# matheusfalcaopinto/triple-hybrid-rag

Hardware: AMD Instinct MI355X
Metric: queries/sec (fused top-10) (higher is better)
Workload: dtype f16 MFMA shortlist scan (f32 accumulate) + f64 rescoring of the f32 rows; 1 GPU; 1000000-doc / 768-d dense-only brute-force cosine top-10 (BASELINE.json configs[1]); pipeline=dense, docs=1000000, dim=768, semantic_top_k=100, fused_top_k=10, shortlist=f16, parallelism=single GPU, world_size_seen=1, rescued_queries=0

## Files before the change

triple-hybrid-rag_amd/_native.py:

```python
from __future__ import annotations

import ctypes as C
import os
from typing import Optional, Tuple

import torch

from . import _build

THR_FLAG_CERTIFIED = 1
THR_FLAG_OVERFLOW = 2
THR_FLAG_EXACT = 4
THR_DENSE_MAX_K = 256
THR_BM25_MAX_TERMS = 32
THR_BM25_MAX_QUERIES = 1 << 20
THR_GRAPH_MAX_SEEDS = 16
THR_RRF_MAX_PER_CHANNEL = 128
THR_TOPK_MAX = 128
THR_SCOPE_MAX_COLS = 8
THR_SCOPE_MAX_PREDS = 4096
THR_SCOPE_MAX_QUERIES = 1 << 20
MAXSIM_TOK_DIMS = (16, 32, 64, 96, 128, 192, 256)
ABI_VERSION = 9

_lib = None


class NativeError(RuntimeError):
    pass


_i64, _i32, _dbl, _sz, _vp = C.c_int64, C.c_int, C.c_double, C.c_size_t, C.c_void_p
_SIGNATURES = {
    "thr_abi_version": (C.c_int, []),
    "thr_error_string": (C.c_char_p, [_i32]),
    "thr_device_info": (_i32, [C.POINTER(_i32), C.POINTER(_i64), C.c_char_p, _i32]),
    "thr_embed_postproc": (_i32, [_vp, _i32, _i32, _i32, _vp, _vp]),
    "thr_doc_norms": (_i32, [_vp, _i64, _i32, _vp, _vp, _vp]),
    "thr_dense_workspace_bytes": (_sz, [_i64, _i32, _i32, _i32]),
    "thr_dense_topk": (_i32, [_vp, _vp, _vp, _i64, _i32, _i64, _vp, _i32, _i32, _i32, _vp, _vp, _vp, _vp,
                              _vp, _vp, _vp, _sz, _vp]),
    "thr_dense_exact_workspace_bytes": (_sz, [_i64, _i32]),
    "thr_dense_topk_exact": (_i32, [_vp, _vp, _i64, _i32, _i64, _vp, _i32, _i32, _vp, _vp, _vp, _vp, _vp,
                                    _vp, _vp, _sz, _vp]),
    "thr_dense_scan_probe": (_i32, [_vp, _vp, _i64, _i32, _vp, _i32, _vp, _sz, _vp]),
    "thr_dense_rescue_workspace_bytes": (_sz, [_i32, _i32]),
    "thr_dense_rescue": (_i32, [_vp, _vp, _i64, _i32, _i64, _vp, _i32, _i32, _vp, _vp, _vp, _vp, _vp, _vp, _vp,
                                _vp, _sz, _vp]),
    "thr_dense_quantize_f16": (_i32, [_vp, _i64, _i32, _vp, _vp, _vp]),
    "thr_dense_f16_workspace_bytes": (_sz, [_i64, _i32, _i32, _i32]),
    "thr_dense_f16_copy_bytes": (_sz, [_i64, _i32]),
    "thr_dense_f16_query_tile": (_i32, [_i32, _i32, _i32]),
    "thr_dense_f16_max_queries": (_i32, [_i32, _i32]),
    "thr_dense_topk_f16": (_i32, [_vp, _vp, _dbl, _vp, _vp, _i64, _i32, _i64, _vp, _i32, _i32,
                                  _i32, _vp, _vp, _vp, _vp, _vp, _vp, _vp, _sz, _vp]),
    "thr_dense_shortlist_f16": (_i32, [_vp, _vp, _dbl, _vp, _i64, _i32, _vp, _i32, _i32, _vp, _vp, _i32, _vp,
                                       _vp, _sz, _vp]),
    "thr_dense_floor": (_i32, [_vp, _i32, _i32, _i32, _i32, _vp, _vp]),
    "thr_dense_finish_f16": (_i32, [_vp, _vp, _dbl, _vp, _vp, _i64, _i32, _i64, _vp, _i32, _i32,
                                    _i32, _vp, _vp, _vp, _vp, _i32, _i32, _vp, _vp, _vp, _vp, _vp, _sz, _vp]),
    "thr_dense_scan_probe_f16": (_i32, [_vp, _vp, _vp, _i64, _i32, _vp, _i32, _vp, _sz, _vp]),
    "thr_dense_scan_stamps_f16": (_i32, [_vp, _i64, _i32, _i32, _vp, _sz, _vp, C.POINTER(_i32), _vp]),
    "thr_lexical_build_workspace_bytes": (_sz, [_i64, _i64]),
    "thr_lexical_build": (_i32, [_vp, _vp, _vp, _i64, _i64, _i64, _vp, _vp, _vp, _vp, _vp, _vp, _vp, _sz, _vp]),
    "thr_csr_append": (_i32, [_vp, _i64, _i64, _vp, _vp, _vp, _i64, _i64, _vp, _vp, _vp, _vp, _vp, _i64, _vp]),
    "thr_csr_compact_workspace_bytes": (_sz, [_i64, _i64]),
    "thr_csr_compact": (_i32, [_vp, _i64, _i64, _vp, _vp, _vp, _i64, _i64, _vp, _vp, _vp, _i64, _vp, _vp, _sz, _vp]),
    "thr_scope_resolve_workspace_bytes": (_sz, [_i64, _i32]),
    "thr_scope_resolve": (_i32, [_vp, _i32, _i64, _vp, _i32, _vp, _vp, _i64, _vp, _vp, _vp, _sz, _vp]),
    "thr_dense_topk_rows_workspace_bytes": (_sz, [_i32, _i32, _i32]),
    "thr_dense_topk_rows": (_i32, [_vp, _vp, _i64, _i32, _i64, _vp, _i32, _i32, _vp, _vp, _i64, _i32, _vp,
                                   _vp, _vp, _vp, _vp, _vp, _sz, _vp]),
    "thr_bm25_block_count": (_sz, [_i64]),
    "thr_bm25_bounds": (_i32, [_vp, _vp, _vp, _vp, _vp, _dbl, _dbl, _dbl, _i64, _i64, _vp, _vp, _vp, _vp]),
    "thr_bm25_workspace_bytes": (_sz, [_i32, _i32, _i32]),
    "thr_bm25_dense_stride": (_i64, [_i64]),
    "thr_bm25_dense_rows": (_i32, [_vp, _vp, _vp, _vp, _vp, _i32, _i64, _i64, _vp, _vp, _vp]),
    "thr_bm25_topk": (_i32, [_vp, _vp, _vp, _vp, _vp, _vp, _vp, _vp, _vp, _vp, _vp, _i64, _dbl, _dbl, _dbl, _i64, _i64, _i64,
                             _vp, _i32, _i32, _i32, _i32, _vp, _vp, _vp, _vp, _vp, _vp, _sz, _vp]),
    "thr_graph_workspace_bytes": (_sz, [_i32, _i64]),
    "thr_graph_topk": (_i32, [_vp, _vp, _i64, _vp, _vp, _vp, _vp, _vp, _vp, _i64, _i64, _vp, _i32,
                              _i32, _i32, _i32, _vp, _vp, _vp, _vp, _vp, _sz, _vp]),
    "thr_graph_topk_scoped": (_i32, [_vp, _vp, _i64, _vp, _vp, _vp, _vp, _vp, _vp, _i64, _i64, _vp, _vp, _vp,
                                     _i32, _i32, _i32, _i32, _vp, _vp, _vp, _vp, _vp, _sz, _vp]),
    "thr_rrf_fuse": (_i32, [_vp, _i32, _vp, _i32, _vp, _i32, _i32, _dbl, _dbl, _dbl, _i32, _i32,
                            _vp, _vp, _vp, _vp, _vp]),
    "thr_rrf_fuse_standalone": (_i32, [_vp, _i32, _vp, _i32, _vp, _i32, _i32, _dbl, _dbl, _dbl, _i32, _i32,
                                       _vp, _vp, _vp, _vp, _vp]),
    "thr_fuse_post": (_i32, [_vp, _vp, _vp, _vp, _i32, _i32, _vp, _i32, _vp, _i32, _vp, _i32, _dbl, _i32,
                             _dbl, _i32, _i32, _vp, _vp, _vp, _vp]),
    "thr_rerank_order": (_i32, [_vp, _i32, _i64, _vp, _vp, _i32, _i32, _i32, _vp, _vp, _vp, _vp]),
    "thr_maxsim": (_i32, [_vp, _i32, _i32, _vp, _i64, _i32, _i32, _vp, _i32, _vp, _i32, _vp]),
    "thr_maxsim_ids": (_i32, [_vp, _i32, _i32, _vp, _i64, _i32, _i32, _vp, _i64, _i32, _vp, _i32, _vp]),
    "thr_maxsim_pack": (_i32, [_vp, _i64, _i32, _i32, _vp, _vp]),
    "thr_merge_topk": (_i32, [_vp, _vp, _i32, _i32, _i32, _i64, _i32, _vp, _vp, _vp, _vp]),
}
EXPORTED_SYMBOLS = tuple(_SIGNATURES)


def lib_path() -> str:
    return _build.LIB_PATH


def load(build_if_missing: bool = True):
    global _lib
    if _lib is not None:
        return _lib
    path = _build.LIB_PATH
    if not os.path.exists(path):
        if not build_if_missing:
            raise NativeError(f"{path} is missing: build it with __graft_entry__.build()")
        _build.build_native()
    try:
        lib = C.CDLL(path)
    except OSError as e:
        raise NativeError(f"cannot load {path}: {e}") from e
    for name, (res, args) in _SIGNATURES.items():
        try:
            fn = getattr(lib, name)
        except AttributeError as e:
            raise NativeError(f"{path} does not export {name}") from e
        fn.restype, fn.argtypes = res, args
    if lib.thr_abi_version() != ABI_VERSION:
        raise NativeError("libthr_hip.so ABI version mismatch; rebuild")
    _lib = lib
    return lib


def _check(rc: int, what: str) -> None:
    if rc != 0:
        msg = load().thr_error_string(rc).decode()
        raise NativeError(f"{what} failed: {msg} (code {rc})")


def _stream() -> int:
    return torch.cuda.current_stream().cuda_stream


def _dev(t: Optional[torch.Tensor], dtype, name: str, ndim: Optional[int] = None) -> int:
    if t is None:
        return 0
    if not isinstance(t, torch.Tensor) or not t.is_cuda:
        raise NativeError(f"{name}: expected a CUDA(HIP) tensor")
    if t.dtype != dtype:
        raise NativeError(f"{name}: expected dtype {dtype}, got {t.dtype}")
    if not t.is_contiguous():
        raise NativeError(f"{name}: must be contiguous")
    if ndim is not None and t.dim() != ndim:
        raise NativeError(f"{name}: expected {ndim} dims, got {t.dim()}")
    return t.data_ptr()


def device_info() -> Tuple[int, int, str]:
    cus, hbm = C.c_int(0), C.c_int64(0)
    arch = C.create_string_buffer(128)
    torch.cuda.current_device()
    _check(load().thr_device_info(C.byref(cus), C.byref(hbm), arch, 128), "thr_device_info")
    return cus.value, hbm.value, arch.value.decode()


def embed_postproc(full: torch.Tensor, store_dim: int) -> torch.Tensor:
    p = _dev(full, torch.float32, "full", 2)
    n, fd = full.shape
    out = torch.empty((n, min(fd, store_dim)), dtype=torch.float32, device=full.device)
    if n:
        _check(load().thr_embed_postproc(p, n, fd, store_dim, out.data_ptr(), _stream()),
               "thr_embed_postproc")
    return out


def doc_norms(docs: torch.Tensor) -> Tuple[torch.Tensor, torch.Tensor]:
    p = _dev(docs, torch.float32, "docs", 2)
    n, d = docs.shape
    dn = torch.empty(n, dtype=torch.float64, device=docs.device)
    inv = torch.empty(n, dtype=torch.float32, device=docs.device)
    if n:
        _check(load().thr_doc_norms(p, n, d, dn.data_ptr(), inv.data_ptr(), _stream()),
               "thr_doc_norms")
    return dn, inv


def dense_workspace_bytes(n_docs: int, dim: int, n_queries: int, kprime: int) -> int:
    return int(load().thr_dense_workspace_bytes(n_docs, dim, n_queries, kprime))


def _alloc_out(nq: int, k: int, device):
    tile = torch.empty((2, nq, k), dtype=torch.int64, device=device)
    return (tile[0].view(torch.float64), tile[1],
            torch.empty(nq, dtype=torch.int32, device=device),
            torch.empty(nq, dtype=torch.int32, device=device))


def _coll(doc_coll, query_coll, n: int, nq: int):
    if query_coll is None:
        return None, None
    if doc_coll is None:
        raise NativeError("query_coll without doc_coll")
    if doc_coll.shape != (n,) or query_coll.shape != (nq,):
        raise NativeError("doc_coll / query_coll have the wrong length")
    return _dev(doc_coll, torch.int32, "doc_coll", 1), _dev(query_coll, torch.int32, "query_coll", 1)


def dense_topk(docs, dnorm, inv_norm, queries, k: int, kprime: int, id_base: int = 0,
               workspace: Optional[torch.Tensor] = None, doc_coll=None, query_coll=None):
    pd = _dev(docs, torch.float32, "docs", 2)
    n, d = docs.shape
    pq = _dev(queries, torch.float32, "queries", 2)
    nq = queries.shape[0]
    if queries.shape[1] != d:
        raise NativeError(f"queries dim {queries.shape[1]} != docs dim {d}")
    pn = _dev(dnorm, torch.float64, "dnorm", 1)
    pi = _dev(inv_norm, torch.float32, "inv_norm", 1)
    if dnorm.shape[0] != n or inv_norm.shape[0] != n:
        raise NativeError("dnorm / inv_norm length != n_docs")
    need = dense_workspace_bytes(n, d, nq, kprime)
    if workspace is None or workspace.numel() * workspace.element_size() < need:
        workspace = torch.empty(need, dtype=torch.uint8, device=docs.device)
    pw = _dev(workspace, workspace.dtype, "workspace")
    S, I, cnt, flg = _alloc_out(nq, k, docs.device)
    pdc, pqc = _coll(doc_coll, query_coll, n, nq)
    _check(load().thr_dense_topk(pd, pn, pi, n, d, id_base, pq, nq, k, kprime, pdc, pqc, S.data_ptr(),
                                 I.data_ptr(), cnt.data_ptr(), flg.data_ptr(), pw,
                                 workspace.numel() * workspace.element_size(), _stream()),
           "thr_dense_topk")
    return S, I, cnt, flg


def dense_topk_exact(docs, dnorm, queries, k: int, id_base: int = 0, doc_coll=None, query_coll=None):
    pd = _dev(docs, torch.float32, "docs", 2)
    n, d = docs.shape
    pq = _dev(queries, torch.float32, "queries", 2)
    nq = queries.shape[0]
    if queries.shape[1] != d:
        raise NativeError(f"queries dim {queries.shape[1]} != docs dim {d}")
    pn = _dev(dnorm, torch.float64, "dnorm", 1)
    if dnorm.shape[0] != n:
        raise NativeError("dnorm length != n_docs")
    need = int(load().thr_dense_exact_workspace_bytes(n, nq))
    ws = torch.empty(need, dtype=torch.uint8, device=docs.device)
    S, I, cnt, flg = _alloc_out(nq, k, docs.device)
    pdc, pqc = _coll(doc_coll, query_coll, n, nq)
    _check(load().thr_dense_topk_exact(pd, pn, n, d, id_base, pq, nq, k, pdc, pqc, S.data_ptr(),
                                       I.data_ptr(), cnt.data_ptr(), flg.data_ptr(),
                                       ws.data_ptr(), need, _stream()), "thr_dense_topk_exact")
    return S, I, cnt, flg


def dense_scan_probe(docs, inv_norm, queries, workspace: torch.Tensor) -> None:
    pd = _dev(docs, torch.float32, "docs", 2)
    n, d = docs.shape
    pq = _dev(queries, torch.float32, "queries", 2)
    if queries.shape[1] != d or inv_norm.shape[0] != n:
        raise NativeError("probe: shape mismatch")
    pi = _dev(inv_norm, torch.float32, "inv_norm", 1)
    pw = _dev(workspace, workspace.dtype, "workspace")
    _check(load().thr_dense_scan_probe(pd, pi, n, d, pq, queries.shape[0], pw,
                                       workspace.numel() * workspace.element_size(), _stream()),
           "thr_dense_scan_probe")


def dense_f16_query_tile(dim: int, packed: bool, n_queries: int) -> int:
    return int(load().thr_dense_f16_query_tile(dim, 1 if packed else 0, n_queries))


def dense_f16_max_queries(dim: int, packed: bool) -> int:
    return int(load().thr_dense_f16_max_queries(dim, 1 if packed else 0))


def dense_rescue_workspace_bytes(n_queries: int, k: int) -> int:
    return int(load().thr_dense_rescue_workspace_bytes(n_queries, k))


def dense_rescue(docs, dnorm, queries, S, I, cnt, flg, id_base: int = 0,
                 workspace: Optional[torch.Tensor] = None, doc_coll=None, query_coll=None) -> torch.Tensor:
    pd = _dev(docs, torch.float32, "docs", 2)
    pn = _dev(dnorm, torch.float64, "dnorm", 1)
    pq = _dev(queries, torch.float32, "queries", 2)
    n, d = docs.shape
    nq, k = I.shape
    need = int(load().thr_dense_rescue_workspace_bytes(nq, k))
    if workspace is None or workspace.numel() * workspace.element_size() < need:
        workspace = torch.empty(need, dtype=torch.uint8, device=docs.device)
    n_rescued = torch.zeros(1, dtype=torch.int32, device=docs.device)
    pdc, pqc = _coll(doc_coll, query_coll, n, nq)
    _check(load().thr_dense_rescue(pd, pn, n, d, id_base, pq, nq, k, pdc, pqc, S.data_ptr(), I.data_ptr(),
                                   cnt.data_ptr(), flg.data_ptr(), n_rescued.data_ptr(),
                                   workspace.data_ptr(),
                                   workspace.numel() * workspace.element_size(), _stream()),
           "thr_dense_rescue")
    return n_rescued


def dense_quantize_f16(docs: torch.Tensor, keep_copy: bool = True):
    p = _dev(docs, torch.float32, "docs", 2)
    n, d = docs.shape
    d16 = None
    if keep_copy:
        nbytes = int(load().thr_dense_f16_copy_bytes(n, d))
        d16 = torch.empty((nbytes // (2 * d), d), dtype=torch.float16, device=docs.device)
    err = torch.zeros(1, dtype=torch.float32, device=docs.device)
    _check(load().thr_dense_quantize_f16(p, n, d, d16.data_ptr() if keep_copy else None,
                                         err.data_ptr(), _stream()), "thr_dense_quantize_f16")
    return d16, float(err.item())


def dense_quantize_f16_into(docs: torch.Tensor, d16: Optional[torch.Tensor], err: torch.Tensor) -> None:
    p = _dev(docs, torch.float32, "docs", 2)
    n, d = docs.shape
    pe = _dev(err, torch.float32, "err", 1)
    ph = None
    if d16 is not None:
        ph = _dev(d16, torch.float16, "d16", 2)
        if d16.shape[1] != d or d16.numel() * 2 < int(load().thr_dense_f16_copy_bytes(n, d)):
            raise NativeError("dense_quantize_f16_into: the float16 destination is too small")
    if err.numel() != 1:
        raise NativeError("dense_quantize_f16_into: err is one float32")
    _check(load().thr_dense_quantize_f16(p, n, d, ph, pe, _stream()), "thr_dense_quantize_f16")


def dense_f16_layout(dim: int) -> str:
    return f"fragment-major/mfma{32 if os.environ.get('THR_DENSE_MFMA') == '32' else 16}/dim{dim}"


def dense_f16_workspace_bytes(n_docs: int, dim: int, n_queries: int, kprime: int) -> int:
    return int(load().thr_dense_f16_workspace_bytes(n_docs, dim, n_queries, kprime))


def dense_topk_f16(docs, docs16, doc_rel_err: float, dnorm, inv_norm, queries, k: int,
                   kprime: int, id_base: int = 0, workspace: Optional[torch.Tensor] = None,
                   doc_coll=None, query_coll=None):
    pd = _dev(docs, torch.float32, "docs", 2)
    ph = _dev(docs16, torch.float16, "docs16", 2) if docs16 is not None else None
    n, d = docs.shape
    if docs16 is not None and tuple(docs16.shape) != ((n + 31) // 32 * 32, d):
        raise NativeError("docs16 is not the fragment-major copy of docs (thr_dense_quantize_f16)")
    pq = _dev(queries, torch.float32, "queries", 2)
    nq = queries.shape[0]
    if queries.shape[1] != d:
        raise NativeError(f"queries dim {queries.shape[1]} != docs dim {d}")
    pn = _dev(dnorm, torch.float64, "dnorm", 1)
    pi = _dev(inv_norm, torch.float32, "inv_norm", 1)
    if dnorm.shape[0] != n or inv_norm.shape[0] != n:
        raise NativeError("dnorm / inv_norm length != n_docs")
    need = dense_f16_workspace_bytes(n, d, nq, kprime)
    if workspace is None or workspace.numel() * workspace.element_size() < need:
        workspace = torch.empty(need, dtype=torch.uint8, device=docs.device)
    pw = _dev(workspace, workspace.dtype, "workspace")
    S, I, cnt, flg = _alloc_out(nq, k, docs.device)
    pdc, pqc = _coll(doc_coll, query_coll, n, nq)
    _check(load().thr_dense_topk_f16(pd, ph, float(doc_rel_err), pn, pi, n, d, id_base, pq, nq, k,
                                     kprime, pdc, pqc, S.data_ptr(), I.data_ptr(), cnt.data_ptr(),
                                     flg.data_ptr(), pw,
                                     workspace.numel() * workspace.element_size(), _stream()),
           "thr_dense_topk_f16")
    return S, I, cnt, flg


def dense_shortlist_f16(docs, docs16, doc_rel_err: float, inv_norm, queries, kprime: int, m: int,
                        workspace: torch.Tensor, doc_coll=None, query_coll=None) -> torch.Tensor:
    pd = _dev(docs, torch.float32, "docs", 2)
    ph = _dev(docs16, torch.float16, "docs16", 2) if docs16 is not None else None
    n, d = docs.shape
    pq = _dev(queries, torch.float32, "queries", 2)
    nq = queries.shape[0]
    if queries.shape[1] != d or inv_norm.shape[0] != n:
        raise NativeError("shortlist: shape mismatch")
    pi = _dev(inv_norm, torch.float32, "inv_norm", 1)
    need = dense_f16_workspace_bytes(n, d, nq, kprime)
    if workspace.numel() * workspace.element_size() < need:
        raise NativeError("shortlist: workspace smaller than thr_dense_f16_workspace_bytes")
    pw = _dev(workspace, workspace.dtype, "workspace")
    pdc, pqc = _coll(doc_coll, query_coll, n, nq)
    lb = torch.empty((nq, m), dtype=torch.float32, device=docs.device)
    _check(load().thr_dense_shortlist_f16(pd, ph, float(doc_rel_err), pi, n, d, pq, nq, kprime, pdc, pqc,
                                          m, lb.data_ptr(), pw,
                                          workspace.numel() * workspace.element_size(), _stream()),
           "thr_dense_shortlist_f16")
    return lb


def dense_floor(top_lb: torch.Tensor, k: int) -> torch.Tensor:
    p = _dev(top_lb, torch.float32, "top_lb", 3)
    g, nq, m = top_lb.shape
    out = torch.empty(nq, dtype=torch.float32, device=top_lb.device)
    _check(load().thr_dense_floor(p, g, nq, m, k, out.data_ptr(), _stream()), "thr_dense_floor")
    return out


def dense_finish_f16(docs, docs16, doc_rel_err: float, dnorm, inv_norm, queries, k: int, kprime: int,
                     gfloor: Optional[torch.Tensor], id_base: int, workspace: torch.Tensor,
                     doc_coll=None, query_coll=None, lb_all: Optional[torch.Tensor] = None):
    pd = _dev(docs, torch.float32, "docs", 2)
    ph = _dev(docs16, torch.float16, "docs16", 2) if docs16 is not None else None
    n, d = docs.shape
    pq = _dev(queries, torch.float32, "queries", 2)
    nq = queries.shape[0]
    pn = _dev(dnorm, torch.float64, "dnorm", 1)
    pi = _dev(inv_norm, torch.float32, "inv_norm", 1)
    if queries.shape[1] != d or dnorm.shape[0] != n or inv_norm.shape[0] != n:
        raise NativeError("finish: shape mismatch")
    pg = None
    if gfloor is not None:
        pg = _dev(gfloor, torch.float32, "gfloor", 1)
        if gfloor.shape[0] != nq:
            raise NativeError("gfloor: one value per query")
    pl, g, m = None, 0, 0
    if lb_all is not None:
        if gfloor is not None:
            raise NativeError("finish: gfloor or lb_all, not both")
        pl = _dev(lb_all, torch.float32, "lb_all", 3)
        g, nq_l, m = lb_all.shape
        if nq_l != nq:
            raise NativeError("lb_all: [n_shards, nq, m]")
    pw = _dev(workspace, workspace.dtype, "workspace")
    S, I, cnt, flg = _alloc_out(nq, k, docs.device)
    pdc, pqc = _coll(doc_coll, query_coll, n, nq)
    _check(load().thr_dense_finish_f16(pd, ph, float(doc_rel_err), pn, pi, n, d, id_base, pq, nq, k,
                                       kprime, pdc, pqc, pg, pl, g, m, S.data_ptr(), I.data_ptr(),
                                       cnt.data_ptr(), flg.data_ptr(), pw,
                                       workspace.numel() * workspace.element_size(), _stream()),
           "thr_dense_finish_f16")
    return S, I, cnt, flg


def dense_scan_probe_f16(docs, docs16, inv_norm, queries, workspace: torch.Tensor) -> None:
    pd = _dev(docs, torch.float32, "docs", 2)
    ph = _dev(docs16, torch.float16, "docs16", 2) if docs16 is not None else None
    n, d = docs.shape
    pq = _dev(queries, torch.float32, "queries", 2)
    if queries.shape[1] != d or inv_norm.shape[0] != n:
        raise NativeError("probe: shape mismatch")
    pi = _dev(inv_norm, torch.float32, "inv_norm", 1)
    pw = _dev(workspace, workspace.dtype, "workspace")
    _check(load().thr_dense_scan_probe_f16(pd, ph, pi, n, d, pq, queries.shape[0], pw,
                                           workspace.numel() * workspace.element_size(),
                                           _stream()), "thr_dense_scan_probe_f16")


def dense_scan_stamps_f16(docs16, n_docs: int, queries_n: int, workspace: torch.Tensor):
    ph = _dev(docs16, torch.float16, "docs16", 2)
    d = docs16.shape[1]
    pw = _dev(workspace, workspace.dtype, "workspace")
    nbytes = workspace.numel() * workspace.element_size()
    nw = C.c_int(0)
    _check(load().thr_dense_scan_stamps_f16(ph, n_docs, d, queries_n, pw, nbytes, None, C.byref(nw),
                                            _stream()), "thr_dense_scan_stamps_f16")
    out = torch.zeros((nw.value, 8), dtype=torch.int64, device=docs16.device)
    _check(load().thr_dense_scan_stamps_f16(ph, n_docs, d, queries_n, pw, nbytes, out.data_ptr(),
                                            C.byref(nw), _stream()), "thr_dense_scan_stamps_f16")
    return out


def lexical_build(doc: torch.Tensor, term: torch.Tensor, tf: Optional[torch.Tensor], n_docs: int,
                  n_vocab: int):
    pdoc = _dev(doc, torch.int32, "doc", 1)
    pterm = _dev(term, torch.int32, "term", 1)
    ptf = _dev(tf, torch.int32, "tf", 1) if tf is not None else None
    n = doc.shape[0]
    if term.shape[0] != n or (tf is not None and tf.shape[0] != n):
        raise NativeError("lexical_build: doc / term / tf lengths differ")
    dev = doc.device
    rowptr = torch.empty(n_vocab + 1, dtype=torch.int64, device=dev)
    post_doc = torch.empty(max(n, 1), dtype=torch.int32, device=dev)
    post_tf = torch.empty(max(n, 1), dtype=torch.int32, device=dev)
    doclen = torch.empty(n_docs, dtype=torch.float32, device=dev)
    df = torch.empty(n_vocab, dtype=torch.int64, device=dev)
    nnz = torch.zeros(1, dtype=torch.int64, device=dev)
    if n == 0:
        return rowptr.zero_(), post_doc[:0], post_tf[:0], doclen.zero_(), df.zero_()
    need = int(load().thr_lexical_build_workspace_bytes(n, n_vocab))
    ws = torch.empty(need, dtype=torch.uint8, device=dev)
    _check(load().thr_lexical_build(pdoc, pterm, ptf, n, n_docs, n_vocab, rowptr.data_ptr(),
                                    post_doc.data_ptr(), post_tf.data_ptr(), doclen.data_ptr(),
                                    df.data_ptr(), nnz.data_ptr(), ws.data_ptr(), need, _stream()),
           "thr_lexical_build")
    k = int(nnz.item())
    return rowptr, post_doc[:k].clone(), post_tf[:k].clone(), doclen, df


def csr_append(rowptr_a, a0, a1, rowptr_b, b0, b1, out0=None, out1=None):
    rows_a = 0 if rowptr_a is None else rowptr_a.shape[0] - 1
    rows_b = rowptr_b.shape[0] - 1
    pra = _dev(rowptr_a, torch.int64, "rowptr_a", 1)
    prb = _dev(rowptr_b, torch.int64, "rowptr_b", 1)
    if rows_b < max(rows_a, 1):
        raise NativeError(f"csr_append: B has {rows_b} rows, A has {rows_a} (rows only grow)")
    if b0.dtype.itemsize != 4 or (a0 is not None and a0.dtype != b0.dtype):
        raise NativeError("csr_append: payloads are 4-byte elements of one dtype per array")
    if a0 is not None and (a1 is None) != (b1 is None):
        raise NativeError("csr_append: A and B carry the same number of payload arrays")
    if b1 is not None and (b1.dtype.itemsize != 4 or (a1 is not None and a1.dtype != b1.dtype)):
        raise NativeError("csr_append: payloads are 4-byte elements of one dtype per array")
    nnz_a = 0 if a0 is None else a0.shape[0]
    nnz_b = b0.shape[0]
    if (a1 is not None and a1.shape[0] != nnz_a) or (b1 is not None and b1.shape[0] != nnz_b):
        raise NativeError("csr_append: the payloads of one CSR have one length")
    dev = rowptr_b.device
    nnz = nnz_a + nnz_b
    if out0 is None:
        out0 = torch.empty(nnz, dtype=b0.dtype, device=dev)
    if out1 is None and b1 is not None:
        out1 = torch.empty(nnz, dtype=b1.dtype, device=dev)
    if out0.dtype != b0.dtype or out0.shape[0] < nnz or \
            (b1 is not None and (out1.dtype != b1.dtype or out1.shape[0] < nnz)):
        raise NativeError("csr_append: destination too small or of another dtype")
    rowptr_out = torch.empty(rows_b + 1, dtype=torch.int64, device=dev)
    cap = out0.shape[0] if b1 is None else min(out0.shape[0], out1.shape[0])
    _check(load().thr_csr_append(pra, rows_a, nnz_a, _dev(a0, b0.dtype, "a0", 1) if nnz_a else None,
                                 _dev(a1, b1.dtype, "a1", 1) if nnz_a and b1 is not None else None,
                                 prb, rows_b, nnz_b, _dev(b0, b0.dtype, "b0", 1) if nnz_b else None,
                                 _dev(b1, b1.dtype, "b1", 1) if nnz_b and b1 is not None else None,
                                 rowptr_out.data_ptr(), _dev(out0, b0.dtype, "out0", 1) if nnz else None,
                                 _dev(out1, b1.dtype, "out1", 1) if nnz and b1 is not None else None,
                                 cap, _stream()), "thr_csr_append")
    return rowptr_out, out0, (out1 if b1 is not None else None), nnz


def csr_compact(rowptr, ids, pay, remap, id_base: int = 0, ids_out=None, pay_out=None):
    rows, nnz = rowptr.shape[0] - 1, ids.shape[0]
    if rows < 1:
        raise NativeError("csr_compact: rowptr has no rows")
    if id_base < 0:
        raise NativeError("csr_compact: id_base is negative")
    if pay is not None and (pay.dtype.itemsize != 4 or pay.dim() != 1 or pay.shape[0] != nnz):
        raise NativeError("csr_compact: the payload is a 1-d array of 4-byte elements, one per id")
    if pay is None and pay_out is not None:
        raise NativeError("csr_compact: pay_out without a payload")
    for out, like, name in ((ids_out, ids, "ids_out"), (pay_out, pay, "pay_out")):
        if out is not None and (out.dtype != like.dtype or out.dim() != 1 or out.shape[0] < nnz):
            raise NativeError(f"csr_compact: {name} is too small (room for every entry is needed) or of another dtype")
    prp = _dev(rowptr, torch.int64, "rowptr", 1)
    pid = _dev(ids, torch.int32, "ids", 1)
    prm = _dev(remap, torch.int32, "remap", 1)
    dev = ids.device
    if ids_out is None:
        ids_out = torch.empty(nnz, dtype=torch.int32, device=dev)
    if pay_out is None and pay is not None:
        pay_out = torch.empty(nnz, dtype=pay.dtype, device=dev)
    rowptr_out = torch.empty(rows + 1, dtype=torch.int64, device=dev)
    kept = torch.zeros(1, dtype=torch.int64, device=dev)
    need = int(load().thr_csr_compact_workspace_bytes(rows, nnz))
    ws = torch.empty(max(need, 1), dtype=torch.uint8, device=dev)
    cap = ids_out.shape[0] if pay is None else min(ids_out.shape[0], pay_out.shape[0])
    _check(load().thr_csr_compact(prp, rows, nnz, pid if nnz else None,
                                  _dev(pay, pay.dtype, "pay", 1) if nnz and pay is not None else None,
                                  prm if remap.shape[0] else None, remap.shape[0], int(id_base),
                                  rowptr_out.data_ptr(), _dev(ids_out, torch.int32, "ids_out", 1) if nnz else None,
                                  _dev(pay_out, pay.dtype, "pay_out", 1) if nnz and pay is not None else None,
                                  cap, kept.data_ptr(), ws.data_ptr(), need, _stream()), "thr_csr_compact")
    return rowptr_out, ids_out, (pay_out if pay is not None else None), int(kept.item())


def scope_resolve(cols, preds, cap: Optional[int] = None, want_labels: bool = True, rows_out=None):
    cols = list(cols)
    if not 1 <= len(cols) <= THR_SCOPE_MAX_COLS:
        raise NativeError(f"scope_resolve: 1 .. {THR_SCOPE_MAX_COLS} attribute columns, got {len(cols)}")
    n = cols[0].shape[0]
    if any(c.dim() != 1 or c.shape[0] != n for c in cols):
        raise NativeError("scope_resolve: every column is 1-d of the same length")
    if preds.dim() != 2 or preds.shape[1] != len(cols):
        raise NativeError(f"scope_resolve: preds must be [P, {len(cols)}]")
    P = preds.shape[0]
    if not 1 <= P <= THR_SCOPE_MAX_PREDS:
        raise NativeError(f"scope_resolve: 1 .. {THR_SCOPE_MAX_PREDS} predicates per call, got {P}")
    cap = n if cap is None else int(cap)
    if cap < 0:
        raise NativeError("scope_resolve: cap is negative")
    ptrs = (C.c_void_p * len(cols))(*[_dev(c, torch.int32, "column", 1) for c in cols])
    pp = _dev(preds, torch.int32, "preds", 2)
    dev = preds.device
    rowptr = torch.empty(P + 1, dtype=torch.int64, device=dev)
    if rows_out is not None:
        if rows_out.dim() != 1 or rows_out.shape[0] < cap:
            raise NativeError("scope_resolve: rows_out holds fewer than cap entries")
        _dev(rows_out, torch.int32, "rows_out", 1)
    rows = torch.empty(cap, dtype=torch.int32, device=dev) if rows_out is None else rows_out
    labels = torch.empty(n, dtype=torch.int32, device=dev) if want_labels else None
    overlap = torch.empty(1, dtype=torch.int32, device=dev) if want_labels else None
    need = int(load().thr_scope_resolve_workspace_bytes(n, P))
    ws = torch.empty(max(need, 1), dtype=torch.uint8, device=dev)
    _check(load().thr_scope_resolve(ptrs, len(cols), n, pp, P, rowptr.data_ptr(), rows.data_ptr() if cap else None,
                                    cap, labels.data_ptr() if want_labels else None,
                                    overlap.data_ptr() if want_labels else None, ws.data_ptr(), need, _stream()),
           "thr_scope_resolve")
    return rowptr, rows, labels, overlap


def dense_topk_rows(docs, dnorm, queries, k: int, rowptr, rows, query_scope, id_base: int = 0):
    pd = _dev(docs, torch.float32, "docs", 2)
    n, d = docs.shape
    pq = _dev(queries, torch.float32, "queries", 2)
    nq = queries.shape[0]
    if queries.shape[1] != d:
        raise NativeError(f"queries dim {queries.shape[1]} != docs dim {d}")
    pn = _dev(dnorm, torch.float64, "dnorm", 1)
    if dnorm.shape[0] != n:
        raise NativeError("dnorm length != n_docs")
    P = rowptr.shape[0] - 1
    if not 1 <= P <= THR_SCOPE_MAX_PREDS:
        raise NativeError(f"dense_topk_rows: 1 .. {THR_SCOPE_MAX_PREDS} scopes")
    if query_scope.shape != (nq,):
        raise NativeError("dense_topk_rows: query_scope has the wrong length")
    if not 1 <= k <= THR_DENSE_MAX_K:
        raise NativeError(f"dense_topk_rows: k must be 1 .. {THR_DENSE_MAX_K}")
    prp = _dev(rowptr, torch.int64, "rowptr", 1)
    prw = _dev(rows, torch.int32, "rows", 1)
    pqs = _dev(query_scope, torch.int32, "query_scope", 1)
    need = int(load().thr_dense_topk_rows_workspace_bytes(nq, P, k))
    ws = torch.empty(max(need, 1), dtype=torch.uint8, device=docs.device)
    S, I, cnt, flg = _alloc_out(nq, k, docs.device)
    _check(load().thr_dense_topk_rows(pd, pn, n, d, int(id_base), pq, nq, k, prp, prw if rows.shape[0] else None,
                                      rows.shape[0], P, pqs, S.data_ptr(), I.data_ptr(), cnt.data_ptr(),
                                      flg.data_ptr(), ws.data_ptr(), need, _stream()), "thr_dense_topk_rows")
    return S, I, cnt, flg


def bm25_bounds(rowptr, post_doc, post_tf, doclen, idf, avgdl: float, k1: float = 1.2,
                b: float = 0.75):
    pr = _dev(rowptr, torch.int64, "rowptr", 1)
    pdoc = _dev(post_doc, torch.int32, "post_doc", 1)
    ptf = _dev(post_tf, torch.int32, "post_tf", 1)
    pdl = _dev(doclen, torch.float32, "doclen", 1)
    pidf = _dev(idf, torch.float64, "idf", 1)
    v, nnz = idf.shape[0], post_doc.shape[0]
    tub = torch.zeros(v, dtype=torch.float64, device=rowptr.device)
    bub = torch.zeros(max(int(load().thr_bm25_block_count(nnz)), 1), dtype=torch.float64,
                      device=rowptr.device)
    imp = torch.zeros(nnz + 4, dtype=torch.uint8, device=rowptr.device)
    if nnz:
        _check(load().thr_bm25_bounds(pr, pdoc, ptf, pdl, pidf, avgdl, k1, b, v, nnz, tub.data_ptr(),
                                      bub.data_ptr(), imp.data_ptr(), _stream()), "thr_bm25_bounds")
    return tub, bub, imp


def bm25_dense_terms(rowptr, post_doc, post_tf, post_imp, n_docs: int, min_share: float = 0.125,
                     max_terms: int = 512, max_bytes: int = 12 << 30):
    _dev(rowptr, torch.int64, "rowptr", 1)
    df = rowptr[1:] - rowptr[:-1]
    cand = torch.nonzero(df.to(torch.float64) >= min_share * n_docs).flatten()
    if cand.numel() == 0 or n_docs <= 0:
        return None
    max_terms = min(max_terms, max_bytes // (3 * int(load().thr_bm25_dense_stride(n_docs))))
    if max_terms <= 0:
        return None
    keep = []
    for t in cand[torch.argsort(df[cand], descending=True, stable=True)][:max_terms].tolist():
        lo, hi = int(rowptr[t]), int(rowptr[t + 1])
        if int(post_tf[lo:hi].max()) <= 65535:
            keep.append(t)
    if not keep:
        return None
    terms = torch.tensor(sorted(keep), dtype=torch.int32, device=rowptr.device)
    stride = int(load().thr_bm25_dense_stride(n_docs))
    dimp = torch.empty((len(keep), stride), dtype=torch.uint8, device=rowptr.device)
    dtf = torch.empty((len(keep), stride), dtype=torch.int16, device=rowptr.device)
    _check(load().thr_bm25_dense_rows(_dev(rowptr, torch.int64, "rowptr", 1), _dev(post_doc, torch.int32, "post_doc", 1),
                                      _dev(post_tf, torch.int32, "post_tf", 1), _dev(post_imp, torch.uint8, "post_imp", 1),
                                      terms.data_ptr(), len(keep), n_docs, int(df[terms.long()].max()),
                                      dimp.data_ptr(), dtf.data_ptr(), _stream()), "thr_bm25_dense_rows")
    slot = torch.full((rowptr.shape[0] - 1,), -1, dtype=torch.int32, device=rowptr.device)
    slot[terms.long()] = torch.arange(len(keep), dtype=torch.int32, device=rowptr.device)
    return slot, dimp, dtf, stride


def bm25_workspace_bytes(n_queries: int, max_terms: int, k: int) -> int:
    return int(load().thr_bm25_workspace_bytes(n_queries, max_terms, k))


def bm25_check_batch(n_queries: int) -> None:
    if n_queries > THR_BM25_MAX_QUERIES:
        raise NativeError(f"bm25: {n_queries} queries in one call, the limit is {THR_BM25_MAX_QUERIES} "
                          "(THR_BM25_MAX_QUERIES): split the batch")


def bm25_topk(rowptr, post_doc, post_tf, doclen, idf, avgdl: float, query_terms, k: int,
              id_base: int = 0, k1: float = 1.2, b: float = 0.75, bounds=None,
              conjunctive: bool = False, doc_coll=None, query_coll=None,
              workspace: Optional[torch.Tensor] = None, dense=None):
    pr = _dev(rowptr, torch.int64, "rowptr", 1)
    pdoc = _dev(post_doc, torch.int32, "post_doc", 1)
    ptf = _dev(post_tf, torch.int32, "post_tf", 1)
    pdl = _dev(doclen, torch.float32, "doclen", 1)
    pidf = _dev(idf, torch.float64, "idf", 1)
    pqt = _dev(query_terms, torch.int32, "query_terms", 2)
    if post_doc.shape != post_tf.shape or idf.shape[0] + 1 != rowptr.shape[0]:
        raise NativeError("bm25: CSR arrays are inconsistent")
    nq, mt = query_terms.shape
    bm25_check_batch(nq)
    if mt > THR_BM25_MAX_TERMS or k > THR_TOPK_MAX:
        raise NativeError("bm25: too many terms per query or k too large")
    ptu = pbu = pim = None
    if bounds is not None:
        ptu, pbu = _dev(bounds[0], torch.float64, "term_ub", 1), _dev(bounds[1], torch.float64, "block_ub", 1)
        if bounds[0].shape[0] != idf.shape[0]:
            raise NativeError("bm25: term_ub length != vocabulary size")
        if len(bounds) > 2 and bounds[2] is not None:
            pim = _dev(bounds[2], torch.uint8, "post_imp", 1)
            if bounds[2].shape[0] < post_doc.shape[0]:
                raise NativeError("bm25: post_imp shorter than the posting array")
    pds = pdi = pdt = None
    dstride = 0
    if dense is not None:
        if pim is None:
            raise NativeError("bm25: dense rows need the bounds with the impacts")
        pds, pdi = _dev(dense[0], torch.int32, "dense_slot", 1), _dev(dense[1], torch.uint8, "dense_imp", 2)
        pdt, dstride = _dev(dense[2], torch.int16, "dense_tf", 2), int(dense[3])
        if dense[0].shape[0] != idf.shape[0] or dense[1].shape != dense[2].shape or dense[1].shape[1] != dstride:
            raise NativeError("bm25: dense rows are inconsistent")
    pdc = pqc = None
    if query_coll is not None:
        if doc_coll is None:
            raise NativeError("bm25: query_coll without doc_coll")
        pdc, pqc = _dev(doc_coll, torch.int32, "doc_coll", 1), _dev(query_coll, torch.int32, "query_coll", 1)
        if doc_coll.shape[0] != doclen.shape[0] or query_coll.shape[0] != nq:
            raise NativeError("bm25: doc_coll / query_coll have the wrong length")
    S, I, cnt, _ = _alloc_out(nq, k, rowptr.device)
    need = bm25_workspace_bytes(nq, mt, k)
    if workspace is None or workspace.numel() * workspace.element_size() < need:
        workspace = torch.empty(need, dtype=torch.uint8, device=rowptr.device)
    pw = _dev(workspace, workspace.dtype, "workspace")
    _check(load().thr_bm25_topk(pr, pdoc, ptf, pdl, pidf, ptu, pbu, pim, pds, pdi, pdt, dstride,
                                avgdl, k1, b, doclen.shape[0],
                                idf.shape[0], id_base, pqt, nq, mt, k, 1 if conjunctive else 0, pdc,
                                pqc, S.data_ptr(), I.data_ptr(), cnt.data_ptr(), pw,
                                workspace.numel() * workspace.element_size(), _stream()),
           "thr_bm25_topk")
    return S, I, cnt


def graph_workspace_bytes(n_queries: int, n_entities: int) -> int:
    return int(load().thr_graph_workspace_bytes(n_queries, n_entities))


def graph_topk(ent_rowptr, ent_col, men_rowptr, men_chunk, men_conf, query_seeds, hops: int,
               k: int, chunk_base: int, n_chunks: int, transposed=None,
               workspace: Optional[torch.Tensor] = None):
    return _graph_call("thr_graph_topk", ent_rowptr, ent_col, men_rowptr, men_chunk, men_conf, query_seeds,
                       hops, k, chunk_base, n_chunks, transposed, workspace, None)


def graph_topk_scoped(ent_rowptr, ent_col, men_rowptr, men_chunk, men_conf, query_seeds, hops: int,
                      k: int, chunk_base: int, n_chunks: int, doc_label, query_label, transposed=None,
                      workspace: Optional[torch.Tensor] = None):
    if doc_label is None or query_label is None:
        raise NativeError("graph_topk_scoped: doc_label and query_label are required (graph_topk is the unfiltered call)")
    return _graph_call("thr_graph_topk_scoped", ent_rowptr, ent_col, men_rowptr, men_chunk, men_conf,
                       query_seeds, hops, k, chunk_base, n_chunks, transposed, workspace, (doc_label, query_label))


def _graph_call(entry, ent_rowptr, ent_col, men_rowptr, men_chunk, men_conf, query_seeds, hops, k, chunk_base,
                n_chunks, transposed, workspace, labels):
    per = _dev(ent_rowptr, torch.int64, "ent_rowptr", 1)
    pec = _dev(ent_col, torch.int32, "ent_col", 1)
    pmr = _dev(men_rowptr, torch.int64, "men_rowptr", 1)
    pmc = _dev(men_chunk, torch.int32, "men_chunk", 1)
    pmw = _dev(men_conf, torch.float32, "men_conf", 1)
    pqs = _dev(query_seeds, torch.int32, "query_seeds", 2)
    if ent_rowptr.shape != men_rowptr.shape or men_chunk.shape != men_conf.shape:
        raise NativeError("graph: CSR arrays are inconsistent")
    ptr = pte = ptw = None
    n_ent = ent_rowptr.shape[0] - 1
    if transposed is not None:
        tr, te, tw = transposed
        ptr, pte, ptw = (_dev(tr, torch.int64, "tmen_rowptr", 1), _dev(te, torch.int32, "tmen_ent", 1),
                         _dev(tw, torch.float32, "tmen_conf", 1))
        if tr.shape[0] != n_chunks + 1 or te.shape != tw.shape:
            raise NativeError("graph: transposed mention CSR is inconsistent")
    nq, ms = query_seeds.shape
    if ms > THR_GRAPH_MAX_SEEDS or k > THR_TOPK_MAX:
        raise NativeError("graph: too many seeds per query or k too large")
    scoped = ()
    if labels is not None:
        doc_label, query_label = labels
        scoped = (_dev(doc_label, torch.int32, "doc_label", 1), _dev(query_label, torch.int32, "query_label", 1))
        if doc_label.shape[0] != n_chunks or query_label.shape[0] != nq:
            raise NativeError("graph: doc_label holds one label per chunk of the shard, query_label one per query")
    need = int(load().thr_graph_workspace_bytes(nq, n_ent if transposed is not None else 0))
    ws = workspace
    if ws is None or ws.numel() * ws.element_size() < need:
        ws = torch.empty(max(need, 8), dtype=torch.uint8, device=ent_rowptr.device)
    S, I, cnt, flg = _alloc_out(nq, k, ent_rowptr.device)
    _check(getattr(load(), entry)(per, pec, n_ent, pmr, pmc, pmw, ptr, pte, ptw, chunk_base, n_chunks, *scoped,
                                  pqs, nq, ms, hops, k, S.data_ptr(), I.data_ptr(), cnt.data_ptr(),
                                  flg.data_ptr(), ws.data_ptr(), need, _stream()),
           entry)
    return S, I, cnt, flg


def graph_transpose_mentions(men_rowptr, men_chunk, men_conf, chunk_base: int, n_chunks: int):
    ne = men_rowptr.shape[0] - 1
    ent = torch.repeat_interleave(torch.arange(ne, dtype=torch.int32, device=men_rowptr.device),
                                  (men_rowptr[1:] - men_rowptr[:-1]))
    local = men_chunk.to(torch.int64) - chunk_base
    keep = (local >= 0) & (local < n_chunks)
    ent, conf, local = ent[keep], men_conf[keep], local[keep]
    order = torch.sort(local, stable=True).indices
    counts = torch.bincount(local, minlength=n_chunks)
    rowptr = torch.zeros(n_chunks + 1, dtype=torch.int64, device=men_rowptr.device)
    rowptr[1:] = torch.cumsum(counts, 0)
    return rowptr, ent[order].contiguous(), conf[order].contiguous()


def rrf_fuse(lex_ids, sem_ids, graph_ids, top_k: int, w_lex: float = 0.7, w_sem: float = 0.8,
             w_graph: float = 1.0, rrf_k: int = 60, want_ranks: bool = False):
    chans = [lex_ids, sem_ids, graph_ids]
    ref = next(c for c in chans if c is not None)
    nq = ref.shape[0]
    ptrs, widths = [], []
    for name, c in zip(("lex_ids", "sem_ids", "graph_ids"), chans):
        if c is None:
            ptrs.append(0)
            widths.append(0)
            continue
        ptrs.append(_dev(c, torch.int64, name, 2))
        if c.shape[0] != nq or c.shape[1] > THR_RRF_MAX_PER_CHANNEL:
            raise NativeError(f"rrf: bad shape for {name}")
        widths.append(c.shape[1])
    dev = ref.device
    out_ids = torch.empty((nq, top_k), dtype=torch.int64, device=dev)
    out_sc = torch.empty((nq, top_k), dtype=torch.float64, device=dev)
    out_rk = torch.empty((nq, top_k, 3), dtype=torch.int32, device=dev) if want_ranks else None
    cnt = torch.empty(nq, dtype=torch.int32, device=dev)
    _check(load().thr_rrf_fuse(ptrs[0], widths[0], ptrs[1], widths[1], ptrs[2], widths[2], nq,
                               w_lex, w_sem, w_graph, rrf_k, top_k, out_ids.data_ptr(),
                               out_sc.data_ptr(), out_rk.data_ptr() if want_ranks else 0,
                               cnt.data_ptr(), _stream()), "thr_rrf_fuse")
    return out_ids, out_sc, out_rk, cnt


def rrf_fuse_standalone(lex_ids, sem_ids, graph_ids, top_k: int, w_lex: float = 0.7, w_sem: float = 0.8,
                        w_graph: float = 1.0, two_channels: bool = False, want_ranks: bool = True):
    chans = [lex_ids, sem_ids, graph_ids]
    ref = next(c for c in chans if c is not None)
    nq = ref.shape[0]
    ptrs, widths = [], []
    for name, c in zip(("lex_ids", "sem_ids", "graph_ids"), chans):
        if c is None:
            ptrs.append(0)
            widths.append(0)
            continue
        ptrs.append(_dev(c, torch.int64, name, 2))
        if c.shape[0] != nq or c.shape[1] > THR_RRF_MAX_PER_CHANNEL:
            raise NativeError(f"rrf: bad shape for {name}")
        widths.append(c.shape[1])
    dev = ref.device
    out_ids = torch.empty((nq, top_k), dtype=torch.int64, device=dev)
    out_sc = torch.empty((nq, top_k), dtype=torch.float64, device=dev)
    out_rk = torch.empty((nq, top_k, 3), dtype=torch.int32, device=dev) if want_ranks else None
    cnt = torch.empty(nq, dtype=torch.int32, device=dev)
    _check(load().thr_rrf_fuse_standalone(ptrs[0], widths[0], ptrs[1], widths[1], ptrs[2], widths[2], nq,
                                          w_lex, w_sem, w_graph, 1 if two_channels else 0, top_k,
                                          out_ids.data_ptr(), out_sc.data_ptr(),
                                          out_rk.data_ptr() if want_ranks else 0, cnt.data_ptr(),
                                          _stream()), "thr_rrf_fuse_standalone")
    return out_ids, out_sc, out_rk, cnt


def fuse_post(ids, scores, ranks=None, counts=None, channel_scores=(None, None, None),
              safety_threshold: float = 0.0, denoise_quantile: Optional[float] = None,
              normalize: bool = False, top_k: int = 0):
    pi = _dev(ids, torch.int64, "ids", 2)
    ps = _dev(scores, torch.float64, "scores", 2)
    nq, n = ids.shape
    if tuple(scores.shape) != (nq, n):
        raise NativeError("fuse_post: ids / scores shape mismatch")
    pr = _dev(ranks, torch.int32, "ranks", 3) if ranks is not None else None
    if ranks is not None and tuple(ranks.shape) != (nq, n, 3):
        raise NativeError("fuse_post: ranks must be [nq, n, 3]")
    pc = _dev(counts, torch.int32, "counts", 1) if counts is not None else None
    cp, cw = [], []
    for name, c in zip(("lex_scores", "sem_scores", "graph_scores"), channel_scores):
        cp.append(_dev(c, torch.float64, name, 2) if c is not None else None)
        cw.append(c.shape[1] if c is not None else 0)
        if c is not None and c.shape[0] != nq:
            raise NativeError(f"fuse_post: bad shape for {name}")
    out_ids = torch.empty_like(ids)
    out_sc = torch.empty_like(scores)
    out_c = torch.empty(nq, dtype=torch.int32, device=ids.device)
    _check(load().thr_fuse_post(pi, ps, pr, pc, nq, n, cp[0], cw[0], cp[1], cw[1], cp[2], cw[2],
                                float(safety_threshold), 0 if denoise_quantile is None else 1,
                                float(denoise_quantile or 0.0), 1 if normalize else 0, int(top_k),
                                out_ids.data_ptr(), out_sc.data_ptr(), out_c.data_ptr(), _stream()),
           "thr_fuse_post")
    return out_ids, out_sc, out_c


def maxsim_check_tokens(what: str, tok_dim: int, *n_tokens: int) -> None:
    if any(n <= 0 or n % 32 for n in n_tokens):
        raise NativeError(f"{what}: q_tokens / d_tokens must be positive multiples of 32, got {n_tokens}")
    if tok_dim not in MAXSIM_TOK_DIMS:
        raise NativeError(f"{what}: tok_dim {tok_dim} is not supported: the MaxSim kernels take tok_dim in "
                          f"{list(MAXSIM_TOK_DIMS)}")


def maxsim_pack(dtok: torch.Tensor) -> torch.Tensor:
    pdt = _dev(dtok, torch.float16, "dtok", 3)
    nd, dt, td = dtok.shape
    maxsim_check_tokens("maxsim_pack", td, dt)
    out = torch.empty_like(dtok)
    _check(load().thr_maxsim_pack(pdt, nd, dt, td, out.data_ptr(), _stream()), "thr_maxsim_pack")
    return out


def maxsim(qtok: torch.Tensor, dtok: torch.Tensor, cand: torch.Tensor,
           packed: bool = False) -> torch.Tensor:
    pq = _dev(qtok, torch.float16, "qtok", 3)
    pdt = _dev(dtok, torch.float16, "dtok", 3)
    pc = _dev(cand, torch.int32, "cand", 2)
    nq, qt, td = qtok.shape
    nd, dt, td2 = dtok.shape
    if td != td2 or cand.shape[0] != nq:
        raise NativeError("maxsim: shape mismatch")
    maxsim_check_tokens("maxsim", td, qt, dt)
    out = torch.empty(cand.shape, dtype=torch.float32, device=qtok.device)
    _check(load().thr_maxsim(pq, nq, qt, pdt, nd, dt, td, pc, cand.shape[1], out.data_ptr(),
                             1 if packed else 0, _stream()), "thr_maxsim")
    return out


def maxsim_ids(qtok: torch.Tensor, dtok: torch.Tensor, cand_ids: torch.Tensor, id_base: int,
               packed: bool = False) -> torch.Tensor:
    pq = _dev(qtok, torch.float16, "qtok", 3)
    pdt = _dev(dtok, torch.float16, "dtok", 3)
    pc = _dev(cand_ids, torch.int64, "cand_ids", 2)
    nq, qt, td = qtok.shape
    nd, dt, td2 = dtok.shape
    if td != td2 or cand_ids.shape[0] != nq:
        raise NativeError("maxsim: shape mismatch")
    maxsim_check_tokens("maxsim_ids", td, qt, dt)
    out = torch.empty(cand_ids.shape, dtype=torch.float32, device=qtok.device)
    _check(load().thr_maxsim_ids(pq, nq, qt, pdt, nd, dt, td, pc, int(id_base), cand_ids.shape[1],
                                 out.data_ptr(), 1 if packed else 0, _stream()), "thr_maxsim_ids")
    return out


def rerank_order(scores: torch.Tensor, ids: torch.Tensor, counts: Optional[torch.Tensor], top_k: int):
    if scores.dim() == 2:
        scores = scores.unsqueeze(0)
    ps = _dev(scores, torch.float32, "scores", 3)
    pi = _dev(ids, torch.int64, "ids", 2)
    pc = _dev(counts, torch.int32, "counts", 1) if counts is not None else None
    nl, nq, n = scores.shape
    if tuple(ids.shape) != (nq, n):
        raise NativeError("rerank_order: ids shape != scores shape")
    out_ids = torch.empty((nq, top_k), dtype=torch.int64, device=ids.device)
    out_s = torch.empty((nq, top_k), dtype=torch.float64, device=ids.device)
    out_c = torch.empty(nq, dtype=torch.int32, device=ids.device)
    _check(load().thr_rerank_order(ps, nl, nq * n, pi, pc, nq, n, top_k, out_ids.data_ptr(),
                                   out_s.data_ptr(), out_c.data_ptr(), _stream()), "thr_rerank_order")
    return out_ids, out_s, out_c


def merge_topk(in_scores: torch.Tensor, in_ids: torch.Tensor, k_out: int):
    if in_scores.shape != in_ids.shape or in_scores.dim() != 3:
        raise NativeError("merge: shape mismatch")
    if in_scores.dtype != torch.float64 or in_ids.dtype != torch.int64 or not in_scores.is_cuda:
        raise NativeError("merge: in_scores must be float64, in_ids int64, on the GPU")
    nl, nq, kin = in_scores.shape
    for t in (in_scores, in_ids):
        if t.stride(2) != 1 or t.stride(1) != kin or (nl > 1 and t.stride(0) < nq * kin):
            raise NativeError("merge: lists must be contiguous [n_queries, k_in] blocks")
    if nl > 1 and in_scores.stride(0) != in_ids.stride(0):
        raise NativeError("merge: scores and ids must share the list stride")
    stride = in_scores.stride(0) if nl > 1 else nq * kin
    S, I, cnt, _ = _alloc_out(nq, k_out, in_scores.device)
    _check(load().thr_merge_topk(in_scores.data_ptr(), in_ids.data_ptr(), nq, nl, kin, stride,
                                 k_out, S.data_ptr(), I.data_ptr(), cnt.data_ptr(), _stream()),
           "thr_merge_topk")
    return S, I, cnt
```

triple-hybrid-rag_amd/csrc/dense.hip:

```cpp
#include <stdlib.h>

#include "dense_common.hpp"

namespace thr {

struct DenseKnobs {
    bool forced_q;
    int shape;
    bool forced32;
};
static const DenseKnobs& dense_knobs() {
    static const DenseKnobs knobs = [] {
        DenseKnobs K;
        const char* e = getenv("THR_DENSE_F16");
        K.forced_q = e && e[0] == 'q';
        e = getenv("THR_DENSE_MFMA");
        K.shape = (e && atoi(e) == 32) ? 32 : 16;
        e = getenv("THR_DENSE_QW");
        K.forced32 = e && atoi(e) == 32;
        return K;
    }();
    return knobs;
}

bool qreg_staggered(int dim) { return !dense_knobs().forced_q && dim <= 768; }
int qreg_waves(int dim) { return qreg_staggered(dim) ? 8 : 4; }
int qreg_shape(int) { return dense_knobs().shape; }
int qreg_qw(int dim) {
    return (dim == 1024 && !qreg_staggered(dim) && qreg_shape(dim) == 16 && !dense_knobs().forced32) ? 48 : 32;
}
constexpr int QREG_MAX_SEG = 1024;
int qreg_max_queries(int dim) {
    const int qt = qreg_qw(dim) * qreg_waves(dim);
    const int64_t m = (int64_t)UINT32_MAX / ((int64_t)CAND_CAP * (int64_t)sizeof(Cand));
    return (int)(m / qt * qt);
}


static DensePlan make_plan(void* ws, int64_t n_docs, int n_queries, int kprime, int kind, int dim,
                           bool packed) {
    DensePlan p;
    p.kind = kind;
    p.packed = kind == KIND_F16 && packed;
    p.nq = (kind == KIND_F16 && !p.packed) ? f16_pick_nq(dim) : 1;
    p.row_bits = (kind == KIND_F16 && !p.packed) ? ROW_BITS_F16 : ROW_BITS;
    p.qtile = p.packed ? qreg_qw(dim) * qreg_waves(dim)
              : kind == KIND_F16 ? 32 * p.nq : MF_QT;
    p.ntiles = (n_queries + p.qtile - 1) / p.qtile;
    p.qpad = p.ntiles * p.qtile;
    const int64_t groups = (n_docs + MF_ROWS - 1) / MF_ROWS;
    p.sampled = n_docs > CAND_CAP / 2;
    const int ks_cap = p.packed ? 32 : 64;
    p.ksample = kprime < ks_cap ? kprime : ks_cap;
    double aim = (p.packed ? 2896.0 : 4096.0) * sqrt((double)n_docs / 1.0e6);
    const double aim_lo = 8.0 * kprime < 4096.0 ? 8.0 * kprime : 4096.0;
    aim = aim < aim_lo ? aim_lo : aim > 4096.0 ? 4096.0 : aim;
    int64_t target = (int64_t)((double)n_docs * (double)p.ksample / aim);
    if (target > SAMPLE_MAX) target = SAMPLE_MAX;
    if (target < 4 * (int64_t)p.ksample) target = 4 * (int64_t)p.ksample;
    int64_t sg = (target + MF_ROWS - 1) / MF_ROWS;
    if (sg > groups) sg = groups;
    p.sample_stride = sg > 0 ? groups / sg : 1;
    if (p.sample_stride < 1) p.sample_stride = 1;
    p.sample_groups = p.sampled ? sg : 0;
    p.sample_docs = p.sample_groups * MF_ROWS;
    p.groups = groups;
    p.tile_cap = p.packed ? 1 : p.qtile * (CAND_CAP / 2);
    const size_t qpad = (size_t)p.qpad;
    Arena A{(char*)ws};
    p.tau = A.take<float>(qpad);
    p.qerr = A.take<float>(qpad);
    if (kind != KIND_F16) p.qerr = nullptr;
    p.cnt = A.take<int>(qpad * (p.packed ? QREG_MAX_SEG : 1));
    p.tcnt = A.take<int>(p.ntiles);
    p.cand = A.take<Cand>(qpad * CAND_CAP);
    p.tlist = A.take<Cand>((size_t)p.ntiles * p.tile_cap);
    p.sample = A.take<float>(qpad * (size_t)p.sample_docs);
    p.qfrag = A.take<_Float16>(p.packed ? qpad * (size_t)dim : 0);
    p.sel_rows = A.take<int32_t>(qpad * SEL_BIG_BAND);
    p.sel_meta = A.take<int32_t>(4 * qpad);
    p.total = A.total;
    return p;
}

dim3 scan_grid(int ntiles, int64_t n_row_tiles, int waves, bool* shared_rows, int blocks_per_cu,
               int m_cap) {
    const int cus = num_cus() * blocks_per_cu;
    int64_t m_max = n_row_tiles / (8 * (int64_t)waves);
    if (m_max < 1) m_max = 1;
    if (m_max > m_cap) m_max = m_cap;
    int best_m = 1;
    double best_eff = 0.0;
    for (int m = 1; m <= (int)m_max; ++m) {
        const int64_t g = 8 * (int64_t)m * ntiles;
        const int64_t rounds = (g + cus - 1) / cus;
        const double eff = (double)g / (double)(rounds * cus);
        if (eff > best_eff + 1e-9) {
            best_eff = eff;
            best_m = m;
        }
    }
    *shared_rows = ntiles > 1;
    return dim3((unsigned)(8 * best_m * ntiles), 1u);
}

bool scan_nt(bool shared_rows) { return !shared_rows; }


template <int MODE>
static int launch_scan(const DensePlan& P, const DenseIndex& X, const DenseBatch& B, int* nseg = nullptr) {
    constexpr bool all = MODE == MODE_ALL;
    const int64_t units = all ? P.sample_groups : P.groups, stride = all ? P.sample_stride : 1;
    const float* tau = all ? nullptr : P.tau;
    float* smp = all ? P.sample : nullptr;
    const int64_t ld = all ? P.sample_docs : 0;
    const int32_t* doc_coll = all ? nullptr : X.doc_coll;
    const int32_t* query_coll = all ? nullptr : B.query_coll;
    if (P.packed)
        return launch_scan_f16q<MODE>(X.dim, X.docs16, P.qfrag, P.ntiles, units, stride, tau,
                                      all ? nullptr : P.cnt, all ? nullptr : P.cand, smp, ld, B.st,
                                      nseg, doc_coll, query_coll, B.n_queries);
    int* tcnt = all ? nullptr : P.tcnt;
    Cand* tlist = all ? nullptr : P.tlist;
    const int tile_cap = all ? 0 : P.tile_cap;
    if (P.kind == KIND_F16)
        return launch_scan_f16<MODE>(X.dim, P.nq, X.docs, X.inv_norm, X.n_docs, B.queries, B.n_queries,
                                     P.ntiles, units, stride, tau, tcnt, tlist, tile_cap, smp, ld, B.st,
                                     doc_coll, query_coll);
    return launch_scan_mfma<MODE>(X.dim, X.docs, X.inv_norm, X.n_docs, B.queries, B.n_queries, P.ntiles,
                                  units, stride, tau, tcnt, tlist, tile_cap, smp, ld, B.st, doc_coll,
                                  query_coll);
}

static int dense_pipeline(const DensePlan& P, const DenseIndex& X, const DenseBatch& B,
                          const DensePhase& S) {
    int rc, nseg = 0;
    if (S.phase != PIPE_FINISH) {
        hipError_t e = hipMemsetAsync(P.cnt, 0, (char*)P.cand - (char*)P.cnt, B.st);
        if (e != hipSuccess) return (int)e;
        if (P.packed && (rc = launch_pack_queries(X.dim, B.queries, B.n_queries, P.qpad, P.qfrag, P.qerr, B.st)))
            return rc;
        if (P.sampled && (rc = launch_scan<MODE_ALL>(P, X, B))) return rc;
        if ((rc = launch_threshold(P, X, B))) return rc;
        if ((rc = launch_scan<MODE_FILTER>(P, X, B, &nseg))) return rc;
        if (!P.packed && (rc = launch_bucket(P, B.st))) return rc;
    } else if (P.packed) {
        if ((rc = launch_scan_f16q<MODE_FILTER, true>(X.dim, X.docs16, P.qfrag, P.ntiles, P.groups, 1,
                                                      nullptr, nullptr, nullptr, nullptr, 0, B.st, &nseg)))
            return rc;
    }
    if ((rc = launch_band(P, X, B, S, nseg))) return rc;
    if (S.phase == PIPE_SHORTLIST) return THR_OK;
    return launch_rescore(P, X, B);
}

}

using namespace thr;

extern "C" size_t thr_dense_workspace_bytes(int64_t n_docs, int dim, int n_queries, int kprime) {
    if (n_docs <= 0 || n_queries <= 0) return 0;
    return make_plan(nullptr, n_docs, n_queries, kprime, KIND_F32, dim, false).total;
}

static int dense_args_ok(const void* docs, const void* dnorm, const void* inv_norm,
                         const void* queries, const void* a, const void* b, const void* c,
                         const void* d, const void* ws, int64_t n_docs, int n_queries, int k,
                         int kprime) {
    THR_RETURN_IF(!docs || !dnorm || !inv_norm || !queries || !a || !b || !c || !d || !ws,
                  THR_ERR_INVALID);
    THR_RETURN_IF(n_docs <= 0 || n_queries <= 0 || k <= 0 || kprime < k ||
                      kprime > THR_DENSE_MAX_K,
                  THR_ERR_INVALID);
    return THR_OK;
}

extern "C" int thr_dense_topk(const float* docs, const double* dnorm, const float* inv_norm,
                              int64_t n_docs, int dim, int64_t id_base, const float* queries,
                              int n_queries, int k, int kprime, const int32_t* doc_coll,
                              const int32_t* query_coll, double* out_scores,
                              int64_t* out_ids, int32_t* out_counts, uint32_t* out_flags,
                              void* workspace, size_t workspace_bytes, thr_stream_t stream) {
    clear_status();
    int rc = dense_args_ok(docs, dnorm, inv_norm, queries, out_scores, out_ids, out_counts,
                           out_flags, workspace, n_docs, n_queries, k, kprime);
    if (rc) return rc;
    THR_RETURN_IF((query_coll != nullptr) != (doc_coll != nullptr), THR_ERR_INVALID);
    THR_RETURN_IF(dim <= 0 || dim % CHUNK != 0 || dim / CHUNK > 4, THR_ERR_UNSUPPORTED);
    THR_RETURN_IF(n_docs >= (int64_t)1 << ROW_BITS, THR_ERR_UNSUPPORTED);
    const DensePlan P = make_plan(workspace, n_docs, n_queries, kprime, KIND_F32, dim, false);
    THR_RETURN_IF(workspace_bytes < P.total, THR_ERR_WORKSPACE);
    const DenseIndex X{docs, inv_norm, n_docs, dim, dnorm, id_base, doc_coll};
    const DenseBatch B{queries, n_queries, k, kprime, query_coll, (hipStream_t)stream,
                       out_scores, out_ids, out_counts, out_flags};
    return dense_pipeline(P, X, B, DensePhase{});
}

extern "C" size_t thr_dense_f16_workspace_bytes(int64_t n_docs, int dim, int n_queries,
                                                int kprime) {
    if (n_docs <= 0 || n_queries <= 0) return 0;
    const size_t a = make_plan(nullptr, n_docs, n_queries, kprime, KIND_F16, dim, false).total;
    const size_t b = make_plan(nullptr, n_docs, n_queries, kprime, KIND_F16, dim, true).total;
    return a > b ? a : b;
}

extern "C" int thr_dense_f16_max_queries(int dim, int packed) {
    if (dim != 512 && dim != 768 && dim != 1024) return 0;
    return packed ? qreg_max_queries(dim) : INT32_MAX;
}

extern "C" int thr_dense_f16_query_tile(int dim, int packed, int n_queries) {
    if (dim != 512 && dim != 768 && dim != 1024) return 0;
    (void)n_queries;
    return packed ? qreg_qw(dim) * qreg_waves(dim) : 32 * f16_pick_nq(dim);
}

extern "C" size_t thr_dense_f16_copy_bytes(int64_t n_docs, int dim) {
    if (n_docs <= 0 || dim <= 0) return 0;
    return sizeof(_Float16) * (size_t)((n_docs + 31) / 32 * 32) * (size_t)dim;
}

extern "C" int thr_dense_quantize_f16(const float* docs, int64_t n_docs, int dim, uint16_t* docs16,
                                      float* max_rel_err, thr_stream_t stream) {
    clear_status();
    THR_RETURN_IF(!docs || !max_rel_err || n_docs <= 0 || dim <= 0, THR_ERR_INVALID);
    THR_RETURN_IF(dim % 64 != 0, THR_ERR_UNSUPPORTED);
    hipStream_t st = (hipStream_t)stream;
    hipError_t e = hipMemsetAsync(max_rel_err, 0, sizeof(float), st);
    if (e != hipSuccess) return (int)e;
    return launch_quantize_f16(docs, n_docs, dim, reinterpret_cast<_Float16*>(docs16),
                               reinterpret_cast<unsigned int*>(max_rel_err), st);
}

static int f16_args_ok(const float* docs, const uint16_t* docs16, double doc_rel_err, int64_t n_docs,
                       int dim, int n_queries, const int32_t* doc_coll, const int32_t* query_coll) {
    (void)docs;
    THR_RETURN_IF((query_coll != nullptr) != (doc_coll != nullptr), THR_ERR_INVALID);
    THR_RETURN_IF(!(doc_rel_err >= 0.0) || !(doc_rel_err < 1.0), THR_ERR_INVALID);
    THR_RETURN_IF(dim != 512 && dim != 768 && dim != 1024, THR_ERR_UNSUPPORTED);
    THR_RETURN_IF(n_docs >= (int64_t)1 << ROW_BITS_F16, THR_ERR_UNSUPPORTED);
    THR_RETURN_IF(docs16 != nullptr && n_queries > qreg_max_queries(dim), THR_ERR_UNSUPPORTED);
    return THR_OK;
}


extern "C" int thr_dense_topk_f16(const float* docs, const uint16_t* docs16, double doc_rel_err,
                                  const double* dnorm, const float* inv_norm, int64_t n_docs,
                                  int dim, int64_t id_base, const float* queries, int n_queries,
                                  int k, int kprime, const int32_t* doc_coll,
                                  const int32_t* query_coll, double* out_scores, int64_t* out_ids,
                                  int32_t* out_counts, uint32_t* out_flags, void* workspace,
                                  size_t workspace_bytes, thr_stream_t stream) {
    clear_status();
    int rc = dense_args_ok(docs, dnorm, inv_norm, queries, out_scores, out_ids, out_counts,
                           out_flags, workspace, n_docs, n_queries, k, kprime);
    if (rc) return rc;
    if ((rc = f16_args_ok(docs, docs16, doc_rel_err, n_docs, dim, n_queries, doc_coll, query_coll))) return rc;
    const DensePlan P = make_plan(workspace, n_docs, n_queries, kprime, KIND_F16, dim, docs16 != nullptr);
    THR_RETURN_IF(workspace_bytes < P.total, THR_ERR_WORKSPACE);
    const DenseIndex X{docs, inv_norm, n_docs, dim, dnorm, id_base, doc_coll,
                       reinterpret_cast<const _Float16*>(docs16), doc_rel_err};
    const DenseBatch B{queries, n_queries, k, kprime, query_coll, (hipStream_t)stream,
                       out_scores, out_ids, out_counts, out_flags};
    return dense_pipeline(P, X, B, DensePhase{});
}

extern "C" int thr_dense_shortlist_f16(const float* docs, const uint16_t* docs16, double doc_rel_err,
                                       const float* inv_norm, int64_t n_docs, int dim,
                                       const float* queries, int n_queries, int kprime,
                                       const int32_t* doc_coll, const int32_t* query_coll, int m,
                                       float* top_lb, void* workspace, size_t workspace_bytes,
                                       thr_stream_t stream) {
    clear_status();
    THR_RETURN_IF(!docs || !inv_norm || !queries || !top_lb || !workspace, THR_ERR_INVALID);
    THR_RETURN_IF(n_docs <= 0 || n_queries <= 0 || kprime <= 0 || kprime > THR_DENSE_MAX_K || m <= 0 ||
                      m > THR_DENSE_MAX_K,
                  THR_ERR_INVALID);
    int rc = f16_args_ok(docs, docs16, doc_rel_err, n_docs, dim, n_queries, doc_coll, query_coll);
    if (rc) return rc;
    const DensePlan P = make_plan(workspace, n_docs, n_queries, kprime, KIND_F16, dim, docs16 != nullptr);
    THR_RETURN_IF(workspace_bytes < P.total, THR_ERR_WORKSPACE);
    const DenseIndex X{docs, inv_norm, n_docs, dim, nullptr, 0, doc_coll,
                       reinterpret_cast<const _Float16*>(docs16), doc_rel_err};
    const DenseBatch B{queries, n_queries, 0, kprime, query_coll, (hipStream_t)stream};
    return dense_pipeline(P, X, B, DensePhase{PIPE_SHORTLIST, top_lb, m});
}

extern "C" int thr_dense_finish_f16(const float* docs, const uint16_t* docs16, double doc_rel_err,
                                    const double* dnorm, const float* inv_norm, int64_t n_docs,
                                    int dim, int64_t id_base, const float* queries, int n_queries,
                                    int k, int kprime, const int32_t* doc_coll,
                                    const int32_t* query_coll, const float* gfloor,
                                    const float* top_lb_all, int n_shards, int m,
                                    double* out_scores, int64_t* out_ids, int32_t* out_counts,
                                    uint32_t* out_flags, void* workspace, size_t workspace_bytes,
                                    thr_stream_t stream) {
    clear_status();
    int rc = dense_args_ok(docs, dnorm, inv_norm, queries, out_scores, out_ids, out_counts,
                           out_flags, workspace, n_docs, n_queries, k, kprime);
    if (rc) return rc;
    if ((rc = f16_args_ok(docs, docs16, doc_rel_err, n_docs, dim, n_queries, doc_coll, query_coll))) return rc;
    THR_RETURN_IF(gfloor && top_lb_all, THR_ERR_INVALID);
    THR_RETURN_IF(top_lb_all && (n_shards <= 0 || m <= 0), THR_ERR_INVALID);
    THR_RETURN_IF(top_lb_all && (int64_t)n_shards * m > CS_BINS, THR_ERR_CAPACITY);
    const DensePlan P = make_plan(workspace, n_docs, n_queries, kprime, KIND_F16, dim, docs16 != nullptr);
    THR_RETURN_IF(workspace_bytes < P.total, THR_ERR_WORKSPACE);
    const DenseIndex X{docs, inv_norm, n_docs, dim, dnorm, id_base, doc_coll,
                       reinterpret_cast<const _Float16*>(docs16), doc_rel_err};
    const DenseBatch B{queries, n_queries, k, kprime, query_coll, (hipStream_t)stream,
                       out_scores, out_ids, out_counts, out_flags};
    return dense_pipeline(P, X, B, DensePhase{PIPE_FINISH, nullptr, m, gfloor, top_lb_all, n_shards});
}

static int scan_probe(const DensePlan& P, const DenseIndex& X, const DenseBatch& B) {
    if (!P.packed) {
        hipError_t e = hipMemsetAsync(P.tcnt, 0, sizeof(int) * P.ntiles, B.st);
        if (e != hipSuccess) return (int)e;
    }
    return launch_scan<MODE_FILTER>(P, X, B);
}

extern "C" int thr_dense_scan_probe(const float* docs, const float* inv_norm, int64_t n_docs,
                                    int dim, const float* queries, int n_queries, void* workspace,
                                    size_t workspace_bytes, thr_stream_t stream) {
    clear_status();
    THR_RETURN_IF(!docs || !inv_norm || !queries || !workspace, THR_ERR_INVALID);
    THR_RETURN_IF(dim <= 0 || dim % CHUNK != 0 || dim / CHUNK > 4, THR_ERR_UNSUPPORTED);
    THR_RETURN_IF(n_docs <= 0 || n_docs >= (int64_t)1 << ROW_BITS || n_queries <= 0,
                  THR_ERR_INVALID);
    const DensePlan P = make_plan(workspace, n_docs, n_queries, 128, KIND_F32, dim, false);
    THR_RETURN_IF(workspace_bytes < P.total, THR_ERR_WORKSPACE);
    return scan_probe(P, DenseIndex{docs, inv_norm, n_docs, dim},
                      DenseBatch{queries, n_queries, 0, 128, nullptr, (hipStream_t)stream});
}

extern "C" int thr_dense_scan_probe_f16(const float* docs, const uint16_t* docs16,
                                        const float* inv_norm,
                                        int64_t n_docs, int dim, const float* queries,
                                        int n_queries, void* workspace, size_t workspace_bytes,
                                        thr_stream_t stream) {
    clear_status();
    THR_RETURN_IF((!docs16 && !docs) || !inv_norm || !queries || !workspace, THR_ERR_INVALID);
    THR_RETURN_IF(dim != 512 && dim != 768 && dim != 1024, THR_ERR_UNSUPPORTED);
    THR_RETURN_IF(n_docs <= 0 || n_docs >= (int64_t)1 << ROW_BITS_F16 || n_queries <= 0,
                  THR_ERR_INVALID);
    THR_RETURN_IF(docs16 != nullptr && n_queries > qreg_max_queries(dim), THR_ERR_UNSUPPORTED);
    const DensePlan P = make_plan(workspace, n_docs, n_queries, 128, KIND_F16, dim, docs16 != nullptr);
    THR_RETURN_IF(workspace_bytes < P.total, THR_ERR_WORKSPACE);
    DenseIndex X{docs, inv_norm, n_docs, dim};
    X.docs16 = reinterpret_cast<const _Float16*>(docs16);
    return scan_probe(P, X, DenseBatch{queries, n_queries, 0, 128, nullptr, (hipStream_t)stream});
}

extern "C" int thr_dense_scan_stamps_f16(const uint16_t* docs16, int64_t n_docs, int dim,
                                         int n_queries, void* workspace, size_t workspace_bytes,
                                         unsigned long long* stamps, int* h_n_waves,
                                         thr_stream_t stream) {
    clear_status();
    THR_RETURN_IF(!docs16 || !workspace || !h_n_waves, THR_ERR_INVALID);
    THR_RETURN_IF(dim != 512 && dim != 768 && dim != 1024, THR_ERR_UNSUPPORTED);
    THR_RETURN_IF(n_docs <= 0 || n_queries <= 0, THR_ERR_INVALID);
    THR_RETURN_IF(qreg_staggered(dim), THR_ERR_UNSUPPORTED);
    THR_RETURN_IF(n_queries > qreg_max_queries(dim), THR_ERR_UNSUPPORTED);
    const DensePlan P = make_plan(workspace, n_docs, n_queries, 128, KIND_F16, dim, true);
    THR_RETURN_IF(workspace_bytes < P.total, THR_ERR_WORKSPACE);
    int blocks = 0;
    int rc = launch_scan_f16q<MODE_FILTER, true>(
        dim, reinterpret_cast<const _Float16*>(docs16), P.qfrag, P.ntiles, P.groups, 1, P.tau, P.cnt,
        P.cand, nullptr, 0, (hipStream_t)stream, nullptr, nullptr, nullptr, n_queries, stamps, &blocks);
    *h_n_waves = blocks * qreg_waves(dim);
    return rc;
}
```

triple-hybrid-rag_amd/csrc/dense_common.hpp:

```cpp
#pragma once
#include <type_traits>

#include "thr_common.hpp"

namespace thr {

constexpr int CHUNK = 256;
constexpr int MODE_ALL = 0, MODE_FILTER = 1;
constexpr int CAND_CAP = 16384;
constexpr int SAMPLE_MAX = 1 << 20;
constexpr int WBUF = 256;
constexpr int ROW_BITS = 27;
constexpr uint32_t ROW_MASK = (1u << ROW_BITS) - 1;
constexpr int ROW_BITS_F16 = 25;
constexpr int SEL_BIG_BAND = 1024;
constexpr int CS_BINS = 4096;

struct Cand {
    float score;
    uint32_t doc;
};

}
struct ScanSlot {
    int qtile, slice, nslices;
};
__device__ __forceinline__ ScanSlot scan_slot(int n_qtiles) {
    ScanSlot s;
    const int b = blockIdx.x, xcd = b & 7, j = b >> 3;
    s.qtile = j % n_qtiles;
    s.slice = xcd + 8 * (j / n_qtiles);
    s.nslices = gridDim.x / n_qtiles;
    return s;
}

namespace thr {

template <int I, int N, typename F>
__device__ __forceinline__ void static_for(F&& f) {
    if constexpr (I < N) {
        f(std::integral_constant<int, I>{});
        static_for<I + 1, N>(f);
    }
}

typedef float f32x16 __attribute__((ext_vector_type(16)));
typedef float f32x4 __attribute__((ext_vector_type(4)));
typedef _Float16 half8 __attribute__((ext_vector_type(8)));

constexpr int MF_ROWS = 32;
constexpr int MF_QT = 32;
constexpr int MF2_STAGE_F4 = MF_ROWS * 8;
constexpr int H_WAVES = 8;

__device__ __forceinline__ int mf_qslot(int q, int cidx, int chunks_per_row) {
    return q * chunks_per_row + ((cidx & ~15) | ((cidx ^ q) & 15));
}

__device__ __forceinline__ int mf2_slot(int row, int chunk) {
    return row * 8 + (chunk ^ ((row >> 1) & 7));
}

__device__ __forceinline__ f32x4 pack_f16x8(f32x4 lo, f32x4 hi) {
    typedef _Float16 half4 __attribute__((ext_vector_type(4)));
    const half4 a = __builtin_convertvector(lo, half4), b = __builtin_convertvector(hi, half4);
    half8 v = {a[0], a[1], a[2], a[3], b[0], b[1], b[2], b[3]};
    return __builtin_bit_cast(f32x4, v);
}

inline size_t f16_lds_bytes(int dim, int nq) {
    return sizeof(_Float16) * 32 * nq * (size_t)dim +
           (sizeof(Cand) * WBUF + sizeof(float4) * MF2_STAGE_F4) * H_WAVES;
}
inline int f16_pick_nq(int dim) { return f16_lds_bytes(dim, 2) <= 160 * 1024 ? 2 : 1; }

inline double scan_eps(int dim) {
    const double u = 5.9604644775390625e-08;
    return ((double)dim + 16.0) * u;
}

constexpr int KIND_F32 = 0, KIND_F16 = 1;
struct DensePlan {
    int kind;
    bool packed;
    int nq, qtile, ntiles, qpad, row_bits, ksample, tile_cap;
    bool sampled;
    int64_t groups, sample_groups, sample_stride, sample_docs;
    float* tau;
    float* qerr;
    int* cnt;
    int* tcnt;
    Cand *cand, *tlist;
    float* sample;
    _Float16* qfrag;
    int32_t *sel_rows, *sel_meta;
    size_t total;
};
struct DenseIndex {
    const float *docs, *inv_norm;
    int64_t n_docs;
    int dim;
    const double* dnorm = nullptr;
    int64_t id_base = 0;
    const int32_t* doc_coll = nullptr;
    const _Float16* docs16 = nullptr;
    double doc_rel_err = 0.0;
};
struct DenseBatch {
    const float* queries;
    int n_queries, k, kprime;
    const int32_t* query_coll;
    hipStream_t st;
    double* out_scores = nullptr;
    int64_t* out_ids = nullptr;
    int32_t* out_counts = nullptr;
    uint32_t* out_flags = nullptr;
};
enum { PIPE_ALL = 0, PIPE_SHORTLIST = 1, PIPE_FINISH = 2 };
struct DensePhase {
    int phase = PIPE_ALL;
    float* top_lb = nullptr;
    int top_m = 0;
    const float* gfloor = nullptr;
    const float* lb_all = nullptr;
    int n_shards = 0;
};

bool qreg_staggered(int dim);
int qreg_waves(int dim);
int qreg_shape(int dim);
int qreg_qw(int dim);
int qreg_max_queries(int dim);
dim3 scan_grid(int ntiles, int64_t n_row_tiles, int waves, bool* shared_rows, int blocks_per_cu = 1,
               int m_cap = 64);
bool scan_nt(bool shared_rows);

template <int MODE>
int launch_scan_mfma(int dim, const float* docs, const float* inv_norm, int64_t n_docs,
                     const float* queries, int n_queries, int ntiles, int64_t n_row_tiles,
                     int64_t tile_stride, const float* tau, int* tile_cnt, Cand* tile_list,
                     int tile_cap, float* sample, int64_t sample_ld, hipStream_t st,
                     const int32_t* doc_coll = nullptr, const int32_t* query_coll = nullptr);
template <int MODE>
int launch_scan_f16(int dim, int nq, const float* rows32, const float* inv_norm, int64_t n_docs,
                    const float* queries, int n_queries, int ntiles, int64_t n_row_tiles,
                    int64_t tile_stride, const float* tau, int* tile_cnt, Cand* tile_list,
                    int tile_cap, float* sample, int64_t sample_ld, hipStream_t st,
                    const int32_t* doc_coll = nullptr, const int32_t* query_coll = nullptr);
template <int MODE, bool PROF = false>
int launch_scan_f16q(int dim, const _Float16* rows16, const _Float16* qfrag, int n_qtiles,
                     int64_t n_row_tiles, int64_t tile_stride, const float* tau, int* seg_cnt,
                     Cand* cand, float* sample, int64_t sample_ld, hipStream_t st,
                     int* nseg_out = nullptr, const int32_t* doc_coll = nullptr,
                     const int32_t* query_coll = nullptr, int n_queries = 1 << 30,
                     unsigned long long* stamps = nullptr, int* n_blocks = nullptr);
int launch_pack_queries(int dim, const float* queries, int n_queries, int qpad, _Float16* qfrag,
                        float* qerr, hipStream_t st);
int launch_quantize_f16(const float* docs, int64_t n_docs, int dim, _Float16* docs16,
                        unsigned int* max_rel_err, hipStream_t st);
int launch_threshold(const DensePlan& P, const DenseIndex& X, const DenseBatch& B);
int launch_bucket(const DensePlan& P, hipStream_t st);
int launch_band(const DensePlan& P, const DenseIndex& X, const DenseBatch& B, const DensePhase& S, int nseg);
int launch_rescore(const DensePlan& P, const DenseIndex& X, const DenseBatch& B);
int launch_merge_scoped(const double* slab_s, const int64_t* slab_id, int n_queries, int n_slabs, int k,
                        int64_t id_base, const int32_t* query_scope, int n_scopes, double* out_scores,
                        int64_t* out_ids, int32_t* out_counts, uint32_t* out_flags, hipStream_t st);

}
```

triple-hybrid-rag_amd/csrc/dense_exact.hip:

```cpp
#include "dense_common.hpp"

namespace thr {

__device__ __forceinline__ double seq_dot_f64(const float* __restrict__ a, const float* b, int d) {
    double s = 0.0;
    const float4* a4 = reinterpret_cast<const float4*>(a);
    for (int i = 0; i < d / 4; ++i) {
        float4 x = a4[i];
        s = __dadd_rn(s, __dmul_rn((double)x.x, (double)b[4 * i + 0]));
        s = __dadd_rn(s, __dmul_rn((double)x.y, (double)b[4 * i + 1]));
        s = __dadd_rn(s, __dmul_rn((double)x.z, (double)b[4 * i + 2]));
        s = __dadd_rn(s, __dmul_rn((double)x.w, (double)b[4 * i + 3]));
    }
    return s;
}

constexpr int EX_THREADS = 256;
constexpr int EX_CAP = 1024;
constexpr int EX_SLABS = 64;

__global__ __launch_bounds__(EX_THREADS) void exact_slab_topk(
    const float* __restrict__ docs, const double* __restrict__ dnorm, int64_t n_docs, int dim,
    const float* __restrict__ queries, int n_queries, int k, double* __restrict__ slab_s,
    int64_t* __restrict__ slab_id, const uint32_t* __restrict__ skip_certified,
    const int32_t* __restrict__ doc_coll, const int32_t* __restrict__ query_coll) {
    extern __shared__ float lds_qv[];
    __shared__ double b_s[EX_CAP];
    __shared__ int64_t b_id[EX_CAP];
    __shared__ int b_cnt;
    __shared__ double t_s;
    __shared__ int64_t t_id;
    __shared__ double s_qn;
    __shared__ unsigned long long s_todo;
    const int slab = blockIdx.x;
    {
        const int q = blockIdx.y + (int)threadIdx.x * (int)gridDim.y;
        const bool todo = threadIdx.x < 64 && q < n_queries &&
                          !(skip_certified && (skip_certified[q] & THR_FLAG_CERTIFIED));
        const unsigned long long m = __ballot(todo);
        if (threadIdx.x == 0) s_todo = m;
        __syncthreads();
    }
    for (unsigned long long todo = s_todo; todo; todo &= todo - 1) {
        const int q = blockIdx.y + (__ffsll((long long)todo) - 1) * (int)gridDim.y;
        __syncthreads();
        for (int i = threadIdx.x; i < dim; i += EX_THREADS) lds_qv[i] = queries[(int64_t)q * dim + i];
        __syncthreads();
        if (threadIdx.x == 0) s_qn = __dsqrt_rn(seq_dot_f64(lds_qv, lds_qv, dim));
        BlockTopK<EX_CAP, EX_THREADS> tk;
        tk.init(b_s, b_id, &b_cnt, &t_s, &t_id, k);
        const double qn = s_qn;
        const int qc = query_coll ? query_coll[q] : -1;
        const int64_t per = (n_docs + EX_SLABS - 1) / EX_SLABS;
        const int64_t lo = slab * per, hi = (lo + per < n_docs) ? lo + per : n_docs;
        for (int64_t base = lo; base < hi; base += EX_THREADS) {
            int64_t row = base + threadIdx.x;
            bool ok = row < hi;
            double sim = -INFINITY;
            if (ok) {
                double dn = dnorm[row];
                if (qc != -1 && doc_coll[row] != qc) dn = 0.0;
                if (dn > 0.0) {
                    double dot = seq_dot_f64(docs + row * dim, lds_qv, dim);
                    sim = qn > 0.0 ? __ddiv_rn(dot, __dmul_rn(qn, dn)) : 0.0;
                }
            }
            tk.push(ok && sim > -INFINITY, sim, row);
        }
        int n = tk.finish();
        for (int i = threadIdx.x; i < k; i += EX_THREADS) {
            int64_t o = ((int64_t)q * EX_SLABS + slab) * k + i;
            slab_s[o] = i < n ? b_s[i] : -INFINITY;
            slab_id[o] = i < n ? b_id[i] : INT64_MAX;
        }
    }
}

template <bool GATED>
__global__ __launch_bounds__(256) void merge_lists(const double* __restrict__ in_s,
                                                   const int64_t* __restrict__ in_id,
                                                   int64_t q_stride, int64_t list_stride,
                                                   int n_lists, int k_in, int k_out,
                                                   int64_t id_add, uint32_t flag_value,
                                                   double* __restrict__ out_s,
                                                   int64_t* __restrict__ out_id,
                                                   int32_t* __restrict__ out_counts,
                                                   uint32_t* __restrict__ out_flags,
                                                   const uint32_t* __restrict__ skip_certified,
                                                   int32_t* __restrict__ n_done,
                                                   const int32_t* __restrict__ query_scope, int P) {
    if (skip_certified && (skip_certified[blockIdx.x] & THR_FLAG_CERTIFIED)) return;
    if (n_done && threadIdx.x == 0) atomicAdd(n_done, 1);
    __shared__ double b_s[EX_CAP];
    __shared__ int64_t b_id[EX_CAP];
    __shared__ int b_cnt;
    __shared__ double t_s;
    __shared__ int64_t t_id;
    const int q = blockIdx.x;
    bool live = true;
    if constexpr (GATED) live = query_scope[q] >= 0 && query_scope[q] < P;
    int n = 0;
    if (live) {
        BlockTopK<EX_CAP, EX_THREADS> tk;
        tk.init(b_s, b_id, &b_cnt, &t_s, &t_id, k_out);
        const int total = n_lists * k_in;
        for (int base = 0; base < total; base += blockDim.x) {
            int i = base + threadIdx.x;
            bool ok = i < total;
            double s = -INFINITY;
            int64_t id = INT64_MAX;
            if (ok) {
                int64_t o = (int64_t)q * q_stride + (int64_t)(i / k_in) * list_stride + (i % k_in);
                s = in_s[o];
                id = in_id[o];
            }
            tk.push(ok && s > -INFINITY && id >= 0 && id != INT64_MAX, s, id);
        }
        n = tk.finish();
    }
    for (int i = threadIdx.x; i < k_out; i += blockDim.x) {
        out_s[(int64_t)q * k_out + i] = i < n ? b_s[i] : -INFINITY;
        out_id[(int64_t)q * k_out + i] = i < n ? b_id[i] + id_add : -1;
    }
    if (threadIdx.x == 0) {
        if (out_counts) out_counts[q] = n;
        if (out_flags) out_flags[q] = flag_value;
    }
}

__global__ __launch_bounds__(256) void merge_ranked_lists(const double* __restrict__ in_s,
                                                          const int64_t* __restrict__ in_id,
                                                          int64_t q_stride, int64_t list_stride,
                                                          int n_lists, int k_in, int k_out,
                                                          double* __restrict__ out_s,
                                                          int64_t* __restrict__ out_id,
                                                          int32_t* __restrict__ out_counts) {
    __shared__ double b_s[EX_CAP];
    __shared__ int64_t b_id[EX_CAP];
    __shared__ int unsorted, n_valid;
    const int q = blockIdx.x;
    const int total = n_lists * k_in;
    if (threadIdx.x == 0) unsorted = 0, n_valid = 0;
    for (int i = threadIdx.x; i < EX_CAP; i += blockDim.x) {
        double sc = -INFINITY;
        int64_t id = INT64_MAX;
        if (i < total) {
            const int64_t o = (int64_t)q * q_stride + (int64_t)(i / k_in) * list_stride + (i % k_in);
            sc = in_s[o];
            id = in_id[o];
            if (!(sc > -INFINITY) || id < 0) sc = -INFINITY, id = INT64_MAX;
        }
        b_s[i] = sc;
        b_id[i] = id;
    }
    for (int i = threadIdx.x; i < k_out; i += blockDim.x) {
        out_s[(int64_t)q * k_out + i] = -INFINITY;
        out_id[(int64_t)q * k_out + i] = -1;
    }
    __syncthreads();
    int mine = 0;
    for (int i = threadIdx.x; i < total; i += blockDim.x) {
        mine += b_id[i] != INT64_MAX ? 1 : 0;
        if (i % k_in + 1 < k_in && better(b_s[i + 1], b_id[i + 1], b_s[i], b_id[i])) unsorted = 1;
    }
    if (mine) atomicAdd(&n_valid, mine);
    __syncthreads();
    if (!unsorted) {
        for (int i = threadIdx.x; i < total; i += blockDim.x) {
            const double ms = b_s[i];
            const int64_t mi = b_id[i];
            if (mi == INT64_MAX) continue;
            const int a = i / k_in;
            int rank = i % k_in;
            for (int b = 0; b < n_lists && rank < k_out; ++b) {
                if (b == a) continue;
                int lo = 0, hi = k_in;
                while (lo < hi) {
                    const int mid = (lo + hi) >> 1;
                    if (better(b_s[b * k_in + mid], b_id[b * k_in + mid], ms, mi)) lo = mid + 1;
                    else hi = mid;
                }
                rank += lo;
            }
            if (rank < k_out) {
                out_s[(int64_t)q * k_out + rank] = ms;
                out_id[(int64_t)q * k_out + rank] = mi;
            }
        }
    } else {
        bitonic_sort_desc<EX_CAP>(b_s, b_id);
        for (int i = threadIdx.x; i < k_out && i < n_valid; i += blockDim.x) {
            out_s[(int64_t)q * k_out + i] = b_s[i];
            out_id[(int64_t)q * k_out + i] = b_id[i];
        }
    }
    if (threadIdx.x == 0 && out_counts) out_counts[q] = n_valid < k_out ? n_valid : k_out;
}

}

using namespace thr;

extern "C" size_t thr_dense_exact_workspace_bytes(int64_t n_docs, int n_queries) {
    (void)n_docs;
    return (size_t)n_queries * EX_SLABS * THR_DENSE_MAX_K * (sizeof(double) + sizeof(int64_t));
}

extern "C" size_t thr_dense_rescue_workspace_bytes(int n_queries, int k) {
    if (n_queries <= 0 || k <= 0) return 0;
    return (size_t)n_queries * EX_SLABS * (size_t)k * (sizeof(double) + sizeof(int64_t));
}

static int exact_topk(const float* docs, const double* dnorm, int64_t n_docs, int dim, int64_t id_base,
                      const float* queries, int n_queries, int k, const int32_t* doc_coll,
                      const int32_t* query_coll, double* out_scores, int64_t* out_ids,
                      int32_t* out_counts, uint32_t* out_flags, void* workspace, size_t workspace_bytes,
                      size_t need, thr_stream_t stream, int grid_y, const uint32_t* certified,
                      int32_t* n_rescued) {
    clear_status();
    THR_RETURN_IF(!docs || !dnorm || !queries || !out_scores || !out_ids || !out_counts ||
                      !out_flags || !workspace,
                  THR_ERR_INVALID);
    THR_RETURN_IF(n_docs <= 0 || n_queries <= 0 || k <= 0 || k > THR_DENSE_MAX_K, THR_ERR_INVALID);
    THR_RETURN_IF(dim <= 0 || dim % 4 != 0, THR_ERR_UNSUPPORTED);
    THR_RETURN_IF(workspace_bytes < need, THR_ERR_WORKSPACE);
    hipStream_t st = (hipStream_t)stream;
    double* slab_s = (double*)workspace;
    int64_t* slab_id = (int64_t*)(slab_s + (size_t)n_queries * EX_SLABS * k);
    hipLaunchKernelGGL(exact_slab_topk, dim3(EX_SLABS, grid_y), dim3(EX_THREADS),
                       sizeof(float) * dim, st, docs, dnorm, n_docs, dim, queries, n_queries, k,
                       slab_s, slab_id, certified, doc_coll, query_coll);
    int rc = launch_status();
    if (rc) return rc;
    hipLaunchKernelGGL(merge_lists<false>, dim3(n_queries), dim3(256), 0, st, slab_s, slab_id,
                       (int64_t)EX_SLABS * k, (int64_t)k, EX_SLABS, k, k, id_base,
                       THR_FLAG_CERTIFIED | THR_FLAG_EXACT, out_scores, out_ids, out_counts,
                       out_flags, certified, n_rescued, (const int32_t*)nullptr, 0);
    return launch_status();
}

int thr::launch_merge_scoped(const double* slab_s, const int64_t* slab_id, int n_queries, int n_slabs, int k,
                             int64_t id_base, const int32_t* query_scope, int n_scopes, double* out_scores,
                             int64_t* out_ids, int32_t* out_counts, uint32_t* out_flags, hipStream_t st) {
    hipLaunchKernelGGL(merge_lists<true>, dim3(n_queries), dim3(256), 0, st, slab_s, slab_id,
                       (int64_t)n_slabs * k, (int64_t)k, n_slabs, k, k, id_base,
                       THR_FLAG_CERTIFIED | THR_FLAG_EXACT, out_scores, out_ids, out_counts, out_flags,
                       (const uint32_t*)nullptr, (int32_t*)nullptr, query_scope, n_scopes);
    return launch_status();
}

extern "C" int thr_dense_topk_exact(const float* docs, const double* dnorm, int64_t n_docs, int dim,
                                    int64_t id_base, const float* queries, int n_queries, int k,
                                    const int32_t* doc_coll, const int32_t* query_coll,
                                    double* out_scores, int64_t* out_ids, int32_t* out_counts,
                                    uint32_t* out_flags, void* workspace, size_t workspace_bytes,
                                    thr_stream_t stream) {
    return exact_topk(docs, dnorm, n_docs, dim, id_base, queries, n_queries, k, doc_coll, query_coll,
                      out_scores, out_ids, out_counts, out_flags, workspace, workspace_bytes,
                      thr_dense_exact_workspace_bytes(n_docs, n_queries), stream, n_queries, nullptr,
                      nullptr);
}

extern "C" int thr_dense_rescue(const float* docs, const double* dnorm, int64_t n_docs, int dim,
                                int64_t id_base, const float* queries, int n_queries, int k,
                                const int32_t* doc_coll, const int32_t* query_coll,
                                double* io_scores, int64_t* io_ids, int32_t* io_counts,
                                uint32_t* io_flags, int32_t* n_rescued, void* workspace,
                                size_t workspace_bytes, thr_stream_t stream) {
    const int rows = (n_queries + 63) / 64 > 16 ? (n_queries + 63) / 64 : (n_queries < 16 ? n_queries : 16);
    return exact_topk(docs, dnorm, n_docs, dim, id_base, queries, n_queries, k, doc_coll, query_coll,
                      io_scores, io_ids, io_counts, io_flags, workspace, workspace_bytes,
                      thr_dense_rescue_workspace_bytes(n_queries, k), stream, rows, io_flags, n_rescued);
}

extern "C" int thr_merge_topk(const double* in_scores, const int64_t* in_ids, int n_queries,
                              int n_lists, int k_in, int64_t list_stride, int k_out,
                              double* out_scores, int64_t* out_ids, int32_t* out_counts,
                              thr_stream_t stream) {
    clear_status();
    THR_RETURN_IF(!in_scores || !in_ids || !out_scores || !out_ids, THR_ERR_INVALID);
    THR_RETURN_IF(n_queries <= 0 || n_lists <= 0 || k_in <= 0 || k_out <= 0 || k_out > EX_CAP / 2,
                  THR_ERR_INVALID);
    if (list_stride == 0) list_stride = (int64_t)n_queries * k_in;
    THR_RETURN_IF(list_stride < (int64_t)n_queries * k_in, THR_ERR_INVALID);
    if ((int64_t)n_lists * k_in <= EX_CAP) {
        hipLaunchKernelGGL(merge_ranked_lists, dim3(n_queries), dim3(256), 0, (hipStream_t)stream,
                           in_scores, in_ids, (int64_t)k_in, list_stride, n_lists, k_in, k_out,
                           out_scores, out_ids, out_counts);
        return launch_status();
    }
    hipLaunchKernelGGL(merge_lists<false>, dim3(n_queries), dim3(256), 0, (hipStream_t)stream, in_scores,
                       in_ids, (int64_t)k_in, list_stride, n_lists, k_in, k_out,
                       (int64_t)0, 0u, out_scores, out_ids, out_counts, (uint32_t*)nullptr,
                       (const uint32_t*)nullptr, (int32_t*)nullptr, (const int32_t*)nullptr, 0);
    return launch_status();
}
```

triple-hybrid-rag_amd/csrc/dense_scan_f16q.hip:

```cpp
#include "dense_scan_f16q.hpp"

namespace thr {

template <int MODE, bool PROF>
int launch_scan_f16q(int dim, const _Float16* rows16, const _Float16* qfrag, int n_qtiles,
                            int64_t n_row_tiles, int64_t tile_stride, const float* tau, int* seg_cnt,
                            Cand* cand, float* sample, int64_t sample_ld, hipStream_t st,
                            int* nseg_out, const int32_t* doc_coll,
                            const int32_t* query_coll, int n_queries,
                            unsigned long long* stamps, int* n_blocks) {
    bool shared_rows = false;
    const bool stag = qreg_staggered(dim);
    const dim3 grid = scan_grid(n_qtiles, n_row_tiles, 1, &shared_rows, (!stag && dim <= 768) ? 2 : 1, 32);
    const int shape = qreg_shape(dim);
    const int nseg = (shape == 16 ? 4 : 2) * (int)(grid.x / n_qtiles);
    if (nseg_out) *nseg_out = nseg;
    if (n_blocks) *n_blocks = (int)grid.x;
    if (PROF && !stamps) return THR_OK;
#define THR_QS_LAUNCH(DIM, SHAPE)                                                                 \
    return launch_lds(dense_scan_f16qs<DIM, MODE, SHAPE>, grid, dim3(QS_NW * 64),                 \
                      QStag<DIM>::LDS_BYTES, st, (const f32x4*)rows16, (const f32x4*)qfrag,       \
                      n_qtiles, n_row_tiles, tile_stride, tau, seg_cnt, cand, CAND_CAP / nseg,    \
                      sample, sample_ld, doc_coll, query_coll, n_queries);
    if (stag) {
        if (dim == 512 && shape == 32) THR_QS_LAUNCH(512, 32)
        if (dim == 512) THR_QS_LAUNCH(512, 16)
        if (shape == 32) THR_QS_LAUNCH(768, 32)
        THR_QS_LAUNCH(768, 16)
    }
#undef THR_QS_LAUNCH
#define THR_Q_LAUNCH(DIM, SHAPE)                                                                  \
    return launch_lds(dense_scan_f16q<DIM, MODE, PROF, SHAPE>, grid, dim3(Q_NW * 64),             \
                      QScan<DIM>::LDS_BYTES, st, (const f32x4*)rows16, (const f32x4*)qfrag,       \
                      n_qtiles, n_row_tiles, tile_stride, tau, seg_cnt, cand, CAND_CAP / nseg,    \
                      sample, sample_ld, doc_coll, query_coll, n_queries, stamps);
    switch (dim) {
        case 512: if (shape == 16) THR_Q_LAUNCH(512, 16) THR_Q_LAUNCH(512, 32)
        case 768: if (shape == 16) THR_Q_LAUNCH(768, 16) THR_Q_LAUNCH(768, 32)
        case 1024:
            if (shape == 16 && qreg_qw(dim) == 48) THR_Q_LAUNCH(1024, 48)
            if (shape == 16) THR_Q_LAUNCH(1024, 16)
            THR_Q_LAUNCH(1024, 32)
        default: return THR_ERR_UNSUPPORTED;
    }
#undef THR_Q_LAUNCH
}

int launch_pack_queries(int dim, const float* queries, int n_queries, int qpad,
                               _Float16* qfrag, float* qerr, hipStream_t st) {
    const dim3 grid((unsigned)(qpad / 32));
    const bool s16 = qreg_shape(dim) == 16;
#define THR_PACK(DIM, SHAPE) \
    hipLaunchKernelGGL((pack_queries_f16<DIM, SHAPE>), grid, dim3(256), 0, st, queries, n_queries, (f32x4*)qfrag, qerr)
    switch (dim) {
        case 512: if (s16) THR_PACK(512, 16); else THR_PACK(512, 32); break;
        case 768: if (s16) THR_PACK(768, 16); else THR_PACK(768, 32); break;
        case 1024: if (s16) THR_PACK(1024, 16); else THR_PACK(1024, 32); break;
        default: return THR_ERR_UNSUPPORTED;
    }
#undef THR_PACK
    return launch_status();
}

int launch_quantize_f16(const float* docs, int64_t n_docs, int dim, _Float16* docs16,
                        unsigned int* max_rel_err, hipStream_t st) {
    if (docs16) {
        THR_RETURN_IF(dim % 16 != 0, THR_ERR_UNSUPPORTED);
        const int64_t n_pad = (n_docs + 31) / 32 * 32;
        hipLaunchKernelGGL(quantize_f16_norm, dim3((unsigned)((n_pad + 3) / 4)), dim3(256), 0, st,
                           docs, n_docs, dim, qreg_shape(dim), docs16, max_rel_err);
        return launch_status();
    }
    hipLaunchKernelGGL(measure_f16_error, dim3((unsigned)((n_docs + 3) / 4)), dim3(256), 0, st, docs,
                       n_docs, dim, max_rel_err);
    return launch_status();
}

#define THR_INSTANTIATE(MODE, PROF)                                                                    \
    template int launch_scan_f16q<MODE, PROF>(int, const _Float16*, const _Float16*, int, int64_t, int64_t, \
                                              const float*, int*, Cand*, float*, int64_t, hipStream_t, int*, \
                                              const int32_t*, const int32_t*, int, unsigned long long*, int*);
THR_INSTANTIATE(MODE_ALL, false)
THR_INSTANTIATE(MODE_FILTER, false)
THR_INSTANTIATE(MODE_FILTER, true)
#undef THR_INSTANTIATE

}
```

triple-hybrid-rag_amd/csrc/dense_scan_f16q.hpp:

```cpp
#pragma once
#include "dense_common.hpp"

namespace thr {

constexpr int Q_RING = 4;
constexpr int Q_NW = 4;

template <int DIM>
struct QScan {
    static constexpr int KS = DIM / 16;
    static constexpr int HS = KS / 2;
    static constexpr int HALF_BYTES = HS * 1024;
    static constexpr int PER_CU = DIM <= 768 ? 2 : 1;
    static constexpr int NB = (160 * 1024 / PER_CU) / HALF_BYTES > 4 ? 4 : (160 * 1024 / PER_CU) / HALF_BYTES;
    static constexpr int PER = HS / Q_NW;
#ifndef THR_Q_RING_1024
#define THR_Q_RING_1024 8
#endif
    static constexpr int RING = PER_CU == 1 ? THR_Q_RING_1024 : Q_RING;
#ifdef Q_PROBE_EXTRA
    static constexpr int VM_PER_PIECE = 2, LDS_BYTES = NB * HALF_BYTES + 32 * 1024;
#else
    static constexpr int VM_PER_PIECE = 1, LDS_BYTES = NB * HALF_BYTES;
#endif
    static_assert(HS % Q_NW == 0 && NB >= 3, "half tile must split evenly over the waves; >= 3 buffers");
};

template <int DIM, int SHAPE>
__global__ __launch_bounds__(256) void pack_queries_f16(const float* __restrict__ queries,
                                                        int n_queries, f32x4* __restrict__ qfrag,
                                                        float* __restrict__ qerr) {
    constexpr int KS = DIM / 16;
    const int lane = threadIdx.x & 63, wave = threadIdx.x >> 6;
    __shared__ double red[4][4][32];
    double e = 0.0, nn = 0.0, e_hi = 0.0, n_hi = 0.0;
#pragma unroll 4
    for (int s = wave; s < KS; s += 4) {
        int q, d0;
        if constexpr (SHAPE == 32) {
            q = blockIdx.x * 32 + (lane & 31);
            d0 = 16 * s + 8 * (lane >> 5);
        } else {
            q = blockIdx.x * 32 + 16 * (s / (KS / 2)) + (lane & 15);
            d0 = 32 * (s % (KS / 2)) + 8 * (lane >> 4);
        }
        f32x4 lo = {0.f, 0.f, 0.f, 0.f}, hi = lo;
        if (q < n_queries) {
            const f32x4* src = reinterpret_cast<const f32x4*>(queries + (int64_t)q * DIM + d0);
            lo = src[0];
            hi = src[1];
        }
        const f32x4 packed = pack_f16x8(lo, hi);
        qfrag[((int64_t)blockIdx.x * KS + s) * 64 + lane] = packed;
        const half8 hv = __builtin_bit_cast(half8, packed);
        double e1 = 0.0, n1 = 0.0;
#pragma unroll
        for (int j = 0; j < 8; ++j) {
            const float v = j < 4 ? lo[j] : hi[j - 4];
            const double d = (double)v - (double)(float)hv[j];
            e1 += d * d;
            n1 += (double)v * (double)v;
        }
        if (SHAPE == 32 || s < KS / 2) {
            e += e1;
            nn += n1;
        } else {
            e_hi += e1;
            n_hi += n1;
        }
    }
    if constexpr (SHAPE == 32) {
        e += __shfl_xor(e, 32, WAVE);
        nn += __shfl_xor(nn, 32, WAVE);
        if (lane < 32) {
            red[wave][0][lane] = e;
            red[wave][1][lane] = nn;
        }
    } else {
#pragma unroll
        for (int m = 16; m <= 32; m <<= 1) {
            e += __shfl_xor(e, m, WAVE);
            nn += __shfl_xor(nn, m, WAVE);
            e_hi += __shfl_xor(e_hi, m, WAVE);
            n_hi += __shfl_xor(n_hi, m, WAVE);
        }
        if (lane < 16) {
            red[wave][0][lane] = e;
            red[wave][1][lane] = nn;
            red[wave][0][16 + lane] = e_hi;
            red[wave][1][16 + lane] = n_hi;
        }
    }
    __syncthreads();
    if (threadIdx.x < 32) {
        double es = 0.0, ns = 0.0;
#pragma unroll
        for (int w = 0; w < 4; ++w) {
            es += red[w][0][threadIdx.x];
            ns += red[w][1][threadIdx.x];
        }
        const float rel = ns > 0.0 ? (float)sqrt(es / ns) : 0.f;
        qerr[blockIdx.x * 32 + threadIdx.x] = __uint_as_float(__float_as_uint(rel) + 1u);
    }
}

#define QS_RD(dst, ks) \
    asm volatile("ds_read_b128 %0, %1 offset:%2" : "=v"(dst) : "v"(abase), "n"((ks) * 1024) : "memory")
template <int S, int HS, int RING>
__device__ __forceinline__ void qs_fill(f32x4 (&a)[RING], uint32_t abase) {
    if constexpr (S < RING && S < HS) {
        QS_RD(a[S], S);
        qs_fill<S + 1, HS>(a, abase);
    }
}
template <int SHAPE>
struct QAcc;
template <>
struct QAcc<32> {
    static constexpr int NQL = 1, SEGS = 2;
    static constexpr int QW = 32, NQB = 2, NREG = 16;
    f32x16 v;
    __device__ __forceinline__ void zero() {
#pragma unroll
        for (int x = 0; x < 16; ++x) v[x] = 0.f;
    }
    template <int X> __device__ __forceinline__ float get() const { return v[X]; }
    template <int X> static __device__ __forceinline__ int row(int lane) { return (X & 3) + 8 * (X >> 2) + 4 * (lane >> 5); }
    template <int X> static constexpr int qsel() { return 0; }
    static __device__ __forceinline__ int query(int lane, int) { return lane & 31; }
    static __device__ __forceinline__ int seg(int lane) { return lane >> 5; }
};
template <>
struct QAcc<48> {
    static constexpr int NQL = 3, SEGS = 4;
    static constexpr int QW = 48, NQB = 3, NREG = 24;
    f32x4 t[6];
    __device__ __forceinline__ void zero() {
#pragma unroll
        for (int x = 0; x < 6; ++x) t[x] = f32x4{0.f, 0.f, 0.f, 0.f};
    }
    template <int X> __device__ __forceinline__ float get() const { return t[X >> 2][X & 3]; }
    template <int X> static __device__ __forceinline__ int row(int lane) { return 16 * ((X >> 2) / 3) + 4 * (lane >> 4) + (X & 3); }
    template <int X> static constexpr int qsel() { return (X >> 2) % 3; }
    static __device__ __forceinline__ int query(int lane, int qb) { return 16 * qb + (lane & 15); }
    static __device__ __forceinline__ int seg(int lane) { return lane >> 4; }
};
template <>
struct QAcc<16> {
    static constexpr int NQL = 2, SEGS = 4;
    static constexpr int QW = 32, NQB = 2, NREG = 16;
    f32x4 t[4];
    __device__ __forceinline__ void zero() {
#pragma unroll
        for (int x = 0; x < 4; ++x) t[x] = f32x4{0.f, 0.f, 0.f, 0.f};
    }
    template <int X> __device__ __forceinline__ float get() const { return t[X >> 2][X & 3]; }
    template <int X> static __device__ __forceinline__ int row(int lane) { return 16 * (X >> 3) + 4 * (lane >> 4) + (X & 3); }
    template <int X> static constexpr int qsel() { return (X >> 2) & 1; }
    static __device__ __forceinline__ int query(int lane, int qb) { return 16 * qb + (lane & 15); }
    static __device__ __forceinline__ int seg(int lane) { return lane >> 4; }
};

template <int S, int K0, int KS, int SHAPE, int NBQ>
__device__ __forceinline__ void qsx_mfma(const f32x4& a, const f32x4 (&bq)[NBQ], QAcc<SHAPE>& acc) {
    if constexpr (SHAPE == 32) {
        acc.v = __builtin_amdgcn_mfma_f32_32x32x16_f16(__builtin_bit_cast(half8, a),
                                                       __builtin_bit_cast(half8, bq[K0 + S]), acc.v, 0, 0, 0);
    } else {
        constexpr int k32 = (K0 + S) / 2, ra = S & 1, NQB = QAcc<SHAPE>::NQB;
        static_assert(NBQ == NQB * KS / 2, "one B fragment per 16-query block and 32-dim step");
        static_for<0, NQB>([&](auto qb) {
            acc.t[NQB * ra + qb] = __builtin_amdgcn_mfma_f32_16x16x32_f16(
                __builtin_bit_cast(half8, a), __builtin_bit_cast(half8, bq[qb * (KS / 2) + k32]),
                acc.t[NQB * ra + qb], 0, 0, 0);
        });
    }
}
template <int S, int HS, int K0, int KS, int PER, int SHAPE, int RING, int NBQ, typename Issue>
__device__ __forceinline__ void qsx_steps(f32x4 (&a)[RING], const f32x4 (&bq)[NBQ], QAcc<SHAPE>& acc,
                                          uint32_t abase, Issue& issue_piece) {
    if constexpr (S < HS) {
        constexpr int left = HS - S - 1 < RING - 1 ? HS - S - 1 : RING - 1;
        asm volatile("s_waitcnt lgkmcnt(%1)" : "+v"(a[S % RING]) : "n"(left) : "memory");
        qsx_mfma<S, K0, KS, SHAPE>(a[S % RING], bq, acc);
        if constexpr (S + RING < HS) QS_RD(a[S % RING], S + RING);
        constexpr int every = HS / PER;
        if constexpr (S % every == 1 && S / every < PER) issue_piece(std::integral_constant<int, S / every>{});
        qsx_steps<S + 1, HS, K0, KS, PER, SHAPE, RING, NBQ>(a, bq, acc, abase, issue_piece);
    }
}

template <int SHAPE>
struct QEmit {
    static constexpr int NQL = QAcc<SHAPE>::NQL;
    const Cand* cand;
    const int32_t* doc_coll;
    float tau[NQL];
    int qc[NQL];
    uint32_t slot[NQL], end[NQL];
    template <int X>
    __device__ __forceinline__ void one(const QAcc<SHAPE>& acc, uint32_t row0, int lane) {
        constexpr int qs = QAcc<SHAPE>::template qsel<X>();
        const float v = acc.template get<X>();
        if (v >= tau[qs]) {
            const uint32_t row = row0 + (uint32_t)QAcc<SHAPE>::template row<X>(lane);
            if (qc[qs] != -1 && doc_coll[row] != qc[qs]) return;
            if (slot[qs] < end[qs]) {
                const uint64_t word = (uint64_t)__float_as_uint(v) | ((uint64_t)row << 32);
                asm volatile("global_store_dwordx2 %0, %1, %2" ::"v"(slot[qs]), "v"(word), "s"(cand) : "memory");
            }
            slot[qs] += 8;
        }
    }
    template <int X>
    __device__ __forceinline__ void all(const QAcc<SHAPE>& acc, uint32_t row0, int lane) {
        if constexpr (X < QAcc<SHAPE>::NREG) {
            one<X>(acc, row0, lane);
            all<X + 1>(acc, row0, lane);
        }
    }
};

template <int S, int HS, int K0, int KS, int PER, int SHAPE, int HF, int RING, int NBQ, typename Issue>
__device__ __forceinline__ void qsx_steps_pe(f32x4 (&a)[RING], const f32x4 (&bq)[NBQ], QAcc<SHAPE>& acc,
                                             uint32_t abase, Issue& issue_piece, QEmit<SHAPE>& em,
                                             const QAcc<SHAPE>& prv, uint32_t row_prv, int lane) {
    if constexpr (S < HS) {
        constexpr int left = HS - S - 1 < RING - 1 ? HS - S - 1 : RING - 1;
        asm volatile("s_waitcnt lgkmcnt(%1)" : "+v"(a[S % RING]) : "n"(left) : "memory");
        qsx_mfma<S, K0, KS, SHAPE>(a[S % RING], bq, acc);
        if constexpr (S + RING < HS) QS_RD(a[S % RING], S + RING);
        constexpr int every = HS / PER;
        if constexpr (S % every == 1 && S / every < PER) issue_piece(std::integral_constant<int, S / every>{});
        constexpr int NRH = QAcc<SHAPE>::NREG / 2, j = S * NRH / HS;
        if constexpr ((S + 1) * NRH / HS > j) em.template one<NRH * HF + j>(prv, row_prv, lane);
        qsx_steps_pe<S + 1, HS, K0, KS, PER, SHAPE, HF, RING, NBQ>(a, bq, acc, abase, issue_piece, em, prv, row_prv, lane);
    }
}
#undef QS_RD

template <int DIM, int MODE, bool PROF = false, int SHAPE = 32>
__global__ __launch_bounds__(Q_NW * 64, QScan<DIM>::PER_CU) void dense_scan_f16q(
    const f32x4* __restrict__ packed, const f32x4* __restrict__ qfrag, int n_qtiles,
    int64_t n_tiles, int64_t tile_stride, const float* __restrict__ tau,
    int* __restrict__ seg_cnt, Cand* __restrict__ cand, int seg_cap,
    float* __restrict__ sample_scores, int64_t sample_ld,
    const int32_t* __restrict__ doc_coll, const int32_t* __restrict__ query_coll, int n_queries,
    unsigned long long* __restrict__ stamps = nullptr) {
    using C = QScan<DIM>;
    using A = QAcc<SHAPE>;
    constexpr int KS = C::KS, HS = C::HS, NB = C::NB, PER = C::PER, NQL = A::NQL, QW = A::QW;
    constexpr int NBQ = SHAPE == 32 ? KS : A::NQB * KS / 2;
    extern __shared__ f32x4 lds_rows[];

    const ScanSlot slot = scan_slot(n_qtiles);
    const int lane = threadIdx.x & 63;
    const int wave = __builtin_amdgcn_readfirstlane(threadIdx.x >> 6);
    const int q32 = slot.qtile * Q_NW + wave;
    const bool idle = (int64_t)q32 * QW >= n_queries;

    f32x4 bq[NBQ];
    if (!idle)
        static_for<0, NBQ>([&](auto s) {
            bq[s] = qfrag[((int64_t)q32 * NBQ + s) * 64 + lane];
        });
    const int nseg = A::SEGS * slot.nslices;
    const int my_seg = A::SEGS * slot.slice + A::seg(lane);
    QEmit<SHAPE> em;
    em.cand = cand;
    em.doc_coll = doc_coll;
    uint32_t start[NQL];
#pragma unroll
    for (int u = 0; u < NQL; ++u) {
        const int q = q32 * QW + A::query(lane, u);
        em.tau[u] = MODE == MODE_FILTER ? tau[q] : 0.f;
        em.qc[u] = (MODE == MODE_FILTER && query_coll && q < n_queries) ? query_coll[q] : -1;
        start[u] = (uint32_t)(((int64_t)q * CAND_CAP + (int64_t)my_seg * seg_cap) * sizeof(Cand));
        em.slot[u] = start[u];
        em.end[u] = start[u] + (uint32_t)(seg_cap * sizeof(Cand));
    }
    __builtin_amdgcn_s_waitcnt(0x0F70);

    const int64_t first = slot.slice, step = slot.nslices;
    const int64_t n_mine = first < n_tiles ? (n_tiles - first + step - 1) / step : 0;
    const int64_t n_half = 2 * n_mine;
    const uint32_t lds_base = (uint32_t)(size_t)(__attribute__((address_space(3))) void*)lds_rows;
    auto piece_src = [&](int64_t j) -> const f32x4* {
        const int64_t jc = j < n_half ? j : n_half - 1;
        const int64_t t = first + (jc >> 1) * step;
        return packed + ((t * tile_stride * KS + (jc & 1) * HS + wave) * 64 + lane);
    };
#ifdef Q_PROBE_EXTRA
    f32x4 probe_reg = {0.f, 0.f, 0.f, 0.f};
#endif
    auto dma = [&](const f32x4* src, int buf, int p) {
        __builtin_amdgcn_global_load_lds(
            (const __attribute__((address_space(1))) void*)(src + p * Q_NW * 64),
            (__attribute__((address_space(3))) void*)(size_t)(lds_base + buf * C::HALF_BYTES +
                                                              (wave + p * Q_NW) * 1024),
            16, 0, 0);
#ifdef Q_PROBE_EXTRA
        const uint32_t scratch = lds_base + NB * C::HALF_BYTES + (wave + (p & 7) * Q_NW) * 1024;
        if constexpr (Q_PROBE_EXTRA == 1) {
            __builtin_amdgcn_global_load_lds(
                (const __attribute__((address_space(1))) void*)(src + p * Q_NW * 64),
                (__attribute__((address_space(3))) void*)(size_t)scratch, 16, 0, 0);
        } else {
            asm volatile("ds_write_b128 %0, %1" ::"v"(scratch + lane * 16), "v"(probe_reg) : "memory");
            asm volatile("global_load_dwordx4 %0, %1, off" : "=v"(probe_reg) : "v"(src + p * Q_NW * 64) : "memory");
        }
#endif
    };
    if (n_half > 0) {
#pragma unroll
        for (int b = 0; b < NB - 1; ++b) {
            const f32x4* src = piece_src(b);
#pragma unroll
            for (int p = 0; p < PER; ++p) dma(src, b, p);
        }
    }

    unsigned long long ph[5] = {0, 0, 0, 0, 0}, t_loop = 0, t_prev = 0;
    auto stamp = [&](int j) {
        if constexpr (PROF) {
            const unsigned long long t = __builtin_amdgcn_s_memtime();
            if (j >= 0) ph[j] += t - t_prev;
            t_prev = t;
        }
    };
    if constexpr (PROF) t_loop = __builtin_amdgcn_s_memtime();

    A acc;
    int buf = 0;
    if (idle) {
#pragma unroll 1
        for (int64_t j = 0; j < n_half; ++j) {
            asm volatile("s_waitcnt vmcnt(%0)" ::"n"((NB - 2) * PER * C::VM_PER_PIECE) : "memory");
            __builtin_amdgcn_s_barrier();
            const int nbuf = buf == 0 ? NB - 1 : buf - 1;
            const f32x4* src = piece_src(j + NB - 1);
#pragma unroll
            for (int p = 0; p < PER; ++p) dma(src, nbuf, p);
            buf = buf + 1 == NB ? 0 : buf + 1;
        }
    }
#ifdef Q_NO_PIPE_EMIT
    constexpr bool PIPE_EMIT = false;
#else
    constexpr bool PIPE_EMIT = true;
#endif
    if constexpr (PIPE_EMIT && MODE == MODE_FILTER && !PROF && C::PER_CU == 1 && SHAPE != 48) {
        A acc2[2];
#pragma unroll
        for (int x = 0; x < A::NREG; ++x) {
            if constexpr (SHAPE == 32) acc2[1].v[x] = -INFINITY;
            else acc2[1].t[x >> 2][x & 3] = -INFINITY;
        }
        uint32_t row_of[2] = {0u, 0u};
#define QS_HALF_PE(hf, CUR, PRV)                                                                   \
    {                                                                                              \
        asm volatile("s_waitcnt vmcnt(%0)" ::"n"((NB - 2) * PER * C::VM_PER_PIECE) : "memory");                      \
        __builtin_amdgcn_s_barrier();                                                              \
        const int nbuf = buf == 0 ? NB - 1 : buf - 1;                  \
        const f32x4* src = piece_src(2 * i + (hf) + NB - 1);                                       \
        auto issue_piece = [&](auto P) { dma(src, nbuf, decltype(P)::value); };                    \
        const uint32_t abase = lds_base + buf * C::HALF_BYTES + lane * 16;                         \
        f32x4 a[C::RING];                                                                           \
        qs_fill<0, HS>(a, abase);                                                                  \
        qsx_steps_pe<0, HS, (hf) * HS, KS, PER, SHAPE, (hf)>(a, bq, acc2[CUR], abase, issue_piece, \
                                                            em, acc2[PRV], row_of[PRV], lane);     \
        buf = buf + 1 == NB ? 0 : buf + 1;                                                         \
    }
        const int64_t n_it = idle ? 0 : n_mine;
        int64_t i = 0;
#pragma unroll 1
        for (; i + 1 < n_it; i += 2) {
            acc2[0].zero();
            QS_HALF_PE(0, 0, 1)
            QS_HALF_PE(1, 0, 1)
            row_of[0] = (uint32_t)((first + i * step) * tile_stride * 32);
            ++i;
            acc2[1].zero();
            QS_HALF_PE(0, 1, 0)
            QS_HALF_PE(1, 1, 0)
            row_of[1] = (uint32_t)((first + i * step) * tile_stride * 32);
            --i;
        }
        if (i < n_it) {
            acc2[0].zero();
            QS_HALF_PE(0, 0, 1)
            QS_HALF_PE(1, 0, 1)
            em.template all<0>(acc2[0], (uint32_t)((first + i * step) * tile_stride * 32), lane);
        } else if (n_it > 0) {
            em.template all<0>(acc2[1], row_of[1], lane);
        }
#undef QS_HALF_PE
    } else {
#pragma unroll 1
    for (int64_t i = 0; i < (idle ? 0 : n_mine); ++i) {
#define QS_HALF(hf)                                                                                \
    {                                                                                              \
        stamp(-1);                                                                                 \
               \
        asm volatile("s_waitcnt vmcnt(%0)" ::"n"((NB - 2) * PER * C::VM_PER_PIECE) : "memory");                      \
        stamp(0);                                                                                  \
        __builtin_amdgcn_s_barrier();                                                              \
        stamp(1);                                                                                  \
        const int nbuf = buf == 0 ? NB - 1 : buf - 1;                  \
        const f32x4* src = piece_src(2 * i + (hf) + NB - 1);                                       \
        auto issue_piece = [&](auto P) { dma(src, nbuf, decltype(P)::value); };                    \
        const uint32_t abase = lds_base + buf * C::HALF_BYTES + lane * 16;                         \
        f32x4 a[C::RING];                                                                           \
        qs_fill<0, HS>(a, abase);                                                                  \
        stamp(2);                                                                                  \
        qsx_steps<0, HS, (hf) * HS, KS, PER, SHAPE>(a, bq, acc, abase, issue_piece);                \
        if constexpr (PROF) {                                                                      \
            if constexpr (SHAPE == 32) asm volatile("" : "+v"(acc.v));                               \
            else {                                                                                 \
                asm volatile("" : "+v"(acc.t[0]), "+v"(acc.t[1]), "+v"(acc.t[2]), "+v"(acc.t[3]));   \
                if constexpr (A::NQB == 3) asm volatile("" : "+v"(acc.t[4]), "+v"(acc.t[5]));       \
            }                                                                                      \
        }                                                                                          \
        stamp(3);                                                                                  \
        buf = buf + 1 == NB ? 0 : buf + 1;                                                         \
    }
        acc.zero();
        QS_HALF(0)
        QS_HALF(1)
#undef QS_HALF

        const int64_t t = first + i * step;
        if constexpr (MODE == MODE_ALL) {
            if constexpr (SHAPE == 32) {
                float* dst = sample_scores + (int64_t)(q32 * 32 + (lane & 31)) * sample_ld + t * 32 + 4 * (lane >> 5);
#pragma unroll
                for (int g = 0; g < 4; ++g) {
                    f32x4 v;
#pragma unroll
                    for (int j = 0; j < 4; ++j) {
                        const float sv = acc.v[4 * g + j];
                        v[j] = sv == sv ? sv : -INFINITY;
                    }
                    *reinterpret_cast<f32x4*>(dst + 8 * g) = v;
                }
            } else {
#pragma unroll
                for (int x = 0; x < 2 * A::NQB; ++x) {
                    f32x4 v = acc.t[x];
#pragma unroll
                    for (int j = 0; j < 4; ++j) v[j] = v[j] == v[j] ? v[j] : -INFINITY;
                    float* dst = sample_scores + (int64_t)(q32 * QW + 16 * (x % A::NQB) + (lane & 15)) * sample_ld +
                                 t * 32 + 16 * (x / A::NQB) + 4 * (lane >> 4);
                    *reinterpret_cast<f32x4*>(dst) = v;
                }
            }
        } else {
            em.template all<0>(acc, (uint32_t)(t * tile_stride * 32), lane);
        }
        stamp(4);
    }
    }
    asm volatile("s_waitcnt vmcnt(0)" ::: "memory");
    if constexpr (MODE == MODE_FILTER) {
#pragma unroll
        for (int u = 0; u < NQL; ++u)
            seg_cnt[(int64_t)(q32 * QW + A::query(lane, u)) * nseg + my_seg] = (int)((em.slot[u] - start[u]) / sizeof(Cand));
    }
    if constexpr (PROF) {
        if (lane == 0) {
            unsigned long long* o = stamps + ((int64_t)blockIdx.x * Q_NW + wave) * 8;
            for (int j = 0; j < 5; ++j) o[j] = ph[j];
            o[5] = (unsigned long long)n_half;
            o[6] = __builtin_amdgcn_s_memtime() - t_loop;
            o[7] = (unsigned long long)__builtin_amdgcn_s_getreg((4 << 0) | (0 << 6) | (31 << 11));
        }
    }
}

constexpr int QS_NW = 8;
constexpr int QS_NBUF = 6;

template <int DIM>
struct QStag {
    static constexpr int KS = DIM / 16, HS = KS / 2, HALF_BYTES = HS * 1024;
    static constexpr int PER = HS / QS_NW;
    static constexpr int LDS_BYTES = QS_NBUF * HALF_BYTES;
    static_assert(HS % QS_NW == 0 && LDS_BYTES <= 160 * 1024, "dim 512 / 768 only");
};

template <int DIM, int MODE, int SHAPE = 32>
__global__ __launch_bounds__(QS_NW * 64) void dense_scan_f16qs(
    const f32x4* __restrict__ packed, const f32x4* __restrict__ qfrag, int n_qtiles,
    int64_t n_tiles, int64_t tile_stride, const float* __restrict__ tau,
    int* __restrict__ seg_cnt, Cand* __restrict__ cand, int seg_cap,
    float* __restrict__ sample_scores, int64_t sample_ld,
    const int32_t* __restrict__ doc_coll, const int32_t* __restrict__ query_coll, int n_queries) {
    using C = QStag<DIM>;
    using A = QAcc<SHAPE>;
    constexpr int KS = C::KS, HS = C::HS, PER = C::PER, NBUF = QS_NBUF, NQL = A::NQL;
    extern __shared__ f32x4 lds_rows[];

    const ScanSlot slot = scan_slot(n_qtiles);
    const int lane = threadIdx.x & 63;
    const int wave = __builtin_amdgcn_readfirstlane(threadIdx.x >> 6);
    const int q32 = slot.qtile * QS_NW + wave;

    f32x4 bq[KS];
    if ((int64_t)q32 * 32 < n_queries)
        static_for<0, KS>([&](auto s) {
            bq[s] = qfrag[((int64_t)q32 * KS + s) * 64 + lane];
        });
    const int nseg = A::SEGS * slot.nslices;
    const int my_seg = A::SEGS * slot.slice + A::seg(lane);
    QEmit<SHAPE> em;
    em.cand = cand;
    em.doc_coll = doc_coll;
    uint32_t start[NQL];
#pragma unroll
    for (int u = 0; u < NQL; ++u) {
        const int q = q32 * 32 + A::query(lane, u);
        em.tau[u] = MODE == MODE_FILTER ? tau[q] : 0.f;
        em.qc[u] = (MODE == MODE_FILTER && query_coll && q < n_queries) ? query_coll[q] : -1;
        start[u] = (uint32_t)(((int64_t)q * CAND_CAP + (int64_t)my_seg * seg_cap) * sizeof(Cand));
        em.slot[u] = start[u];
        em.end[u] = start[u] + (uint32_t)(seg_cap * sizeof(Cand));
    }
    __builtin_amdgcn_s_waitcnt(0x0F70);

    const int64_t first = slot.slice, step = slot.nslices;
    const int64_t n_mine = first < n_tiles ? (n_tiles - first + step - 1) / step : 0;
    const int64_t n_half = 2 * n_mine;
    const uint32_t lds_base = (uint32_t)(size_t)(__attribute__((address_space(3))) void*)lds_rows;
    auto piece_src = [&](int64_t j) -> const f32x4* {
        const int64_t jc = j < n_half ? j : n_half - 1;
        const int64_t t = first + (jc >> 1) * step;
        return packed + ((t * tile_stride * KS + (jc & 1) * HS + wave) * 64 + lane);
    };
    auto dma = [&](const f32x4* src, int buf, int p) {
        __builtin_amdgcn_global_load_lds(
            (const __attribute__((address_space(1))) void*)(src + p * QS_NW * 64),
            (__attribute__((address_space(3))) void*)(size_t)(lds_base + buf * C::HALF_BYTES +
                                                              (wave + p * QS_NW) * 1024),
            16, 0, 0);
    };
    auto emit_all = [&](const A& acc, int64_t i) {
        const int64_t t = first + i * step;
        if constexpr (SHAPE == 32) {
            float* dst = sample_scores + (int64_t)(q32 * 32 + (lane & 31)) * sample_ld + t * 32 + 4 * (lane >> 5);
#pragma unroll
            for (int g = 0; g < 4; ++g) {
                f32x4 v;
#pragma unroll
                for (int j = 0; j < 4; ++j) {
                    const float sv = acc.v[4 * g + j];
                    v[j] = sv == sv ? sv : -INFINITY;
                }
                *reinterpret_cast<f32x4*>(dst + 8 * g) = v;
            }
        } else {
#pragma unroll
            for (int x = 0; x < 4; ++x) {
                f32x4 v = acc.t[x];
#pragma unroll
                for (int j = 0; j < 4; ++j) v[j] = v[j] == v[j] ? v[j] : -INFINITY;
                float* dst = sample_scores + (int64_t)(q32 * 32 + 16 * (x & 1) + (lane & 15)) * sample_ld +
                             t * 32 + 16 * (x >> 1) + 4 * (lane >> 4);
                *reinterpret_cast<f32x4*>(dst) = v;
            }
        }
    };
#define QS_EMIT(i_)                                                                                \
    if constexpr (MODE == MODE_ALL) {                                                              \
        emit_all(acc, (i_));                                                                       \
    } else {                                                                                       \
        em.template all<0>(acc, (uint32_t)((first + (i_) * step) * tile_stride * 32), lane);       \
    }
#define QS_SYNC()                                                      \
    asm volatile("s_waitcnt vmcnt(%0)" ::"n"(3 * PER) : "memory");     \
    __builtin_amdgcn_s_barrier();

    if (n_half > 0) {
#pragma unroll
        for (int b = 0; b < 4; ++b) {
            const f32x4* src = piece_src(b);
#pragma unroll
            for (int p = 0; p < PER; ++p) dma(src, b, p);
        }
    }
    A acc;
    f32x4 a[Q_RING];
    if ((int64_t)q32 * 32 >= n_queries) {
        int buf = wave < 4 ? 4 : 5;
        int64_t j = wave < 4 ? 4 : 5;
        if (wave >= 4) {
            QS_SYNC()
            if (n_half > 0) {
                const f32x4* src = piece_src(4);
#pragma unroll
                for (int p = 0; p < PER; ++p) dma(src, 4, p);
            }
        }
#pragma unroll 1
        for (int64_t k = 0; k < n_half; ++k, ++j) {
            QS_SYNC()
            const f32x4* src = piece_src(j);
#pragma unroll
            for (int p = 0; p < PER; ++p) dma(src, buf, p);
            buf = buf + 1 == NBUF ? 0 : buf + 1;
        }
        if (wave < 4) {
            QS_SYNC()
        }
    } else if (wave < 4) {
        int buf = 0;
#pragma unroll 1
        for (int64_t i = 0; i < n_mine; ++i) {
            {
                QS_SYNC()
                const int nbuf = buf + 4 >= NBUF ? buf + 4 - NBUF : buf + 4;
                const f32x4* src = piece_src(2 * i + 4);
                auto issue_piece = [&](auto P) { dma(src, nbuf, decltype(P)::value); };
                const uint32_t abase = lds_base + buf * C::HALF_BYTES + lane * 16;
                qs_fill<0, HS>(a, abase);
                acc.zero();
                qsx_steps<0, HS, 0, KS, PER, SHAPE>(a, bq, acc, abase, issue_piece);
                buf = buf + 1 == NBUF ? 0 : buf + 1;
            }
            {
                QS_SYNC()
                const int nbuf = buf + 4 >= NBUF ? buf + 4 - NBUF : buf + 4;
                const f32x4* src = piece_src(2 * i + 5);
                auto issue_piece = [&](auto P) { dma(src, nbuf, decltype(P)::value); };
                const uint32_t abase = lds_base + buf * C::HALF_BYTES + lane * 16;
                qs_fill<0, HS>(a, abase);
                qsx_steps<0, HS, HS, KS, PER, SHAPE>(a, bq, acc, abase, issue_piece);
                buf = buf + 1 == NBUF ? 0 : buf + 1;
            }
            QS_EMIT(i)
        }
        QS_SYNC()
    } else {
        QS_SYNC()
        if (n_half > 0) {
            const f32x4* src = piece_src(4);
#pragma unroll
            for (int p = 0; p < PER; ++p) dma(src, 4, p);
        }
        int buf = 0;
#pragma unroll 1
        for (int64_t i = 0; i < n_mine; ++i) {
            const int buf1 = buf + 1 == NBUF ? 0 : buf + 1;
            const int buf2 = buf1 + 1 == NBUF ? 0 : buf1 + 1;
            {
                QS_SYNC()
                if (i > 0) {
                    QS_EMIT(i - 1)
                }
                const int nbuf = buf + 5 >= NBUF ? buf + 5 - NBUF : buf + 5;
                const f32x4* src = piece_src(2 * i + 5);
                auto issue_piece = [&](auto P) { dma(src, nbuf, decltype(P)::value); };
                const uint32_t abase = lds_base + buf * C::HALF_BYTES + lane * 16;
                if (i == 0) qs_fill<0, HS>(a, abase);
                acc.zero();
                qsx_steps<0, HS, 0, KS, PER, SHAPE>(a, bq, acc, abase, issue_piece);
                qs_fill<0, HS>(a, lds_base + buf1 * C::HALF_BYTES + lane * 16);
            }
            {
                QS_SYNC()
                const f32x4* src = piece_src(2 * i + 6);
                auto issue_piece = [&](auto P) { dma(src, buf, decltype(P)::value); };
                const uint32_t abase = lds_base + buf1 * C::HALF_BYTES + lane * 16;
                qsx_steps<0, HS, HS, KS, PER, SHAPE>(a, bq, acc, abase, issue_piece);
                if (i + 1 < n_mine)
                    qs_fill<0, HS>(a, lds_base + buf2 * C::HALF_BYTES + lane * 16);
            }
            buf = buf2;
        }
        if (n_mine > 0) {
            QS_EMIT(n_mine - 1)
        }
    }
#undef QS_SYNC
#undef QS_EMIT
    asm volatile("s_waitcnt vmcnt(0)" ::: "memory");
    if constexpr (MODE == MODE_FILTER) {
#pragma unroll
        for (int u = 0; u < NQL; ++u)
            seg_cnt[(int64_t)(q32 * 32 + A::query(lane, u)) * nseg + my_seg] = (int)((em.slot[u] - start[u]) / sizeof(Cand));
    }
}

__global__ __launch_bounds__(256) void quantize_f16_norm(const float* __restrict__ docs,
                                                         int64_t n_docs, int dim, int shape,
                                                         _Float16* __restrict__ packed,
                                                         unsigned int* __restrict__ max_err_bits) {
    const int lane = threadIdx.x & 63;
    const int64_t row = (int64_t)blockIdx.x * (blockDim.x / WAVE) + (threadIdx.x >> 6);
    const int64_t n_pad = (n_docs + 31) / 32 * 32;
    if (row >= n_pad) return;
    const int64_t tile = row >> 5;
    const int r = (int)(row & 31), ks = dim / 16;
    const float* x = docs + row * dim;
    double nn = 0.0;
    if (row < n_docs)
        for (int i = lane; i < dim; i += WAVE) nn += (double)x[i] * (double)x[i];
    for (int m = 32; m >= 1; m >>= 1) nn += __shfl_xor(nn, m, WAVE);
    const double dn = sqrt(nn);
    const bool live = dn > 0.0;
    double err = 0.0;
    for (int i = lane; i < dim; i += WAVE) {
        const float v = live ? x[i] : 0.f;
        const _Float16 hv = live ? (_Float16)(float)((double)v / dn) : (_Float16)__builtin_nanf("");
        if (packed) {
            if (shape == 32) {
                const int s = i >> 4, hh = (i >> 3) & 1, e = i & 7;
                packed[(((tile * ks + s) * 64) + r + 32 * hh) * 8 + e] = hv;
            } else {
                const int k32 = i >> 5, g = (i >> 3) & 3, e = i & 7, ra = r >> 4;
                packed[(((tile * ks + 2 * k32 + ra) * 64) + (r & 15) + 16 * g) * 8 + e] = hv;
            }
        }
        if (live) {
            const double d = (double)v / dn - (double)(float)hv;
            err += d * d;
        }
    }
    for (int m = 32; m >= 1; m >>= 1) err += __shfl_xor(err, m, WAVE);
    if (lane == 0 && live) {
        float rel = (float)sqrt(err);
        rel = __uint_as_float(__float_as_uint(rel) + 1u);
        atomicMax(max_err_bits, __float_as_uint(rel));
    }
}

__global__ __launch_bounds__(256) void measure_f16_error(const float* __restrict__ docs, int64_t n_docs,
                                                         int dim, unsigned int* __restrict__ max_rel_bits) {
    const int lane = threadIdx.x & 63;
    const int64_t row = (int64_t)blockIdx.x * (blockDim.x / WAVE) + (threadIdx.x >> 6);
    if (row >= n_docs) return;
    const float* x = docs + row * dim;
    double err = 0.0, nrm = 0.0;
    for (int i = lane; i < dim; i += WAVE) {
        const float v = x[i];
        const double d = (double)v - (double)(float)(_Float16)v;
        err += d * d;
        nrm += (double)v * (double)v;
    }
    for (int m = 32; m >= 1; m >>= 1) {
        err += __shfl_xor(err, m, WAVE);
        nrm += __shfl_xor(nrm, m, WAVE);
    }
    if (lane == 0 && nrm > 0.0) {
        float rel = (float)sqrt(err / nrm);
        rel = __uint_as_float(__float_as_uint(rel) + 1u);
        atomicMax(max_rel_bits, __float_as_uint(rel));
    }
}

}
```

triple-hybrid-rag_amd/csrc/dense_select.hip:

```cpp
#include "dense_common.hpp"

namespace thr {

constexpr int BUCKET_BLOCKS = 32;
__global__ __launch_bounds__(256) void bucket_candidates(const int* __restrict__ tile_cnt,
                                                         const Cand* __restrict__ tile_list,
                                                         int tile_cap, int qtile, int row_bits,
                                                         int* __restrict__ cand_cnt,
                                                         Cand* __restrict__ cand) {
    __shared__ int count[128], base[128], fill[128];
    const uint32_t row_mask = (1u << row_bits) - 1u;
    const int tile = blockIdx.y;
    int n = tile_cnt[tile];
    n = n < tile_cap ? n : tile_cap;
    const int per = (n + gridDim.x - 1) / gridDim.x;
    const int lo = blockIdx.x * per, hi = lo + per < n ? lo + per : n;
    const Cand* list = tile_list + (int64_t)tile * tile_cap;
    if (threadIdx.x < 128) count[threadIdx.x] = fill[threadIdx.x] = 0;
    __syncthreads();
    for (int i = lo + threadIdx.x; i < hi; i += blockDim.x)
        atomicAdd(&count[list[i].doc >> row_bits], 1);
    __syncthreads();
    if (threadIdx.x < qtile && count[threadIdx.x] > 0)
        base[threadIdx.x] = atomicAdd(&cand_cnt[tile * qtile + threadIdx.x], count[threadIdx.x]);
    __syncthreads();
    for (int i = lo + threadIdx.x; i < hi; i += blockDim.x) {
        const Cand e = list[i];
        const int ql = (int)(e.doc >> row_bits);
        const int p = base[ql] + atomicAdd(&fill[ql], 1);
        if (p < CAND_CAP)
            cand[(int64_t)(tile * qtile + ql) * CAND_CAP + p] = Cand{e.score, e.doc & row_mask};
    }
}

template <typename KeyFn>
__device__ uint32_t block_radix_select_local(KeyFn keyfn, int my_n, int kk, int* hist, int* bc) {
    uint32_t prefix = 0, mask = 0;
    int remaining = kk;
    for (int shift = 24; shift >= 0; shift -= 8) {
        for (int i = threadIdx.x; i < 256; i += blockDim.x) hist[i] = 0;
        __syncthreads();
        for (int u0 = 0; u0 < my_n; u0 += 8) {
            uint32_t key[8];
#pragma unroll
            for (int u = 0; u < 8; ++u) key[u] = u0 + u < my_n ? keyfn(u0 + u) : 0u;
#pragma unroll
            for (int u = 0; u < 8; ++u)
                if (u0 + u < my_n && (key[u] & mask) == prefix) atomicAdd(&hist[(key[u] >> shift) & 255], 1);
        }
        __syncthreads();
        if (threadIdx.x == 0) {
            int cum = 0, b = 255;
            for (; b > 0; --b) {
                if (cum + hist[b] >= remaining) break;
                cum += hist[b];
            }
            bc[0] = b;
            bc[1] = cum;
        }
        __syncthreads();
        remaining -= bc[1];
        prefix |= (uint32_t)bc[0] << shift;
        mask |= 255u << shift;
        __syncthreads();
    }
    return prefix;
}

__device__ __forceinline__ void coarse_find_bin(const int* hist, int remaining, int* aux) {
    const int t = threadIdx.x, lane = t & 63, w = t >> 6;
    const int top = CS_BINS - 16 * t;
    int mine = 0;
#pragma unroll
    for (int b = 1; b <= 16; ++b) mine += hist[top - b];
    int incl = mine;
#pragma unroll
    for (int o = 1; o < 64; o <<= 1) {
        const int v = __shfl_up(incl, o, WAVE);
        if (lane >= o) incl += v;
    }
    if (lane == 63) aux[4 + w] = incl;
    if (t == 0) aux[0] = 0, aux[1] = -1;
    __syncthreads();
    int before = 0;
    for (int x = 0; x < w; ++x) before += aux[4 + x];
    incl += before;
    const int excl = incl - mine;
    if (excl < remaining && remaining <= incl) {
        int cum = excl, b = top - 1;
        for (; b > top - 16; --b) {
            if (cum + hist[b] >= remaining) break;
            cum += hist[b];
        }
        aux[0] = b;
        aux[1] = cum;
    }
    __syncthreads();
    if (aux[1] < 0) {
        if (t == 255) aux[0] = 0, aux[1] = incl - hist[0];
        __syncthreads();
    }
}

template <typename KeyFn>
__device__ uint32_t block_coarse_select(KeyFn keyfn, int n, int kk, int* hist, int* aux) {
    uint32_t prefix = 0;
    int remaining = kk;
#pragma unroll 1
    for (int pass = 0; pass < 2; ++pass) {
        for (int i = threadIdx.x; i < CS_BINS; i += 256) hist[i] = 0;
        __syncthreads();
        for (int base = threadIdx.x; base < n; base += 8 * 256) {
            uint32_t key[8];
#pragma unroll
            for (int u = 0; u < 8; ++u) {
                const int i = base + u * 256;
                key[u] = i < n ? keyfn(i) : 0u;
            }
#pragma unroll
            for (int u = 0; u < 8; ++u) {
                const int i = base + u * 256;
                if (i >= n) continue;
                if (pass == 0) atomicAdd(&hist[key[u] >> 20], 1);
                else if ((key[u] >> 20) == (prefix >> 20)) atomicAdd(&hist[(key[u] >> 8) & 4095], 1);
            }
        }
        __syncthreads();
        coarse_find_bin(hist, remaining, aux);
        remaining -= aux[1];
        prefix |= (uint32_t)aux[0] << (pass == 0 ? 20 : 8);
        __syncthreads();
    }
    return prefix;
}
__device__ __forceinline__ float coarse_value(uint32_t key) {
    const float v = fkey_inv(key);
    return v == v ? v : -INFINITY;
}

__device__ bool query_is_void(const float* __restrict__ queries, int n_queries, int dim, int q,
                              int* flag) {
    if (threadIdx.x == 0) *flag = 0;
    __syncthreads();
    if (q < n_queries) {
        int nz = 0;
        for (int i = threadIdx.x; i < dim; i += blockDim.x) nz |= queries[(int64_t)q * dim + i] != 0.f;
        if (nz) *flag = 1;
    }
    __syncthreads();
    return *flag == 0;
}

__global__ __launch_bounds__(256) void kth_select(const float* __restrict__ sample_scores,
                                                  int64_t sample_ld, int n_sample, int kk,
                                                  const float* __restrict__ queries, int n_queries,
                                                  int dim, float* __restrict__ tau,
                                                  float* __restrict__ qerr,
                                                  const int32_t* __restrict__ doc_coll,
                                                  const int32_t* __restrict__ query_coll, int unit,
                                                  int64_t stride, int64_t n_docs) {
    __shared__ int hist[CS_BINS];
    __shared__ int aux[8];
    __shared__ int flag;
    __shared__ double red[2][256];
    const int q = blockIdx.x;
    if (qerr) {
        double e = 0.0, nn = 0.0;
        if (q < n_queries)
            for (int i = threadIdx.x; i < dim; i += blockDim.x) {
                const float v = queries[(int64_t)q * dim + i];
                const double dd = (double)v - (double)(float)(_Float16)v;
                e += dd * dd;
                nn += (double)v * (double)v;
            }
        red[0][threadIdx.x] = e;
        red[1][threadIdx.x] = nn;
        __syncthreads();
        for (int o = 128; o > 0; o >>= 1) {
            if (threadIdx.x < o) {
                red[0][threadIdx.x] += red[0][threadIdx.x + o];
                red[1][threadIdx.x] += red[1][threadIdx.x + o];
            }
            __syncthreads();
        }
        if (threadIdx.x == 0) {
            float rel = red[1][0] > 0.0 ? (float)sqrt(red[0][0] / red[1][0]) : 0.f;
            qerr[q] = __uint_as_float(__float_as_uint(rel) + 1u);
        }
    }
    if (query_is_void(queries, n_queries, dim, q, &flag)) {
        if (threadIdx.x == 0) tau[q] = INFINITY;
        return;
    }
    if (n_sample < kk) {
        if (threadIdx.x == 0) tau[q] = -INFINITY;
        return;
    }
    const float* s = sample_scores + (int64_t)q * sample_ld;
    const int qc = (query_coll && q < n_queries) ? query_coll[q] : -1;
    auto val = [&](int i) {
        float v = s[i];
        if (qc != -1) {
            const int64_t row = (int64_t)(i / unit) * stride * unit + i % unit;
            if (row >= n_docs || doc_coll[row] != qc) v = -INFINITY;
        }
        return v;
    };
    __shared__ float kred[4];
    __shared__ int kcnt;
    const int lane = threadIdx.x & 63, wave = threadIdx.x >> 6;
    auto sweep = [&](auto&& fn) {
        for (int base = threadIdx.x; base < n_sample; base += 8 * 256) {
            float v[8];
#pragma unroll
            for (int u = 0; u < 8; ++u) v[u] = base + u * 256 < n_sample ? val(base + u * 256) : -INFINITY;
#pragma unroll
            for (int u = 0; u < 8; ++u) fn(v[u]);
        }
    };
    float m = -INFINITY;
    sweep([&](float v) { m = fmaxf(m, v); });
#pragma unroll
    for (int o = 32; o > 0; o >>= 1) m = fmaxf(m, __shfl_xor(m, o, WAVE));
    if (lane == 0) kred[wave] = m;
    if (threadIdx.x == 0) kcnt = 0;
    for (int i = threadIdx.x; i < CS_BINS; i += 256) hist[i] = 0;
    __syncthreads();
    m = fmaxf(fmaxf(kred[0], kred[1]), fmaxf(kred[2], kred[3]));
    if (m > 0.f && m < INFINITY) {
        const float thr = 0.5f * m, scale = 4095.f / (m - thr);
        int c = 0;
        sweep([&](float v) {
            if (v >= thr) {
                const int bn = (int)((v - thr) * scale);
                atomicAdd(&hist[bn > CS_BINS - 1 ? CS_BINS - 1 : bn], 1);
                ++c;
            }
        });
#pragma unroll
        for (int o = 32; o > 0; o >>= 1) c += __shfl_xor(c, o, WAVE);
        if (lane == 0 && c) atomicAdd(&kcnt, c);
        __syncthreads();
        if (kcnt >= kk) {
            coarse_find_bin(hist, kk, aux);
            if (threadIdx.x == 0) tau[q] = thr + (float)aux[0] / scale;
            return;
        }
        __syncthreads();
    }
    const uint32_t key = block_coarse_select([&](int i) { return fkey(val(i)); }, n_sample, kk, hist, aux);
    if (threadIdx.x == 0) tau[q] = coarse_value(key);
}

constexpr int SEL_THREADS = 256;
constexpr int SEL_REG = 16;
constexpr int SEL_FLAT = 8192;
static size_t band_lds_bytes(int dim) { return sizeof(float) * dim + sizeof(int) * CS_BINS; }
constexpr int CAPB = SEL_BIG_BAND;
template <bool TOPM>
__global__ __launch_bounds__(SEL_THREADS, 4) void select_band(
    int dim, const float* __restrict__ queries, const float* __restrict__ tau,
    const int* __restrict__ cand_cnt, const Cand* __restrict__ cand,
    const int* __restrict__ tile_cnt, int tile_cap, int qtile, int k, int kprime, double eps32,
    double doc_relerr, const float* __restrict__ qerr, int nseg, int seg_cap,
    const int32_t* __restrict__ doc_coll, const int32_t* __restrict__ query_coll,
    int32_t* __restrict__ sel_rows, int32_t* __restrict__ sel_meta,
    const float* __restrict__ gfloor, const float* __restrict__ lb_all, int n_shards, int lb_m,
    float* __restrict__ top_lb, int top_m) {
    extern __shared__ float4 lds_sel[];
    __shared__ int aux[8];
    __shared__ int bc[4];
    __shared__ int32_t s_id[CAPB];
    __shared__ int n_sel;
    __shared__ double wsum[4];
    float* lds_qv = reinterpret_cast<float*>(lds_sel);
    int* hist = reinterpret_cast<int*>(lds_sel + dim / 4);

    const int q = blockIdx.x;
    const int lane = threadIdx.x & 63, wave = threadIdx.x >> 6;
    const double eq = qerr ? (double)qerr[q] : 0.0;
    const double eps = eps32 + doc_relerr * (1.0 + eq) + eq;
    const Cand* c = cand + (int64_t)q * CAND_CAP;
    const Cand* my_ptr = c + threadIdx.x;
    int my_n, my_c[4] = {0, 0, 0, 0};
    bool overflow, flat = true;
    int n;
    __shared__ unsigned short src_off[SEL_FLAT];
    if (nseg == 0) {
        const int cnt = cand_cnt[q];
        overflow = cnt > CAND_CAP || tile_cnt[q / qtile] > tile_cap;
        n = cnt < CAND_CAP ? cnt : CAND_CAP;
        my_n = n > (int)threadIdx.x ? (n - (int)threadIdx.x + SEL_THREADS - 1) / SEL_THREADS : 0;
    } else {
        __shared__ int wtot[4];
        bool over = false;
        int tot = 0;
#pragma unroll
        for (int x = 0; x < 4; ++x) {
            const int sg = (int)threadIdx.x + x * SEL_THREADS;
            int sc = sg < nseg ? cand_cnt[(int64_t)q * nseg + sg] : 0;
            over |= sc > seg_cap;
            my_c[x] = sc < seg_cap ? sc : seg_cap;
            tot += my_c[x];
        }
        int incl = tot;
#pragma unroll
        for (int o = 1; o < 64; o <<= 1) {
            const int v = __shfl_up(incl, o, WAVE);
            if (lane >= o) incl += v;
        }
        if (lane == 63) wtot[wave] = incl;
        overflow = __syncthreads_or(over) != 0;
        int base = incl - tot;
        for (int x = 0; x < wave; ++x) base += wtot[x];
        n = wtot[0] + wtot[1] + wtot[2] + wtot[3];
        flat = n <= SEL_FLAT;
        if (flat) {
#pragma unroll
            for (int x = 0; x < 4; ++x) {
                const int first = ((int)threadIdx.x + x * SEL_THREADS) * seg_cap;
                for (int j = 0; j < my_c[x]; ++j) src_off[base + j] = (unsigned short)(first + j);
                base += my_c[x];
            }
            __syncthreads();
            my_n = n > (int)threadIdx.x ? (n - (int)threadIdx.x + SEL_THREADS - 1) / SEL_THREADS : 0;
        } else {
            my_n = tot;
        }
    }
    auto cand_at = [&](int u) -> Cand {
        if (nseg == 0) return my_ptr[(int64_t)u * SEL_THREADS];
        if (flat) return c[src_off[(int)threadIdx.x + u * SEL_THREADS]];
        int sg = threadIdx.x;
#pragma unroll
        for (int x = 0; x < 3; ++x)
            if (u >= my_c[x]) {
                u -= my_c[x];
                sg += SEL_THREADS;
            } else {
                break;
            }
        return c[(int64_t)sg * seg_cap + u];
    };

    const int qc = query_coll ? query_coll[q] : -1;
    auto load_cand = [&](int u) -> Cand {
        Cand e = cand_at(u);
        if (qc != -1 && doc_coll[e.doc] != qc) e.score = -INFINITY;
        return e;
    };
    Cand mine[SEL_REG];
#pragma unroll
    for (int u = 0; u < SEL_REG; ++u) mine[u] = u < my_n ? load_cand(u) : Cand{-INFINITY, 0u};
    if (qc != -1) {
        __shared__ int n_pass;
        if (threadIdx.x == 0) n_pass = 0;
        __syncthreads();
        int mine_ok = 0;
#pragma unroll
        for (int u = 0; u < SEL_REG; ++u) mine_ok += (u < my_n && mine[u].score > -INFINITY) ? 1 : 0;
        for (int u = SEL_REG; u < my_n; ++u) mine_ok += load_cand(u).score > -INFINITY ? 1 : 0;
        if (mine_ok) atomicAdd(&n_pass, mine_ok);
        __syncthreads();
        n = n_pass;
    }
    for (int i = threadIdx.x; i < dim / 4; i += SEL_THREADS)
        lds_sel[i] = reinterpret_cast<const float4*>(queries + (int64_t)q * dim)[i];
    if (threadIdx.x == 0) n_sel = 0;
    __syncthreads();

    {
        double part = 0.0;
        for (int i = threadIdx.x; i < dim; i += SEL_THREADS) part += (double)lds_qv[i] * (double)lds_qv[i];
        for (int o = 32; o > 0; o >>= 1) part += __shfl_xor(part, o, WAVE);
        if (lane == 0) wsum[wave] = part;
        __syncthreads();
    }
    const double qn_hi = sqrt(wsum[0] + wsum[1] + wsum[2] + wsum[3]) * (1.0 + 1e-6);

    float gF = -INFINITY;
    if (!TOPM) {
        if (gfloor) {
            gF = gfloor[q];
        } else if (lb_all && n_shards * lb_m >= k) {
            __shared__ float s_gF;
            float* fv = reinterpret_cast<float*>(hist);
            const int nv = n_shards * lb_m, nv4 = (nv + 3) & ~3;
            for (int i = threadIdx.x; i < nv4; i += SEL_THREADS)
                fv[i] = i < nv ? lb_all[((int64_t)(i / lb_m) * gridDim.x + q) * lb_m + i % lb_m] : -INFINITY;
            if (threadIdx.x == 0) s_gF = -INFINITY;
            __syncthreads();
            const f32x4* fv4 = reinterpret_cast<const f32x4*>(fv);
            for (int i = threadIdx.x; i < nv; i += SEL_THREADS) {
                const float v = fv[i];
                if (!(v > -INFINITY)) continue;
                int rank = 0;
#pragma unroll 4
                for (int j = 0; j < nv4; j += 4) {
                    const f32x4 w = fv4[j >> 2];
                    rank += (w.x > v || (w.x == v && j < i)) ? 1 : 0;
                    rank += (w.y > v || (w.y == v && j + 1 < i)) ? 1 : 0;
                    rank += (w.z > v || (w.z == v && j + 2 < i)) ? 1 : 0;
                    rank += (w.w > v || (w.w == v && j + 3 < i)) ? 1 : 0;
                }
                if (rank == k - 1) s_gF = v;
            }
            __syncthreads();
            gF = s_gF;
            __syncthreads();
        }
    }
    float band_lo = -INFINITY;
    if (gF > -INFINITY) band_lo = nextafterf((float)((double)gF - 1.5 * eps * qn_hi), -INFINITY);
    float floor32 = tau[q];
    bool band_done = false;
    const int kk = TOPM ? top_m : k;
    float a_kk = -INFINITY;
    if (n > kk) {
        __shared__ float fred[3][4];
        float lo = INFINITY, hi = -INFINITY;
#pragma unroll
        for (int u = 0; u < SEL_REG; ++u)
            if (u < my_n && mine[u].score > -INFINITY) {
                lo = fminf(lo, mine[u].score);
                hi = fmaxf(hi, mine[u].score);
            }
        for (int u = SEL_REG; u < my_n; ++u) {
            const float sc = load_cand(u).score;
            if (sc > -INFINITY) {
                lo = fminf(lo, sc);
                hi = fmaxf(hi, sc);
            }
        }
#pragma unroll
        for (int o = 32; o > 0; o >>= 1) {
            lo = fminf(lo, __shfl_xor(lo, o, WAVE));
            hi = fmaxf(hi, __shfl_xor(hi, o, WAVE));
        }
        if (lane == 0) fred[0][wave] = lo, fred[1][wave] = hi;
        for (int i = threadIdx.x; i < CS_BINS; i += SEL_THREADS) hist[i] = 0;
        __syncthreads();
        lo = fminf(fminf(fred[0][0], fred[0][1]), fminf(fred[0][2], fred[0][3]));
        hi = fmaxf(fmaxf(fred[1][0], fred[1][1]), fmaxf(fred[1][2], fred[1][3]));
        const float scale = hi - lo > 1e-30f ? 4095.f / (hi - lo) : 0.f;
        auto bin_of = [&](float sc) {
            const int bn = (int)((sc - lo) * scale);
            return bn > CS_BINS - 1 ? CS_BINS - 1 : bn;
        };
#pragma unroll
        for (int u = 0; u < SEL_REG; ++u)
            if (u < my_n && mine[u].score > -INFINITY) atomicAdd(&hist[bin_of(mine[u].score)], 1);
        for (int u = SEL_REG; u < my_n; ++u) {
            const float sc = load_cand(u).score;
            if (sc > -INFINITY) atomicAdd(&hist[bin_of(sc)], 1);
        }
        __syncthreads();
        coarse_find_bin(hist, kk, aux);
        const int kbin = aux[0];
        float a_k = INFINITY;
#pragma unroll
        for (int u = 0; u < SEL_REG; ++u)
            if (u < my_n && mine[u].score > -INFINITY && bin_of(mine[u].score) >= kbin)
                a_k = fminf(a_k, mine[u].score);
        for (int u = SEL_REG; u < my_n; ++u) {
            const float sc = load_cand(u).score;
            if (sc > -INFINITY && bin_of(sc) >= kbin) a_k = fminf(a_k, sc);
        }
#pragma unroll
        for (int o = 32; o > 0; o >>= 1) a_k = fminf(a_k, __shfl_xor(a_k, o, WAVE));
        if (lane == 0) fred[2][wave] = a_k;
        __syncthreads();
        a_k = fminf(fminf(fred[2][0], fred[2][1]), fminf(fred[2][2], fred[2][3]));
        a_kk = a_k;
        const float band = (float)((double)a_k - 2.5 * eps * qn_hi);
        band_lo = fmaxf(band_lo, nextafterf(band, -INFINITY));
    }
    if (TOPM) {
        float* o = top_lb + (int64_t)q * top_m;
        float* vals = reinterpret_cast<float*>(s_id);
        const double drop = eps * qn_hi;
        auto lowered = [&](float sc) { return nextafterf((float)((double)sc - drop), -INFINITY); };
        for (int i = threadIdx.x; i < top_m; i += SEL_THREADS) o[i] = -INFINITY;
        for (int u = 0; u < my_n; ++u) {
            const float sc = load_cand(u).score;
            if (sc > -INFINITY && sc >= a_kk) {
                const int p = atomicAdd(&n_sel, 1);
                if (p < CAPB) vals[p] = sc;
            }
        }
        __syncthreads();
        const int c = n_sel;
        if (c <= CAPB) {
            for (int i = threadIdx.x; i < c; i += SEL_THREADS) {
                const float v = vals[i];
                int rank = 0;
                for (int j = 0; j < c; ++j) {
                    const float w = vals[j];
                    rank += (w > v || (w == v && j < i)) ? 1 : 0;
                }
                if (rank < top_m) o[rank] = lowered(v);
            }
            return;
        }
        __syncthreads();
        if (threadIdx.x == 0) n_sel = 0;
        __syncthreads();
        const uint32_t tkey = block_radix_select_local(
            [&](int u) { return fkey(load_cand(u).score); }, my_n, top_m, hist, bc);
        for (int u = 0; u < my_n; ++u) {
            const Cand e = load_cand(u);
            if (fkey(e.score) > tkey) o[atomicAdd(&n_sel, 1)] = lowered(e.score);
        }
        __syncthreads();
        for (int u = 0; u < my_n; ++u) {
            const Cand e = load_cand(u);
            if (fkey(e.score) == tkey) {
                const int p = atomicAdd(&n_sel, 1);
                if (p < top_m) o[p] = lowered(e.score);
            }
        }
        return;
    }
    if (band_lo > -INFINITY) {
#pragma unroll
        for (int u = 0; u < SEL_REG; ++u) {
            const bool in = u < my_n && mine[u].score >= band_lo;
            const unsigned long long m = __ballot(in);
            if (m) {
                int base = 0;
                if (lane == 0) base = atomicAdd(&n_sel, __popcll(m));
                base = __shfl(base, 0, WAVE);
                const int p = base + __popcll(m & ((1ull << lane) - 1ull));
                if (in && p < CAPB) s_id[p] = mine[u].doc;
            }
        }
        for (int u = SEL_REG; u < my_n; ++u) {
            const Cand e = load_cand(u);
            if (e.score >= band_lo) {
                const int p = atomicAdd(&n_sel, 1);
                if (p < CAPB) s_id[p] = e.doc;
            }
        }
        __syncthreads();
        if (n_sel <= CAPB) {
            floor32 = fmaxf(floor32, band_lo);
            band_done = true;
        } else {
            __syncthreads();
            if (threadIdx.x == 0) n_sel = 0;
            __syncthreads();
        }
    }
    if (!band_done) {
        if (n > kprime) {
            const uint32_t tkey = block_radix_select_local(
                [&](int u) { return fkey(load_cand(u).score); }, my_n, kprime, hist, bc);
            floor32 = fkey_inv(tkey);
            for (int u = 0; u < my_n; ++u) {
                const Cand e = load_cand(u);
                if (fkey(e.score) > tkey) {
                    const int p = atomicAdd(&n_sel, 1);
                    s_id[p] = e.doc;
                }
            }
            __syncthreads();
            for (int u = 0; u < my_n; ++u) {
                const Cand e = load_cand(u);
                if (fkey(e.score) == tkey) {
                    const int p = atomicAdd(&n_sel, 1);
                    if (p < kprime) s_id[p] = e.doc;
                }
            }
            __syncthreads();
            if (threadIdx.x == 0 && n_sel > kprime) n_sel = kprime;
        } else {
            for (int u = 0; u < my_n; ++u) {
                const Cand e = load_cand(u);
                if (e.score > -INFINITY) {
                    const int p = atomicAdd(&n_sel, 1);
                    s_id[p] = e.doc;
                }
            }
        }
    }
    __syncthreads();
    const int ns = n_sel;
    for (int i = threadIdx.x; i < ns; i += SEL_THREADS) sel_rows[(int64_t)q * CAPB + i] = s_id[i];
    if (threadIdx.x == 0) {
        sel_meta[4 * q + 0] = ns;
        sel_meta[4 * q + 1] = (int32_t)__float_as_uint(floor32);
        sel_meta[4 * q + 2] = overflow ? 1 : 0;
        sel_meta[4 * q + 3] = (int32_t)__float_as_uint(gF);
    }
}

__global__ __launch_bounds__(256) void dense_floor_kernel(const float* __restrict__ lb, int n_shards,
                                                          int n_queries, int m, int k,
                                                          float* __restrict__ gfloor) {
    extern __shared__ float fl_v[];
    const int q = blockIdx.x, n = n_shards * m;
    for (int i = threadIdx.x; i < n; i += blockDim.x)
        fl_v[i] = lb[((int64_t)(i / m) * n_queries + q) * m + i % m];
    if (threadIdx.x == 0) gfloor[q] = -INFINITY;
    __syncthreads();
    if (n < k) return;
    for (int i = threadIdx.x; i < n; i += blockDim.x) {
        const float v = fl_v[i];
        if (!(v > -INFINITY)) continue;
        int rank = 0;
        for (int j = 0; j < n; ++j) {
            const float w = fl_v[j];
            rank += (w > v || (w == v && j < i)) ? 1 : 0;
        }
        if (rank == k - 1) gfloor[q] = v;
    }
}

int launch_threshold(const DensePlan& P, const DenseIndex& X, const DenseBatch& B) {
    hipLaunchKernelGGL(kth_select, dim3(P.qpad), dim3(256), 0, B.st,
                       P.sampled ? (const float*)P.sample : nullptr, P.sample_docs, (int)P.sample_docs,
                       P.ksample, B.queries, B.n_queries, X.dim, P.tau, P.packed ? nullptr : P.qerr,
                       X.doc_coll, B.query_coll, MF_ROWS, P.sampled ? P.sample_stride : (int64_t)1,
                       X.n_docs);
    return launch_status();
}

int launch_bucket(const DensePlan& P, hipStream_t st) {
    hipLaunchKernelGGL(bucket_candidates, dim3(BUCKET_BLOCKS, P.ntiles), dim3(256), 0, st, P.tcnt,
                       P.tlist, P.tile_cap, P.qtile, P.row_bits, P.cnt, P.cand);
    return launch_status();
}

int launch_band(const DensePlan& P, const DenseIndex& X, const DenseBatch& B, const DensePhase& S,
                int nseg) {
    const bool topm = S.phase == PIPE_SHORTLIST;
    hipLaunchKernelGGL(topm ? select_band<true> : select_band<false>, dim3(B.n_queries),
                       dim3(SEL_THREADS), band_lds_bytes(X.dim), B.st, X.dim, B.queries, P.tau, P.cnt,
                       P.cand, P.tcnt, P.tile_cap, P.qtile, B.k, B.kprime, scan_eps(X.dim),
                       X.doc_rel_err, P.qerr, nseg, nseg ? CAND_CAP / nseg : 0, X.doc_coll,
                       B.query_coll, P.sel_rows, P.sel_meta, S.gfloor, S.lb_all, S.n_shards,
                       topm ? 0 : S.top_m, S.top_lb, topm ? S.top_m : 0);
    return launch_status();
}

}

using namespace thr;

extern "C" int thr_dense_floor(const float* top_lb, int n_shards, int n_queries, int m, int k,
                               float* gfloor, thr_stream_t stream) {
    clear_status();
    THR_RETURN_IF(!top_lb || !gfloor || n_shards <= 0 || n_queries <= 0 || m <= 0 || k <= 0, THR_ERR_INVALID);
    THR_RETURN_IF((int64_t)n_shards * m > 8192, THR_ERR_CAPACITY);
    hipLaunchKernelGGL(dense_floor_kernel, dim3(n_queries), dim3(256), sizeof(float) * n_shards * m,
                       (hipStream_t)stream, top_lb, n_shards, n_queries, m, k, gfloor);
    return launch_status();
}
```

triple-hybrid-rag_amd/csrc/rrf.hip:

```cpp
#include "thr_common.hpp"

namespace thr {

constexpr int RRF_THREADS = 128;
constexpr int RRF_MAXC = THR_RRF_MAX_PER_CHANNEL;
constexpr int RRF_SLOTS = 512;

__device__ __forceinline__ int last_rank(const int64_t* l, int n, int64_t id) {
    int r = 0;
    for (int j = 0; j < n; ++j)
        if (l[j] == id) r = j + 1;
    return r;
}
__device__ __forceinline__ bool seen_before(const int64_t* l, int i, int64_t id) {
    for (int j = 0; j < i; ++j)
        if (l[j] == id) return true;
    return false;
}

constexpr int RRF_RAG2 = 0, RRF_STANDALONE = 1, RRF_TWO = 2;
__device__ __forceinline__ int occurrences(const int64_t* l, int n, int64_t id) {
    int c = 0;
    for (int j = 0; j < n; ++j) c += l[j] == id ? 1 : 0;
    return c;
}

template <int MODE>
__global__ __launch_bounds__(RRF_THREADS) void rrf_fuse_kernel(
    const int64_t* __restrict__ lex, int n_lex, const int64_t* __restrict__ sem, int n_sem,
    const int64_t* __restrict__ gra, int n_gra, double w_lex, double w_sem, double w_gra, int rrf_k,
    int top_k, int64_t* __restrict__ out_ids, double* __restrict__ out_scores,
    int32_t* __restrict__ out_ranks, int32_t* __restrict__ out_counts) {
    static_assert(RRF_THREADS == RRF_MAXC && RRF_THREADS == 2 * WAVE, "one thread per position");
    __shared__ int64_t L[3][RRF_MAXC];
    __shared__ int len[3];
    __shared__ int wave_new[3][2];
    __shared__ double s_s[RRF_SLOTS];
    __shared__ int64_t c_id[RRF_SLOTS];
    __shared__ int c_rank[RRF_SLOTS][3];
    __shared__ int order[RRF_SLOTS];

    const int q = blockIdx.x, t = threadIdx.x, lane = t & 63, wave = t >> 6;
    const int64_t* src[3] = {lex, sem, gra};
    const int width[3] = {lex ? n_lex : 0, sem ? n_sem : 0, gra ? n_gra : 0};
    if (t < 3) len[t] = width[t];
    __syncthreads();
    for (int ch = 0; ch < 3; ++ch) {
        const int64_t id = t < width[ch] ? src[ch][(int64_t)q * width[ch] + t] : -1;
        L[ch][t] = id;
        if (t < width[ch] && id < 0) atomicMin(&len[ch], t);
    }
    __syncthreads();

    bool nw[3];
    int within[3];
    for (int ch = 0; ch < 3; ++ch) {
        nw[ch] = false;
        if (t < len[ch]) {
            const int64_t id = L[ch][t];
            nw[ch] = !seen_before(L[ch], t, id);
            for (int e = 0; e < ch && nw[ch]; ++e)
                if (last_rank(L[e], len[e], id)) nw[ch] = false;
        }
        const uint64_t m = __ballot(nw[ch]);
        within[ch] = __popcll(m & ((1ull << lane) - 1ull));
        if (lane == 0) wave_new[ch][wave] = __popcll(m);
    }
    __syncthreads();
    int base = 0, n = 0;
    for (int ch = 0; ch < 3; ++ch) {
        const int here = base + (wave ? wave_new[ch][0] : 0) + within[ch];
        base += wave_new[ch][0] + wave_new[ch][1];
        if (!nw[ch]) continue;
        const int64_t id = L[ch][t];
        const int lr = last_rank(L[0], len[0], id);
        const int sr = last_rank(L[1], len[1], id);
        const int gr = last_rank(L[2], len[2], id);
        double score = 0.0;
        if (MODE == RRF_RAG2) {
            if (lr) score = __dadd_rn(score, __ddiv_rn(w_lex, (double)(rrf_k + lr)));
            if (sr) score = __dadd_rn(score, __ddiv_rn(w_sem, (double)(rrf_k + sr)));
            if (gr) score = __dadd_rn(score, __ddiv_rn(w_gra, (double)(rrf_k + gr)));
        } else {
            const double w[3] = {w_lex, w_sem, w_gra};
            const int rk[3] = {lr, sr, gr};
#pragma unroll
            for (int c = 0; c < 3; ++c)
                if (rk[c]) {
                    const double v = __dmul_rn(w[c], __ddiv_rn(1.0, (double)(rrf_k + rk[c])));
                    const int reps = (MODE == RRF_TWO && c == 0) ? 1 : occurrences(L[c], len[c], id);
                    for (int r = 0; r < reps; ++r) score = __dadd_rn(score, v);
                }
        }
        c_id[here] = id;
        c_rank[here][0] = lr;
        c_rank[here][1] = sr;
        c_rank[here][2] = gr;
        s_s[here] = score;
    }
    n = base;
    __syncthreads();
    for (int p = t; p < n; p += RRF_THREADS) {
        const double ms = s_s[p];
        int rank = 0;
        for (int j = 0; j < n; ++j) {
            const double o = s_s[j];
            rank += (o > ms || (o == ms && j < p)) ? 1 : 0;
        }
        order[rank] = p;
    }
    __syncthreads();
    for (int i = t; i < top_k; i += RRF_THREADS) {
        const bool ok = i < n;
        const int p = ok ? order[i] : 0;
        out_ids[(int64_t)q * top_k + i] = ok ? c_id[p] : -1;
        out_scores[(int64_t)q * top_k + i] = ok ? s_s[p] : -INFINITY;
        if (out_ranks)
            for (int c = 0; c < 3; ++c)
                out_ranks[((int64_t)q * top_k + i) * 3 + c] = ok ? c_rank[p][c] : 0;
    }
    if (t == 0) out_counts[q] = n < top_k ? n : top_k;
}

__global__ __launch_bounds__(RRF_THREADS) void rerank_order_kernel(
    const float* __restrict__ scores, int n_lists, int64_t list_stride,
    const int64_t* __restrict__ ids, const int32_t* __restrict__ counts, int n, int top_k,
    int64_t* __restrict__ out_ids, double* __restrict__ out_scores, int32_t* __restrict__ out_counts) {
    __shared__ double s_s[RRF_SLOTS];
    __shared__ int order[RRF_SLOTS];
    const int q = blockIdx.x, t = threadIdx.x;
    int cnt = counts ? counts[q] : n;
    cnt = cnt < n ? cnt : n;
    for (int p = t; p < cnt; p += RRF_THREADS) {
        float best = -INFINITY;
        for (int l = 0; l < n_lists; ++l) best = fmaxf(best, scores[(int64_t)l * list_stride + (int64_t)q * n + p]);
        s_s[p] = best > -INFINITY ? (double)best : 0.0;
    }
    __syncthreads();
    for (int p = t; p < cnt; p += RRF_THREADS) {
        const double ms = s_s[p];
        int rank = 0;
        for (int j = 0; j < cnt; ++j) {
            const double o = s_s[j];
            rank += (o > ms || (o == ms && j < p)) ? 1 : 0;
        }
        order[rank] = p;
    }
    __syncthreads();
    for (int i = t; i < top_k; i += RRF_THREADS) {
        const bool ok = i < cnt;
        const int p = ok ? order[i] : 0;
        out_ids[(int64_t)q * top_k + i] = ok ? ids[(int64_t)q * n + p] : -1;
        out_scores[(int64_t)q * top_k + i] = ok ? s_s[p] : -INFINITY;
    }
    if (t == 0) out_counts[q] = cnt < top_k ? cnt : top_k;
}

__global__ __launch_bounds__(RRF_THREADS) void fuse_post_kernel(
    const int64_t* __restrict__ ids, const double* __restrict__ scores,
    const int32_t* __restrict__ ranks, const int32_t* __restrict__ counts, int n,
    const double* __restrict__ lex_s, int n_lex, const double* __restrict__ sem_s, int n_sem,
    const double* __restrict__ gra_s, int n_gra, double safety_threshold, int denoise,
    double quantile, int normalize, int top_k, int64_t* __restrict__ out_ids,
    double* __restrict__ out_scores, int32_t* __restrict__ out_counts) {
    __shared__ double s_s[2][RRF_SLOTS];
    __shared__ int64_t s_id[2][RRF_SLOTS];
    __shared__ int wave_cnt[2];
    __shared__ double red[2][2];
    const int q = blockIdx.x, t = threadIdx.x, lane = t & 63, wave = t >> 6;
    int cnt = counts ? counts[q] : n;
    cnt = cnt < n ? cnt : n;
    auto compact = [&](int from, int m, auto keep) -> int {
        int base = 0;
        for (int b0 = 0; b0 < m; b0 += RRF_THREADS) {
            const int i = b0 + t;
            const bool k = i < m && keep(i);
            const uint64_t bal = __ballot(k);
            if (lane == 0) wave_cnt[wave] = __popcll(bal);
            __syncthreads();
            const int at = base + (wave ? wave_cnt[0] : 0) + __popcll(bal & ((1ull << lane) - 1ull));
            if (k) {
                s_s[from ^ 1][at] = s_s[from][i];
                s_id[from ^ 1][at] = s_id[from][i];
            }
            base += wave_cnt[0] + wave_cnt[1];
            __syncthreads();
        }
        return base;
    };
    const double* chs[3] = {lex_s, sem_s, gra_s};
    const int chw[3] = {n_lex, n_sem, n_gra};
    for (int i = t; i < cnt; i += RRF_THREADS) {
        s_s[0][i] = scores[(int64_t)q * n + i];
        s_id[0][i] = ids[(int64_t)q * n + i];
    }
    __syncthreads();
    int m = cnt, cur = 0;
    if (safety_threshold > 0.0 && ranks) {
        m = compact(0, cnt, [&](int i) {
            double best = 0.0;
            for (int c = 0; c < 3; ++c) {
                const int r = ranks[((int64_t)q * n + i) * 3 + c];
                if (r > 0 && chs[c]) {
                    const double v = chs[c][(int64_t)q * chw[c] + r - 1];
                    best = v > best ? v : best;
                }
            }
            return best >= safety_threshold;
        });
        cur = 1;
    }
    if (denoise && m >= 3) {
        const double v = __dmul_rn((double)(m - 1), quantile);
        int prev = (int)floor(v);
        prev = prev < 0 ? 0 : prev > m - 1 ? m - 1 : prev;
        const int next = prev + 1 > m - 1 ? m - 1 : prev + 1;
        const double g = __dsub_rn(v, (double)prev);
        const double a = s_s[cur][m - 1 - prev], bb = s_s[cur][m - 1 - next];
        const double diff = __dsub_rn(bb, a);
        const double cut = g >= 0.5 ? __dsub_rn(bb, __dmul_rn(diff, __dsub_rn(1.0, g)))
                                    : __dadd_rn(a, __dmul_rn(diff, g));
        __syncthreads();
        const int from = cur;
        m = compact(from, m, [&](int i) { return s_s[from][i] >= cut; });
        cur ^= 1;
    }
    if (top_k > 0 && m > top_k) m = top_k;
    double lo = 0.0, hi = 0.0;
    if (normalize && m > 0) {
        double mn = INFINITY, mx = -INFINITY;
        for (int i = t; i < m; i += RRF_THREADS) {
            const double v = s_s[cur][i];
            mn = v < mn ? v : mn;
            mx = v > mx ? v : mx;
        }
        for (int o = 32; o > 0; o >>= 1) {
            const double a = __shfl_xor(mn, o, WAVE), b2 = __shfl_xor(mx, o, WAVE);
            mn = a < mn ? a : mn;
            mx = b2 > mx ? b2 : mx;
        }
        if (lane == 0) {
            red[0][wave] = mn;
            red[1][wave] = mx;
        }
        __syncthreads();
        lo = red[0][0] < red[0][1] ? red[0][0] : red[0][1];
        hi = red[1][0] > red[1][1] ? red[1][0] : red[1][1];
    }
    for (int i = t; i < n; i += RRF_THREADS) {
        const bool ok = i < m;
        double v = ok ? s_s[cur][i] : -INFINITY;
        if (ok && normalize) v = hi == lo ? 1.0 : __ddiv_rn(__dsub_rn(v, lo), __dsub_rn(hi, lo));
        out_scores[(int64_t)q * n + i] = v;
        out_ids[(int64_t)q * n + i] = ok ? s_id[cur][i] : -1;
    }
    if (t == 0) out_counts[q] = m;
}

}

using namespace thr;

extern "C" int thr_rerank_order(const float* scores, int n_lists, int64_t list_stride,
                                const int64_t* ids, const int32_t* counts, int n_queries, int n,
                                int top_k, int64_t* out_ids, double* out_scores,
                                int32_t* out_counts, thr_stream_t stream) {
    clear_status();
    THR_RETURN_IF(!scores || !ids || !out_ids || !out_scores || !out_counts, THR_ERR_INVALID);
    THR_RETURN_IF(n_queries <= 0 || n_lists <= 0 || n <= 0 || n > RRF_SLOTS || top_k <= 0 || top_k > n,
                  THR_ERR_INVALID);
    if (list_stride == 0) list_stride = (int64_t)n_queries * n;
    THR_RETURN_IF(list_stride < (int64_t)n_queries * n, THR_ERR_INVALID);
    hipLaunchKernelGGL(rerank_order_kernel, dim3(n_queries), dim3(RRF_THREADS), 0, (hipStream_t)stream,
                       scores, n_lists, list_stride, ids, counts, n, top_k, out_ids, out_scores,
                       out_counts);
    return launch_status();
}

extern "C" int thr_rrf_fuse(const int64_t* lex_ids, int n_lex, const int64_t* sem_ids, int n_sem,
                            const int64_t* graph_ids, int n_graph, int n_queries, double w_lex,
                            double w_sem, double w_graph, int rrf_k, int top_k, int64_t* out_ids,
                            double* out_scores, int32_t* out_ranks, int32_t* out_counts,
                            thr_stream_t stream) {
    clear_status();
    THR_RETURN_IF(!out_ids || !out_scores || !out_counts, THR_ERR_INVALID);
    THR_RETURN_IF(n_queries <= 0 || top_k <= 0 || top_k > RRF_SLOTS || rrf_k < 0, THR_ERR_INVALID);
    THR_RETURN_IF(n_lex < 0 || n_sem < 0 || n_graph < 0 || n_lex > RRF_MAXC || n_sem > RRF_MAXC ||
                      n_graph > RRF_MAXC,
                  THR_ERR_INVALID);
    THR_RETURN_IF((!lex_ids || !n_lex) && (!sem_ids || !n_sem) && (!graph_ids || !n_graph),
                  THR_ERR_INVALID);
    hipLaunchKernelGGL(rrf_fuse_kernel<RRF_RAG2>, dim3(n_queries), dim3(RRF_THREADS), 0, (hipStream_t)stream,
                       n_lex ? lex_ids : nullptr, n_lex, n_sem ? sem_ids : nullptr, n_sem,
                       n_graph ? graph_ids : nullptr, n_graph, w_lex, w_sem, w_graph, rrf_k, top_k,
                       out_ids, out_scores, out_ranks, out_counts);
    return launch_status();
}

extern "C" int thr_rrf_fuse_standalone(const int64_t* lex_ids, int n_lex, const int64_t* sem_ids,
                                       int n_sem, const int64_t* graph_ids, int n_graph,
                                       int n_queries, double w_lex, double w_sem, double w_graph,
                                       int two_channels, int top_k, int64_t* out_ids,
                                       double* out_scores, int32_t* out_ranks, int32_t* out_counts,
                                       thr_stream_t stream) {
    clear_status();
    THR_RETURN_IF(!out_ids || !out_scores || !out_counts, THR_ERR_INVALID);
    THR_RETURN_IF(n_queries <= 0 || top_k <= 0 || top_k > RRF_SLOTS, THR_ERR_INVALID);
    THR_RETURN_IF(n_lex < 0 || n_sem < 0 || n_graph < 0 || n_lex > RRF_MAXC || n_sem > RRF_MAXC ||
                      n_graph > RRF_MAXC,
                  THR_ERR_INVALID);
    THR_RETURN_IF((!lex_ids || !n_lex) && (!sem_ids || !n_sem) && (!graph_ids || !n_graph),
                  THR_ERR_INVALID);
    THR_RETURN_IF(two_channels && graph_ids && n_graph, THR_ERR_INVALID);
    const int rrf_k = 60;
#define THR_RRF_LAUNCH(MODE)                                                                        \
    hipLaunchKernelGGL(rrf_fuse_kernel<MODE>, dim3(n_queries), dim3(RRF_THREADS), 0, (hipStream_t)stream, \
                       n_lex ? lex_ids : nullptr, n_lex, n_sem ? sem_ids : nullptr, n_sem,          \
                       n_graph ? graph_ids : nullptr, n_graph, w_lex, w_sem, w_graph, rrf_k, top_k, \
                       out_ids, out_scores, out_ranks, out_counts)
    if (two_channels) THR_RRF_LAUNCH(RRF_TWO);
    else THR_RRF_LAUNCH(RRF_STANDALONE);
#undef THR_RRF_LAUNCH
    return launch_status();
}

extern "C" int thr_fuse_post(const int64_t* ids, const double* scores, const int32_t* ranks,
                             const int32_t* counts, int n_queries, int n, const double* lex_scores,
                             int n_lex, const double* sem_scores, int n_sem,
                             const double* graph_scores, int n_graph, double safety_threshold,
                             int denoise, double quantile, int normalize, int top_k,
                             int64_t* out_ids, double* out_scores, int32_t* out_counts,
                             thr_stream_t stream) {
    clear_status();
    THR_RETURN_IF(!ids || !scores || !out_ids || !out_scores || !out_counts, THR_ERR_INVALID);
    THR_RETURN_IF(n_queries <= 0 || n <= 0 || n > RRF_SLOTS || top_k < 0, THR_ERR_INVALID);
    THR_RETURN_IF(safety_threshold > 0.0 && !ranks, THR_ERR_INVALID);
    THR_RETURN_IF(denoise && !(quantile >= 0.0 && quantile <= 1.0), THR_ERR_INVALID);
    THR_RETURN_IF(n_lex < 0 || n_sem < 0 || n_graph < 0, THR_ERR_INVALID);
    hipLaunchKernelGGL(fuse_post_kernel, dim3(n_queries), dim3(RRF_THREADS), 0, (hipStream_t)stream, ids,
                       scores, ranks, counts, n, lex_scores, n_lex, sem_scores, n_sem, graph_scores,
                       n_graph, safety_threshold, denoise, quantile, normalize, top_k, out_ids,
                       out_scores, out_counts);
    return launch_status();
}
```

Measured before the change: 717,900 queries/s.

## Keep per-segment top-4 in sample scan and radix-select threshold from it

The sampled threshold pass no longer writes every sampled score to global memory. Each wave keeps a register top-4 per query per segment and stores only those, and a new radix kth-select kernel reads that small buffer to set tau. The sampling aim drops so more docs are sampled, and the dense memset of counters is skipped for the packed path. The rescue counter is now zeroed inside the kernel instead of by a host-side zeros call, and RRF gains a single-channel fast path that avoids the general merge. These changes cut sample-buffer traffic, the selection cost and a few small launches, at the risk of a looser tau from a top-4-per-segment approximation, which would mean more candidates in the filter scan.

```diff
diff --git a/triple-hybrid-rag_amd/_native.py b/triple-hybrid-rag_amd/_native.py
--- a/triple-hybrid-rag_amd/_native.py
+++ b/triple-hybrid-rag_amd/_native.py
@@ -281,7 +281,7 @@
     need = int(load().thr_dense_rescue_workspace_bytes(nq, k))
     if workspace is None or workspace.numel() * workspace.element_size() < need:
         workspace = torch.empty(need, dtype=torch.uint8, device=docs.device)
-    n_rescued = torch.zeros(1, dtype=torch.int32, device=docs.device)
+    n_rescued = torch.empty(1, dtype=torch.int32, device=docs.device)
     pdc, pqc = _coll(doc_coll, query_coll, n, nq)
     _check(load().thr_dense_rescue(pd, pn, n, d, id_base, pq, nq, k, pdc, pqc, S.data_ptr(), I.data_ptr(),
                                    cnt.data_ptr(), flg.data_ptr(), n_rescued.data_ptr(),
diff --git a/triple-hybrid-rag_amd/csrc/dense.hip b/triple-hybrid-rag_amd/csrc/dense.hip
--- a/triple-hybrid-rag_amd/csrc/dense.hip
+++ b/triple-hybrid-rag_amd/csrc/dense.hip
@@ -4,10 +4,14 @@
 
 namespace thr {
 
+constexpr double QREG_AIM_1M = 1448.0;
+constexpr int QREG_KS = 32;
 struct DenseKnobs {
     bool forced_q;
     int shape;
     bool forced32;
+    double aim_1m;
+    int ks;
 };
 static const DenseKnobs& dense_knobs() {
     static const DenseKnobs knobs = [] {
@@ -18,6 +22,10 @@
         K.shape = (e && atoi(e) == 32) ? 32 : 16;
         e = getenv("THR_DENSE_QW");
         K.forced32 = e && atoi(e) == 32;
+        e = getenv("THR_DENSE_AIM");
+        K.aim_1m = (e && atof(e) >= 64.0) ? atof(e) : QREG_AIM_1M;
+        e = getenv("THR_DENSE_KS");
+        K.ks = (e && atoi(e) >= 4 && atoi(e) <= 64) ? atoi(e) : QREG_KS;
         return K;
     }();
     return knobs;
@@ -29,7 +37,6 @@
 int qreg_qw(int dim) {
     return (dim == 1024 && !qreg_staggered(dim) && qreg_shape(dim) == 16 && !dense_knobs().forced32) ? 48 : 32;
 }
-constexpr int QREG_MAX_SEG = 1024;
 int qreg_max_queries(int dim) {
     const int qt = qreg_qw(dim) * qreg_waves(dim);
     const int64_t m = (int64_t)UINT32_MAX / ((int64_t)CAND_CAP * (int64_t)sizeof(Cand));
@@ -50,9 +57,9 @@
     p.qpad = p.ntiles * p.qtile;
     const int64_t groups = (n_docs + MF_ROWS - 1) / MF_ROWS;
     p.sampled = n_docs > CAND_CAP / 2;
-    const int ks_cap = p.packed ? 32 : 64;
+    const int ks_cap = p.packed ? dense_knobs().ks : 64;
     p.ksample = kprime < ks_cap ? kprime : ks_cap;
-    double aim = (p.packed ? 2896.0 : 4096.0) * sqrt((double)n_docs / 1.0e6);
+    double aim = (p.packed ? dense_knobs().aim_1m : 4096.0) * sqrt((double)n_docs / 1.0e6);
     const double aim_lo = 8.0 * kprime < 4096.0 ? 8.0 * kprime : 4096.0;
     aim = aim < aim_lo ? aim_lo : aim > 4096.0 ? 4096.0 : aim;
     int64_t target = (int64_t)((double)n_docs * (double)p.ksample / aim);
@@ -75,7 +82,7 @@
     p.tcnt = A.take<int>(p.ntiles);
     p.cand = A.take<Cand>(qpad * CAND_CAP);
     p.tlist = A.take<Cand>((size_t)p.ntiles * p.tile_cap);
-    p.sample = A.take<float>(qpad * (size_t)p.sample_docs);
+    p.sample = A.take<float>(p.packed ? qpad * (size_t)QREG_MAX_SEG * SAMPLE_TOP : qpad * (size_t)p.sample_docs);
     p.qfrag = A.take<_Float16>(p.packed ? qpad * (size_t)dim : 0);
     p.sel_rows = A.take<int32_t>(qpad * SEL_BIG_BAND);
     p.sel_meta = A.take<int32_t>(4 * qpad);
@@ -114,12 +121,12 @@
     const float* tau = all ? nullptr : P.tau;
     float* smp = all ? P.sample : nullptr;
     const int64_t ld = all ? P.sample_docs : 0;
+    if (P.packed)
+        return launch_scan_f16q<MODE>(X.dim, X.docs16, P.qfrag, P.ntiles, units, stride, tau,
+                                      all ? nullptr : P.cnt, all ? nullptr : P.cand, smp, B.st,
+                                      nseg, X.doc_coll, B.query_coll, B.n_queries);
     const int32_t* doc_coll = all ? nullptr : X.doc_coll;
     const int32_t* query_coll = all ? nullptr : B.query_coll;
-    if (P.packed)
-        return launch_scan_f16q<MODE>(X.dim, X.docs16, P.qfrag, P.ntiles, units, stride, tau,
-                                      all ? nullptr : P.cnt, all ? nullptr : P.cand, smp, ld, B.st,
-                                      nseg, doc_coll, query_coll, B.n_queries);
     int* tcnt = all ? nullptr : P.tcnt;
     Cand* tlist = all ? nullptr : P.tlist;
     const int tile_cap = all ? 0 : P.tile_cap;
@@ -134,19 +141,21 @@
 
 static int dense_pipeline(const DensePlan& P, const DenseIndex& X, const DenseBatch& B,
                           const DensePhase& S) {
-    int rc, nseg = 0;
+    int rc, nseg = 0, sample_nseg = 0;
     if (S.phase != PIPE_FINISH) {
-        hipError_t e = hipMemsetAsync(P.cnt, 0, (char*)P.cand - (char*)P.cnt, B.st);
-        if (e != hipSuccess) return (int)e;
+        if (!P.packed) {
+            hipError_t e = hipMemsetAsync(P.cnt, 0, (char*)P.cand - (char*)P.cnt, B.st);
+            if (e != hipSuccess) return (int)e;
+        }
         if (P.packed && (rc = launch_pack_queries(X.dim, B.queries, B.n_queries, P.qpad, P.qfrag, P.qerr, B.st)))
             return rc;
-        if (P.sampled && (rc = launch_scan<MODE_ALL>(P, X, B))) return rc;
-        if ((rc = launch_threshold(P, X, B))) return rc;
+        if (P.sampled && (rc = launch_scan<MODE_ALL>(P, X, B, &sample_nseg))) return rc;
+        if ((rc = launch_threshold(P, X, B, P.packed ? sample_nseg : 0))) return rc;
         if ((rc = launch_scan<MODE_FILTER>(P, X, B, &nseg))) return rc;
         if (!P.packed && (rc = launch_bucket(P, B.st))) return rc;
     } else if (P.packed) {
         if ((rc = launch_scan_f16q<MODE_FILTER, true>(X.dim, X.docs16, P.qfrag, P.ntiles, P.groups, 1,
-                                                      nullptr, nullptr, nullptr, nullptr, 0, B.st, &nseg)))
+                                                      nullptr, nullptr, nullptr, nullptr, B.st, &nseg)))
             return rc;
     }
     if ((rc = launch_band(P, X, B, S, nseg))) return rc;
@@ -367,7 +376,7 @@
     int blocks = 0;
     int rc = launch_scan_f16q<MODE_FILTER, true>(
         dim, reinterpret_cast<const _Float16*>(docs16), P.qfrag, P.ntiles, P.groups, 1, P.tau, P.cnt,
-        P.cand, nullptr, 0, (hipStream_t)stream, nullptr, nullptr, nullptr, n_queries, stamps, &blocks);
+        P.cand, nullptr, (hipStream_t)stream, nullptr, nullptr, nullptr, n_queries, stamps, &blocks);
     *h_n_waves = blocks * qreg_waves(dim);
     return rc;
 }
diff --git a/triple-hybrid-rag_amd/csrc/dense_common.hpp b/triple-hybrid-rag_amd/csrc/dense_common.hpp
--- a/triple-hybrid-rag_amd/csrc/dense_common.hpp
+++ b/triple-hybrid-rag_amd/csrc/dense_common.hpp
@@ -14,6 +14,8 @@
 constexpr uint32_t ROW_MASK = (1u << ROW_BITS) - 1;
 constexpr int ROW_BITS_F16 = 25;
 constexpr int SEL_BIG_BAND = 1024;
+constexpr int QREG_MAX_SEG = 1024;
+constexpr int SAMPLE_TOP = 4;
 constexpr int CS_BINS = 4096;
 
 struct Cand {
@@ -150,7 +152,7 @@
 template <int MODE, bool PROF = false>
 int launch_scan_f16q(int dim, const _Float16* rows16, const _Float16* qfrag, int n_qtiles,
                      int64_t n_row_tiles, int64_t tile_stride, const float* tau, int* seg_cnt,
-                     Cand* cand, float* sample, int64_t sample_ld, hipStream_t st,
+                     Cand* cand, float* sample, hipStream_t st,
                      int* nseg_out = nullptr, const int32_t* doc_coll = nullptr,
                      const int32_t* query_coll = nullptr, int n_queries = 1 << 30,
                      unsigned long long* stamps = nullptr, int* n_blocks = nullptr);
@@ -158,7 +160,7 @@
                         float* qerr, hipStream_t st);
 int launch_quantize_f16(const float* docs, int64_t n_docs, int dim, _Float16* docs16,
                         unsigned int* max_rel_err, hipStream_t st);
-int launch_threshold(const DensePlan& P, const DenseIndex& X, const DenseBatch& B);
+int launch_threshold(const DensePlan& P, const DenseIndex& X, const DenseBatch& B, int sample_nseg);
 int launch_bucket(const DensePlan& P, hipStream_t st);
 int launch_band(const DensePlan& P, const DenseIndex& X, const DenseBatch& B, const DensePhase& S, int nseg);
 int launch_rescore(const DensePlan& P, const DenseIndex& X, const DenseBatch& B);
diff --git a/triple-hybrid-rag_amd/csrc/dense_exact.hip b/triple-hybrid-rag_amd/csrc/dense_exact.hip
--- a/triple-hybrid-rag_amd/csrc/dense_exact.hip
+++ b/triple-hybrid-rag_amd/csrc/dense_exact.hip
@@ -23,7 +23,8 @@
     const float* __restrict__ docs, const double* __restrict__ dnorm, int64_t n_docs, int dim,
     const float* __restrict__ queries, int n_queries, int k, double* __restrict__ slab_s,
     int64_t* __restrict__ slab_id, const uint32_t* __restrict__ skip_certified,
-    const int32_t* __restrict__ doc_coll, const int32_t* __restrict__ query_coll) {
+    const int32_t* __restrict__ doc_coll, const int32_t* __restrict__ query_coll,
+    int32_t* __restrict__ n_done) {
     extern __shared__ float lds_qv[];
     __shared__ double b_s[EX_CAP];
     __shared__ int64_t b_id[EX_CAP];
@@ -33,6 +34,7 @@
     __shared__ double s_qn;
     __shared__ unsigned long long s_todo;
     const int slab = blockIdx.x;
+    if (n_done && blockIdx.x == 0 && blockIdx.y == 0 && threadIdx.x == 0) *n_done = 0;
     {
         const int q = blockIdx.y + (int)threadIdx.x * (int)gridDim.y;
         const bool todo = threadIdx.x < 64 && q < n_queries &&
@@ -229,7 +231,7 @@
     int64_t* slab_id = (int64_t*)(slab_s + (size_t)n_queries * EX_SLABS * k);
     hipLaunchKernelGGL(exact_slab_topk, dim3(EX_SLABS, grid_y), dim3(EX_THREADS),
                        sizeof(float) * dim, st, docs, dnorm, n_docs, dim, queries, n_queries, k,
-                       slab_s, slab_id, certified, doc_coll, query_coll);
+                       slab_s, slab_id, certified, doc_coll, query_coll, n_rescued);
     int rc = launch_status();
     if (rc) return rc;
     hipLaunchKernelGGL(merge_lists<false>, dim3(n_queries), dim3(256), 0, st, slab_s, slab_id,
diff --git a/triple-hybrid-rag_amd/csrc/dense_scan_f16q.hip b/triple-hybrid-rag_amd/csrc/dense_scan_f16q.hip
--- a/triple-hybrid-rag_amd/csrc/dense_scan_f16q.hip
+++ b/triple-hybrid-rag_amd/csrc/dense_scan_f16q.hip
@@ -5,7 +5,7 @@
 template <int MODE, bool PROF>
 int launch_scan_f16q(int dim, const _Float16* rows16, const _Float16* qfrag, int n_qtiles,
                             int64_t n_row_tiles, int64_t tile_stride, const float* tau, int* seg_cnt,
-                            Cand* cand, float* sample, int64_t sample_ld, hipStream_t st,
+                            Cand* cand, float* sample, hipStream_t st,
                             int* nseg_out, const int32_t* doc_coll,
                             const int32_t* query_coll, int n_queries,
                             unsigned long long* stamps, int* n_blocks) {
@@ -21,7 +21,7 @@
     return launch_lds(dense_scan_f16qs<DIM, MODE, SHAPE>, grid, dim3(QS_NW * 64),                 \
                       QStag<DIM>::LDS_BYTES, st, (const f32x4*)rows16, (const f32x4*)qfrag,       \
                       n_qtiles, n_row_tiles, tile_stride, tau, seg_cnt, cand, CAND_CAP / nseg,    \
-                      sample, sample_ld, doc_coll, query_coll, n_queries);
+                      sample, doc_coll, query_coll, n_queries);
     if (stag) {
         if (dim == 512 && shape == 32) THR_QS_LAUNCH(512, 32)
         if (dim == 512) THR_QS_LAUNCH(512, 16)
@@ -33,7 +33,7 @@
     return launch_lds(dense_scan_f16q<DIM, MODE, PROF, SHAPE>, grid, dim3(Q_NW * 64),             \
                       QScan<DIM>::LDS_BYTES, st, (const f32x4*)rows16, (const f32x4*)qfrag,       \
                       n_qtiles, n_row_tiles, tile_stride, tau, seg_cnt, cand, CAND_CAP / nseg,    \
-                      sample, sample_ld, doc_coll, query_coll, n_queries, stamps);
+                      sample, doc_coll, query_coll, n_queries, stamps);
     switch (dim) {
         case 512: if (shape == 16) THR_Q_LAUNCH(512, 16) THR_Q_LAUNCH(512, 32)
         case 768: if (shape == 16) THR_Q_LAUNCH(768, 16) THR_Q_LAUNCH(768, 32)
@@ -78,7 +78,7 @@
 
 #define THR_INSTANTIATE(MODE, PROF)                                                                    \
     template int launch_scan_f16q<MODE, PROF>(int, const _Float16*, const _Float16*, int, int64_t, int64_t, \
-                                              const float*, int*, Cand*, float*, int64_t, hipStream_t, int*, \
+                                              const float*, int*, Cand*, float*, hipStream_t, int*, \
                                               const int32_t*, const int32_t*, int, unsigned long long*, int*);
 THR_INSTANTIATE(MODE_ALL, false)
 THR_INSTANTIATE(MODE_FILTER, false)
diff --git a/triple-hybrid-rag_amd/csrc/dense_scan_f16q.hpp b/triple-hybrid-rag_amd/csrc/dense_scan_f16q.hpp
--- a/triple-hybrid-rag_amd/csrc/dense_scan_f16q.hpp
+++ b/triple-hybrid-rag_amd/csrc/dense_scan_f16q.hpp
@@ -221,6 +221,48 @@
     }
 };
 
+template <int SHAPE>
+struct QTop {
+    static constexpr int NQL = QAcc<SHAPE>::NQL;
+    const int32_t* doc_coll;
+    int qc[NQL];
+    float t[NQL][SAMPLE_TOP];
+    __device__ __forceinline__ void init() {
+#pragma unroll
+        for (int u = 0; u < NQL; ++u)
+#pragma unroll
+            for (int j = 0; j < SAMPLE_TOP; ++j) t[u][j] = -INFINITY;
+    }
+    template <int X>
+    __device__ __forceinline__ void one(const QAcc<SHAPE>& acc, uint32_t row0, int lane) {
+        constexpr int qs = QAcc<SHAPE>::template qsel<X>();
+        float x = acc.template get<X>();
+        x = x == x ? x : -INFINITY;
+        if (doc_coll && qc[qs] != -1 && x > -INFINITY) {
+            const uint32_t row = row0 + (uint32_t)QAcc<SHAPE>::template row<X>(lane);
+            if (doc_coll[row] != qc[qs]) x = -INFINITY;
+        }
+#pragma unroll
+        for (int j = 0; j < SAMPLE_TOP; ++j) {
+            const float hi = fmaxf(t[qs][j], x);
+            x = fminf(t[qs][j], x);
+            t[qs][j] = hi;
+        }
+    }
+    template <int X>
+    __device__ __forceinline__ void all(const QAcc<SHAPE>& acc, uint32_t row0, int lane) {
+        if constexpr (X < QAcc<SHAPE>::NREG) {
+            one<X>(acc, row0, lane);
+            all<X + 1>(acc, row0, lane);
+        }
+    }
+    __device__ __forceinline__ void store(float* __restrict__ sample, int u, int64_t q, int nseg, int seg) const {
+        float* dst = sample + (q * nseg + seg) * SAMPLE_TOP;
+#pragma unroll
+        for (int j = 0; j < SAMPLE_TOP; ++j) dst[j] = t[u][j];
+    }
+};
+
 template <int S, int HS, int K0, int KS, int PER, int SHAPE, int HF, int RING, int NBQ, typename Issue>
 __device__ __forceinline__ void qsx_steps_pe(f32x4 (&a)[RING], const f32x4 (&bq)[NBQ], QAcc<SHAPE>& acc,
                                              uint32_t abase, Issue& issue_piece, QEmit<SHAPE>& em,
@@ -244,7 +286,7 @@
     const f32x4* __restrict__ packed, const f32x4* __restrict__ qfrag, int n_qtiles,
     int64_t n_tiles, int64_t tile_stride, const float* __restrict__ tau,
     int* __restrict__ seg_cnt, Cand* __restrict__ cand, int seg_cap,
-    float* __restrict__ sample_scores, int64_t sample_ld,
+    float* __restrict__ sample,
     const int32_t* __restrict__ doc_coll, const int32_t* __restrict__ query_coll, int n_queries,
     unsigned long long* __restrict__ stamps = nullptr) {
     using C = QScan<DIM>;
@@ -269,12 +311,15 @@
     QEmit<SHAPE> em;
     em.cand = cand;
     em.doc_coll = doc_coll;
+    QTop<SHAPE> top;
+    top.doc_coll = doc_coll;
+    top.init();
     uint32_t start[NQL];
 #pragma unroll
     for (int u = 0; u < NQL; ++u) {
         const int q = q32 * QW + A::query(lane, u);
         em.tau[u] = MODE == MODE_FILTER ? tau[q] : 0.f;
-        em.qc[u] = (MODE == MODE_FILTER && query_coll && q < n_queries) ? query_coll[q] : -1;
+        em.qc[u] = top.qc[u] = (query_coll && q < n_queries) ? query_coll[q] : -1;
         start[u] = (uint32_t)(((int64_t)q * CAND_CAP + (int64_t)my_seg * seg_cap) * sizeof(Cand));
         em.slot[u] = start[u];
         em.end[u] = start[u] + (uint32_t)(seg_cap * sizeof(Cand));
@@ -431,29 +476,7 @@
 
         const int64_t t = first + i * step;
         if constexpr (MODE == MODE_ALL) {
-            if constexpr (SHAPE == 32) {
-                float* dst = sample_scores + (int64_t)(q32 * 32 + (lane & 31)) * sample_ld + t * 32 + 4 * (lane >> 5);
-#pragma unroll
-                for (int g = 0; g < 4; ++g) {
-                    f32x4 v;
-#pragma unroll
-                    for (int j = 0; j < 4; ++j) {
-                        const float sv = acc.v[4 * g + j];
-                        v[j] = sv == sv ? sv : -INFINITY;
-                    }
-                    *reinterpret_cast<f32x4*>(dst + 8 * g) = v;
-                }
-            } else {
-#pragma unroll
-                for (int x = 0; x < 2 * A::NQB; ++x) {
-                    f32x4 v = acc.t[x];
-#pragma unroll
-                    for (int j = 0; j < 4; ++j) v[j] = v[j] == v[j] ? v[j] : -INFINITY;
-                    float* dst = sample_scores + (int64_t)(q32 * QW + 16 * (x % A::NQB) + (lane & 15)) * sample_ld +
-                                 t * 32 + 16 * (x / A::NQB) + 4 * (lane >> 4);
-                    *reinterpret_cast<f32x4*>(dst) = v;
-                }
-            }
+            top.template all<0>(acc, (uint32_t)(t * tile_stride * 32), lane);
         } else {
             em.template all<0>(acc, (uint32_t)(t * tile_stride * 32), lane);
         }
@@ -465,6 +488,9 @@
 #pragma unroll
         for (int u = 0; u < NQL; ++u)
             seg_cnt[(int64_t)(q32 * QW + A::query(lane, u)) * nseg + my_seg] = (int)((em.slot[u] - start[u]) / sizeof(Cand));
+    } else {
+#pragma unroll
+        for (int u = 0; u < NQL; ++u) top.store(sample, u, (int64_t)q32 * QW + A::query(lane, u), nseg, my_seg);
     }
     if constexpr (PROF) {
         if (lane == 0) {
@@ -493,7 +519,7 @@
     const f32x4* __restrict__ packed, const f32x4* __restrict__ qfrag, int n_qtiles,
     int64_t n_tiles, int64_t tile_stride, const float* __restrict__ tau,
     int* __restrict__ seg_cnt, Cand* __restrict__ cand, int seg_cap,
-    float* __restrict__ sample_scores, int64_t sample_ld,
+    float* __restrict__ sample,
     const int32_t* __restrict__ doc_coll, const int32_t* __restrict__ query_coll, int n_queries) {
     using C = QStag<DIM>;
     using A = QAcc<SHAPE>;
@@ -515,12 +541,15 @@
     QEmit<SHAPE> em;
     em.cand = cand;
     em.doc_coll = doc_coll;
+    QTop<SHAPE> top;
+    top.doc_coll = doc_coll;
+    top.init();
     uint32_t start[NQL];
 #pragma unroll
     for (int u = 0; u < NQL; ++u) {
         const int q = q32 * 32 + A::query(lane, u);
         em.tau[u] = MODE == MODE_FILTER ? tau[q] : 0.f;
-        em.qc[u] = (MODE == MODE_FILTER && query_coll && q < n_queries) ? query_coll[q] : -1;
+        em.qc[u] = top.qc[u] = (query_coll && q < n_queries) ? query_coll[q] : -1;
         start[u] = (uint32_t)(((int64_t)q * CAND_CAP + (int64_t)my_seg * seg_cap) * sizeof(Cand));
         em.slot[u] = start[u];
         em.end[u] = start[u] + (uint32_t)(seg_cap * sizeof(Cand));
@@ -543,35 +572,9 @@
                                                               (wave + p * QS_NW) * 1024),
             16, 0, 0);
     };
-    auto emit_all = [&](const A& acc, int64_t i) {
-        const int64_t t = first + i * step;
-        if constexpr (SHAPE == 32) {
-            float* dst = sample_scores + (int64_t)(q32 * 32 + (lane & 31)) * sample_ld + t * 32 + 4 * (lane >> 5);
-#pragma unroll
-            for (int g = 0; g < 4; ++g) {
-                f32x4 v;
-#pragma unroll
-                for (int j = 0; j < 4; ++j) {
-                    const float sv = acc.v[4 * g + j];
-                    v[j] = sv == sv ? sv : -INFINITY;
-                }
-                *reinterpret_cast<f32x4*>(dst + 8 * g) = v;
-            }
-        } else {
-#pragma unroll
-            for (int x = 0; x < 4; ++x) {
-                f32x4 v = acc.t[x];
-#pragma unroll
-                for (int j = 0; j < 4; ++j) v[j] = v[j] == v[j] ? v[j] : -INFINITY;
-                float* dst = sample_scores + (int64_t)(q32 * 32 + 16 * (x & 1) + (lane & 15)) * sample_ld +
-                             t * 32 + 16 * (x >> 1) + 4 * (lane >> 4);
-                *reinterpret_cast<f32x4*>(dst) = v;
-            }
-        }
-    };
 #define QS_EMIT(i_)                                                                                \
     if constexpr (MODE == MODE_ALL) {                                                              \
-        emit_all(acc, (i_));                                                                       \
+        top.template all<0>(acc, (uint32_t)((first + (i_) * step) * tile_stride * 32), lane);      \
     } else {                                                                                       \
         em.template all<0>(acc, (uint32_t)((first + (i_) * step) * tile_stride * 32), lane);       \
     }
@@ -687,6 +690,9 @@
 #pragma unroll
         for (int u = 0; u < NQL; ++u)
             seg_cnt[(int64_t)(q32 * 32 + A::query(lane, u)) * nseg + my_seg] = (int)((em.slot[u] - start[u]) / sizeof(Cand));
+    } else {
+#pragma unroll
+        for (int u = 0; u < NQL; ++u) top.store(sample, u, (int64_t)q32 * 32 + A::query(lane, u), nseg, my_seg);
     }
 }
 
diff --git a/triple-hybrid-rag_amd/csrc/dense_select.hip b/triple-hybrid-rag_amd/csrc/dense_select.hip
--- a/triple-hybrid-rag_amd/csrc/dense_select.hip
+++ b/triple-hybrid-rag_amd/csrc/dense_select.hip
@@ -250,6 +250,62 @@
     }
     const uint32_t key = block_coarse_select([&](int i) { return fkey(val(i)); }, n_sample, kk, hist, aux);
     if (threadIdx.x == 0) tau[q] = coarse_value(key);
+}
+
+constexpr int KT_REG = 16;
+static_assert(QREG_MAX_SEG * SAMPLE_TOP <= 256 * KT_REG, "kth_select_top holds every kept value in registers");
+__global__ __launch_bounds__(256) void kth_select_top(const float* __restrict__ sample, int n_vals, int kk,
+                                                      const float* __restrict__ queries, int n_queries,
+                                                      int dim, float* __restrict__ tau) {
+    __shared__ int hist[256];
+    __shared__ int wsum[4];
+    __shared__ int bc[2];
+    __shared__ int flag;
+    const int q = blockIdx.x, t = threadIdx.x, lane = t & 63, wave = t >> 6;
+    if (query_is_void(queries, n_queries, dim, q, &flag)) {
+        if (t == 0) tau[q] = INFINITY;
+        return;
+    }
+    if (n_vals < kk) {
+        if (t == 0) tau[q] = -INFINITY;
+        return;
+    }
+    uint32_t key[KT_REG];
+#pragma unroll
+    for (int u = 0; u < KT_REG; ++u) {
+        const int i = t + u * 256;
+        key[u] = fkey(i < n_vals ? sample[(int64_t)q * n_vals + i] : -INFINITY);
+    }
+    uint32_t prefix = 0, mask = 0;
+    int remaining = kk;
+#pragma unroll 1
+    for (int shift = 24; shift >= 0; shift -= 8) {
+        hist[t] = 0;
+        __syncthreads();
+#pragma unroll
+        for (int u = 0; u < KT_REG; ++u)
+            if (t + u * 256 < n_vals && (key[u] & mask) == prefix) atomicAdd(&hist[(key[u] >> shift) & 255], 1);
+        __syncthreads();
+        const int mine = hist[255 - t];
+        int incl = mine;
+#pragma unroll
+        for (int o = 1; o < 64; o <<= 1) {
+            const int v = __shfl_up(incl, o, WAVE);
+            if (lane >= o) incl += v;
+        }
+        if (lane == 63) wsum[wave] = incl;
+        __syncthreads();
+        for (int x = 0; x < wave; ++x) incl += wsum[x];
+        if (incl - mine < remaining && remaining <= incl) {
+            bc[0] = 255 - t;
+            bc[1] = incl - mine;
+        }
+        __syncthreads();
+        remaining -= bc[1];
+        prefix |= (uint32_t)bc[0] << shift;
+        mask |= 255u << shift;
+    }
+    if (t == 0) tau[q] = fkey_inv(prefix);
 }
 
 constexpr int SEL_THREADS = 256;
@@ -616,7 +672,12 @@
     }
 }
 
-int launch_threshold(const DensePlan& P, const DenseIndex& X, const DenseBatch& B) {
+int launch_threshold(const DensePlan& P, const DenseIndex& X, const DenseBatch& B, int sample_nseg) {
+    if (P.sampled && sample_nseg > 0) {
+        hipLaunchKernelGGL(kth_select_top, dim3(P.qpad), dim3(256), 0, B.st, (const float*)P.sample,
+                           sample_nseg * SAMPLE_TOP, P.ksample, B.queries, B.n_queries, X.dim, P.tau);
+        return launch_status();
+    }
     hipLaunchKernelGGL(kth_select, dim3(P.qpad), dim3(256), 0, B.st,
                        P.sampled ? (const float*)P.sample : nullptr, P.sample_docs, (int)P.sample_docs,
                        P.ksample, B.queries, B.n_queries, X.dim, P.tau, P.packed ? nullptr : P.qerr,
diff --git a/triple-hybrid-rag_amd/csrc/rrf.hip b/triple-hybrid-rag_amd/csrc/rrf.hip
--- a/triple-hybrid-rag_amd/csrc/rrf.hip
+++ b/triple-hybrid-rag_amd/csrc/rrf.hip
@@ -51,6 +51,47 @@
         if (t < width[ch] && id < 0) atomicMin(&len[ch], t);
     }
     __syncthreads();
+
+    if ((width[0] > 0) + (width[1] > 0) + (width[2] > 0) == 1) {
+        const int ch = width[0] ? 0 : width[1] ? 1 : 2;
+        const double w = ch == 0 ? w_lex : ch == 1 ? w_sem : w_gra;
+        for (int i = t; i < RRF_SLOTS; i += RRF_THREADS) order[i] = -1;
+        __syncthreads();
+        const int n1 = len[ch];
+        int dup = 0;
+        if (t < n1) {
+            const int64_t id = L[ch][t];
+            uint32_t h = (uint32_t)(((uint64_t)id * 0x9E3779B97F4A7C15ull) >> 40);
+            for (;;) {
+                h &= RRF_SLOTS - 1;
+                const int prev = atomicCAS(&order[h], -1, t);
+                if (prev == -1) break;
+                if (L[ch][prev] == id) {
+                    dup = 1;
+                    break;
+                }
+                ++h;
+            }
+        }
+        if (!__syncthreads_or(dup) && w >= 0.0) {
+            for (int i = t; i < top_k; i += RRF_THREADS) {
+                const bool ok = i < n1;
+                const int r = i + 1;
+                double score = -INFINITY;
+                if (ok) {
+                    if (MODE == RRF_RAG2) score = __dadd_rn(0.0, __ddiv_rn(w, (double)(rrf_k + r)));
+                    else score = __dadd_rn(0.0, __dmul_rn(w, __ddiv_rn(1.0, (double)(rrf_k + r))));
+                }
+                out_ids[(int64_t)q * top_k + i] = ok ? L[ch][i] : -1;
+                out_scores[(int64_t)q * top_k + i] = score;
+                if (out_ranks)
+                    for (int c = 0; c < 3; ++c)
+                        out_ranks[((int64_t)q * top_k + i) * 3 + c] = (ok && c == ch) ? r : 0;
+            }
+            if (t == 0) out_counts[q] = n1 < top_k ? n1 : top_k;
+            return;
+        }
+    }
 
     bool nw[3];
     int within[3];
```

Result: faster. 752,100 queries/s (median of 6 runs) (+4.8%).
